# SnakeOnex/vit-is-all-you-need

Measured on AMD Instinct MI355X. Metric: images/sec ViT-B/16 224px bf16 fwd+bwd, higher is better.
Workload: dtype bf16; 1 GPU; ViT-B/16 224x224 bf16 forward+loss+backward, batch 256 per GPU (BASELINE configs[1]; configs[2] at 8 GPUs), random-init weights, 197 tokens, 79.44 M params; global_batch=256, parallelism=dp1

## Files before the change

### include/vitamd.h

```cpp
#ifndef VITAMD_H
#define VITAMD_H

#ifdef __cplusplus
extern "C" {
#endif

#define VITAMD_OK 0
#define VITAMD_ERR_SHAPE 1
#define VITAMD_ERR_ARG 2
#define VITAMD_ERR_LAUNCH 3
#define VITAMD_ERR_INIT 4

int vitamd_abi_version(void);

int vitamd_init(int device, void* stream);

#define VITAMD_EPI_BIAS_BF16 0
#define VITAMD_EPI_GELU 1
#define VITAMD_EPI_RESID_F32 2
#define VITAMD_EPI_DGELU 3
#define VITAMD_EPI_PATCH_F32 4
#define VITAMD_EPI_F32 5
#define VITAMD_EPI_GELU_DG 6
#define VITAMD_EPI_DMUL 7

int vitamd_gemm_nt_bf16(const void* A, const void* B, void* out, void* out2, const float* bias, const void* aux,
                        float* colsum, int M, int N, int K, int ldo, int epi, int n_patches, int seq, int extra,
                        int tile, void* stream);

#define VITAMD_NT_FORM_SMALL 1
#define VITAMD_NT_FORM_PP 2
#define VITAMD_NT_FORM_PP_PERSISTENT 3
#define VITAMD_NT_FORM_SEAM 4
#define VITAMD_NT_FORM_LOADER 5
#define VITAMD_NT_FORM_TAIL_SPLIT 0x80
int vitamd_gemm_nt_plan(int M, int N, int K, int ldo, int epi, int tile);

int vitamd_linear_dropout_resid_bf16(const void* A, const void* B, float* out, const float* bias, const float* resid,
                                     int M, int N, int K, float dropout_p, unsigned long long seed, int tile, void* stream);

int vitamd_gemm_tn_bf16(const void* L, const void* Rm, float* out, int R, int P, int Q, int ldl, int ldr, int ldo,
                        int splits, void* stream);

#define VITAMD_TN_FORM_SHARED 0
#define VITAMD_TN_FORM_EXCLUSIVE 1
int vitamd_gemm_tn_bf16_ws(const void* L, const void* Rm, float* out, int R, int P, int Q, int ldl, int ldr, int ldo,
                           int splits, float* ws, long ws_bytes, int accumulate, int form, void* stream);
long vitamd_gemm_tn_ws_bytes(int R, int P, int Q, int splits);

int vitamd_gemm_tn_bf16_ws_colsum(const void* L, const void* Rm, float* out, float* colsum, int R, int P, int Q, int ldl, int ldr,
                                  int ldo, int splits, float* ws, long ws_bytes, int accumulate, int form, void* stream);

int vitamd_layernorm_fwd(const float* x_in, const void* addend_bf16, float* x_out, void* y_bf16, float* mean,
                         float* rstd, int M, int D, float eps, void* stream);
int vitamd_layernorm_bwd(const void* dy_bf16, const float* x, const float* mean, const float* rstd,
                         const float* g_res, float* g_out, void* g_bf16, float* colsum, int M, int D, void* stream);
int vitamd_layernorm_bwd_dropout(const void* dy_bf16, const float* x, const float* mean, const float* rstd,
                                 const float* g_res, float* g_out, void* g_bf16, float* colsum, int M, int D,
                                 float dropout_p, unsigned long long seed, void* stream);
int vitamd_layernorm_bwd_xhat(const void* dy_bf16, const void* y_bf16, const float* rstd, const float* g_res, float* g_out,
                              void* g_bf16, float* colsum, int M, int D, float dropout_p, unsigned long long seed, void* stream);
int vitamd_layernorm_fwd_keep(const float* x_in, const void* addend_bf16, float* x_out, void* y_bf16, float* mean, float* rstd,
                              int B, int seq, int keep, int D, float eps, void* stream);
int vitamd_layernorm_bwd_keep(const void* dy_bf16, const void* x_or_y, const float* mean, const float* rstd, const float* g_res,
                              float* g_out, void* g_bf16, float* colsum, int B, int seq, int keep, int D, int use_xhat,
                              float dropout_p, unsigned long long seed, void* stream);

int vitamd_layernorm_affine_fwd(const float* x, const float* gamma, const float* beta, void* y_bf16, float* mean,
                                float* rstd, int M, int D, float eps, void* stream);
int vitamd_layernorm_affine_bwd(const void* dy_bf16, const float* x, const float* mean, const float* rstd,
                                const float* gamma, const float* g_res, float* g_out, void* g_bf16, float* colsum,
                                float* dgamma, float* dbeta, int M, int D, void* stream);
int vitamd_layernorm_affine_fwd_f32(const float* x, const float* gamma, const float* beta, float* y, float* mean,
                                    float* rstd, int M, int D, float eps, void* stream);
int vitamd_layernorm_affine_bwd_f32(const float* dy, const float* x, const float* mean, const float* rstd,
                                    const float* gamma, float* g_out, float* dgamma, float* dbeta, int M, int D, void* stream);

int vitamd_attention_fwd(const void* qkv, void* o, float* lse2, int B, int N, int H, int head_dim, int causal,
                         float dropout_p, unsigned long long seed, void* stream);
int vitamd_attention_fwd_resid(const void* qkv, void* o, float* lse2, const float* resid_in, float* resid_out, int B, int N, int H,
                               int head_dim, int causal, float dropout_p, unsigned long long seed, void* stream);
int vitamd_attention_bwd(const void* qkv, const void* o, const float* lse2, const void* d_o, void* dqkv,
                         float* delta, float* dbias, int B, int N, int H, int head_dim, int causal, float dropout_p,
                         unsigned long long seed, void* stream);
int vitamd_attention_keep_forms(int N, int nq);
int vitamd_attention_fwd_keep(const void* qkv, void* o, float* lse2, int B, int N, int H, int head_dim, int nq, void* stream);
int vitamd_attention_bwd_keep(const void* qkv, const void* o, const float* lse2, const void* d_o, void* dqkv, float* delta,
                              float* dbias, int B, int N, int H, int head_dim, int nq, void* stream);

#define VITAMD_ATTN_FWD_SMALL 1
#define VITAMD_ATTN_FWD_SMALL8 2
#define VITAMD_ATTN_FWD_LOOP 3
#define VITAMD_ATTN_FWD_LONG 4
#define VITAMD_ATTN_BWD_PIPE 5
#define VITAMD_ATTN_BWD_LOOP 6
#define VITAMD_ATTN_BWD_LONG 7
#define VITAMD_ATTN_FAMILY(code) ((code) & 0xf)
#define VITAMD_ATTN_TILES(code) ((code) >> 4 & 0xf)
#define VITAMD_ATTN_QTILES(code) ((code) >> 8 & 0xf)
#define VITAMD_ATTN_DROP 0x1000
#define VITAMD_ATTN_CAUSAL 0x2000
#define VITAMD_ATTN_RES 0x4000
#define VITAMD_ATTN_KEEP 0x8000
int vitamd_attention_form(int N, int causal, float dropout_p, int resid, int nq, int backward);

int vitamd_kv_append(const void* qkv, void* k_cache, void* v_cache, const int* len, int B, int T, int H, int head_dim, int Lmax,
                     void* stream);
long vitamd_decode_attention_ws_bytes(int B, int H, int Lmax);
int vitamd_decode_attention(const void* qkv, const void* k_cache, const void* v_cache, void* o, const int* len, int B, int H,
                            int head_dim, int Lmax, float* ws, long ws_bytes, void* stream);
long vitamd_gemm_skinny_ws_bytes(int M, int N, int K);
int vitamd_gemm_skinny_bf16(const void* A, const void* W, void* out, void* out2, const float* bias, const float* aux, int M, int N,
                            int K, int epi, float* ws, long ws_bytes, void* stream);

int vitamd_gemm_skinny_qkv_append(const void* A, const void* W, void* qkv, const float* bias, void* k_cache, void* v_cache, const int* len,
                                  int M, int H, int K, int head_dim, int Lmax, float* ws, long ws_bytes, void* stream);
int vitamd_decode_embed(const float* tok_table, const float* pos_table, const long long* token, const int* len, float* x, int B, int D,
                        int tok_rows, int pos_rows, void* stream);

int vitamd_sample_logits(const float* logits, long long* token, float* info, const float* u, const unsigned long long* step, int B, int V,
                         int ld, float temperature, int top_k, float top_p, unsigned long long seed, void* stream);

int vitamd_cross_entropy_fwd(const void* logits, int logits_bf16, const long long* target, float* loss_row, float* lse, float* stats,
                             int M, int V, int ld, long long ignore_index, void* stream);
int vitamd_cross_entropy_grid_rows(int V);
int vitamd_cross_entropy_bwd(const void* logits, int logits_bf16, const long long* target, const float* lse, const float* stats,
                             const float* grad_out, void* dlogits, int dlogits_bf16, int M, int V, int ld, int ldo,
                             long long ignore_index, void* stream);
int vitamd_soft_cross_entropy_fwd(const void* logits, int logits_bf16, const long long* target_a, const long long* target_b,
                                  const float* lam, float smoothing, float* loss_row, float* lse, float* stats, int M, int V, int ld,
                                  void* stream);
int vitamd_soft_cross_entropy_bwd(const void* logits, int logits_bf16, const long long* target_a, const long long* target_b,
                                  const float* lam, float smoothing, const float* lse, const float* stats, const float* grad_out,
                                  void* dlogits, int dlogits_bf16, int M, int V, int ld, int ldo, void* stream);
int vitamd_embed_tokens_fwd(const float* tok_table, const float* pos_table, const long long* ids, float* x, int B, int S, int D,
                            int tok_rows, int pos_rows, void* stream);
int vitamd_embed_tokens_bwd(const float* g, const long long* ids, float* dtok, float* dpos, int B, int S, int D, int tok_rows, void* stream);
int vitamd_assemble_tokens_fwd(const float* prefix, const float* pos, const float* tok_table, const long long* ids, const float* body,
                               float* x, int B, int E, int S, int D, int tok_rows, int pos_rows, void* stream);
int vitamd_assemble_tokens_bwd(const float* g, const long long* ids, float* dprefix, float* dpos, float* dtok, int B, int E, int S, int D,
                               int tok_rows, int pos_rows, void* stream);
int vitamd_assemble_tokens_grid_cap(void);

int vitamd_frames_prep(const unsigned char* src, const long long* index, const int* geom, const float* table, void* patches_bf16,
                       float* image, int B, int Nsrc, int Hs, int Ws, int C, int H, int W, int p, void* stream);
int vitamd_frames_prep_grid_cap(void);
int vitamd_frames_prep_mix(const unsigned char* src, const long long* index, const int* geom, const float* table, void* patches_bf16,
                           float* image, int B, int Nsrc, int Hs, int Ws, int C, int H, int W, int p, const int* rec, const float* lam,
                           void* stream);
int vitamd_frames_prep_resize(const unsigned char* src, const long long* index, const int* box, const float* mean, const float* std,
                              void* patches_bf16, float* image, int B, int Nsrc, int Hs, int Ws, int C, int H, int W, int p, void* stream);
int vitamd_frames_prep_resize_grid_cap(void);
int vitamd_crop_flip_draw(int* geom, int B, int Hs, int Ws, int H, int W, int flip_enabled, unsigned long long seed,
                          unsigned long long step, void* stream);
int vitamd_frames_to_u8(const float* img, unsigned char* out, int B, int C, int H, int W, void* stream);

int vitamd_cast_f32_bf16(const float* in, void* out_bf16, long n, void* stream);
int vitamd_cast_f32_bf16_dropout(const float* in, void* out_bf16, long n, float dropout_p, unsigned long long seed, void* stream);
int vitamd_dropout_bf16(const void* in, void* out, long n, long group, float dropout_p, unsigned long long seed, void* stream);
int vitamd_dropout_f32(const float* in, float* out, long n, long group, float dropout_p, unsigned long long seed, void* stream);
int vitamd_cast_transpose_weight(const float* w, void* wb, void* wbt, int N, int K, void* stream);
int vitamd_cast_transpose_batched(const void* desc_dev, int n, int total_tiles, void* stream);
int vitamd_im2col_bf16(const float* img, void* out_bf16, int B, int C, int H, int W, int p, void* stream);
int vitamd_colsum_bf16(const void* x_bf16, float* out, int M, int N, int ld, void* stream);
int vitamd_embed_bwd(const float* g, float* dpos, float* dextra, void* dyp_bf16, float* dbias, float* dbias_rows, int B,
                     int seq, int extra, int D, void* stream);

int vitamd_vq_nearest(const float* x, const float* codebook, long long* idx, int M, int K, int d, void* stream);

int vitamd_conv3x3_fwd(const float* x, const float* w, const float* bias, float* y, int B, int Cin, int Cout, int H, int W,
                       void* stream);
// ... 86 lines not shown
```

### vit-is-all-you-need_amd/csrc/attention.hip

```cpp
#include "common.h"
#include "vitamd_internal.h"
#include <type_traits>

namespace {

constexpr int DH = 64;
constexpr int MAX_N = 512;
constexpr int MAX_N_LONG = 16384;
constexpr float NEG_BIG = -1.0e30f;

typedef LDS_AS bf16x4* lds_bf16x4_ptr;

__device__ __forceinline__ int swz(int row) { return (((row >> 1) & 1) << 2) | ((row >> 3) & 3); }

__device__ __forceinline__ void stage_tile(const __bf16* __restrict__ g, int ld, int N, int npad, char* lds, int wave, int lane, int nwaves = 4) {
  const int pieces = npad / 8;
  for (int pc = wave; pc < pieces; pc += nwaves) {
    const int row = pc * 8 + (lane >> 3);
    const int logical = (lane & 7) ^ swz(row);
    const int grow = min(row, N - 1);
    glds16(g + (size_t)grow * ld + logical * 8, lds + pc * 1024);
  }
}

// ... 58 lines not shown
      u32x2 o = {pack_bf16x2(acc[dt][4 * u] * scale, acc[dt][4 * u + 1] * scale),
                 pack_bf16x2(acc[dt][4 * u + 2] * scale, acc[dt][4 * u + 3] * scale)};
      *(u32x2*)(p + 32 * dt + 8 * u) = o;
    }
}

template <int ROWS = 32, bool RES = false>
__device__ __forceinline__ void store_rows_T_img(__bf16* __restrict__ g, int ld, int N, int r0, int lane, const f32x16 (&acc)[2], float scale, char* img,
                                                 float* colacc = nullptr, const float* __restrict__ xi = nullptr, float* __restrict__ xo = nullptr,
                                                 int ldx = 0) {
  const int rr = lane & 31, h = lane >> 5;
  constexpr int ITS = ROWS / 8;
  int pass = 0;
#pragma unroll
  do {
    f32x4 r[ITS][2];
    if constexpr (RES) {
#pragma unroll
      for (int it = 0; it < ITS; ++it) {
        const int row = (lane >> 3) + 8 * it, pc = lane & 7;
        const float* px = xi + (size_t)min(r0 + ROWS * pass + row, N - 1) * ldx + 8 * (pc ^ (row & 7));
        r[it][0] = *(const f32x4*)px;
        r[it][1] = *(const f32x4*)(px + 4);
      }
    }
    if (ROWS == 32 || (rr >> 4) == pass) {
#pragma unroll
      for (int dt = 0; dt < 2; ++dt)
#pragma unroll
        for (int u = 0; u < 4; ++u) {
          u32x2 o = {pack_bf16x2(acc[dt][4 * u] * scale, acc[dt][4 * u + 1] * scale),
                     pack_bf16x2(acc[dt][4 * u + 2] * scale, acc[dt][4 * u + 3] * scale)};
          *(u32x2*)(img + (rr & (ROWS - 1)) * 128 + (((4 * dt + u) ^ (rr & 7)) << 4) + h * 8) = o;
        }
    }
#pragma unroll
    for (int it = 0; it < ITS; ++it) {
      const int row = (lane >> 3) + 8 * it, pc = lane & 7;
      const u32x4 v = *(const u32x4*)(img + row * 128 + pc * 16);
      const int grow = r0 + ROWS * pass + row;
      if (grow < N) {
        const int col = 8 * (pc ^ (row & 7));
        *(u32x4*)(g + (size_t)grow * ld + col) = v;
        if constexpr (RES) {
          f32x4 o0 = {r[it][0][0] + bf16lo(v[0]), r[it][0][1] + bf16hi(v[0]), r[it][0][2] + bf16lo(v[1]), r[it][0][3] + bf16hi(v[1])};
          f32x4 o1 = {r[it][1][0] + bf16lo(v[2]), r[it][1][1] + bf16hi(v[2]), r[it][1][2] + bf16lo(v[3]), r[it][1][3] + bf16hi(v[3])};
          float* po = xo + (size_t)grow * ldx + col;
          *(f32x4*)po = o0;
          *(f32x4*)(po + 4) = o1;
        }
      }
    }
  } while (ROWS == 16 && ++pass < 2);
  if constexpr (ROWS == 32) {
    if (colacc) {
      const int chunk = lane >> 3, within = (lane & 7) * 2;
      const int nrows = min(32, N - r0);
      float sacc = 0.f;
      for (int row = 0; row < nrows; ++row)
        sacc += bf2f(*(const __bf16*)(img + row * 128 + ((chunk ^ (row & 7)) << 4) + within));
      *colacc += sacc;
    }
  }
}

struct AttnArgs {
  const __bf16* qkv;
  __bf16* o;
  float* lse2;
  const __bf16* d_o;
  __bf16* dqkv;
  float* delta;
  float* dbias;
  int B, N, H;
  int causal;
  float scale_log2e;
  float scale;
  unsigned drop_thresh;
  float drop_scale;
  unsigned seed_lo, seed_hi;
  const float* resid_in;
  float* resid_out;
  int nq;
};

struct HeadAddr {
  int b, hh, N, D3, D;
  const __bf16* qbase;
};
template <typename Idx>
__device__ __forceinline__ HeadAddr head_addr(const __bf16* qkv, int N, int H, Idx head) {
  const int b = head / H, hh = head % H, D3 = 3 * H * DH, D = H * DH;
  return {b, hh, N, D3, D, qkv + (size_t)b * N * D3 + hh * DH};
}
__device__ __forceinline__ size_t stat_index(int b, int H, int hh, int N, int row) { return ((size_t)b * H + hh) * N + row; }

__device__ __forceinline__ float attn_keep(const AttnArgs& a, int bh, int query, int key) {
  const unsigned long long idx = ((unsigned long long)bh * a.N + query) * a.N + key;
  return dropout_keep(idx, a.seed_lo, a.seed_hi, a.drop_thresh, a.drop_scale);
}

template <bool DROP>
__global__ __launch_bounds__(256) void attn_fwd_kernel(const AttnArgs a) {
  extern __shared__ __attribute__((aligned(16))) char smem[];
  const int lane = threadIdx.x & 63, wave = __builtin_amdgcn_readfirstlane(threadIdx.x >> 6);
  const auto [b, hh, N, D3, D, qbase] = head_addr(a.qkv, a.N, a.H, blockIdx.x);
  const int nt = (N + 31) / 32, npad = nt * 32;
  char* ktile = smem;
  char* vtile = smem + npad * 128;
  stage_tile(qbase + D, D3, N, npad, ktile, wave, lane);
  stage_tile(qbase + 2 * D, D3, N, npad, vtile, wave, lane);
  asm volatile("s_waitcnt vmcnt(0)" ::: "memory");
  __syncthreads();

  const float c = a.scale_log2e;
  for (int qb = wave; qb < nt; qb += 4) {
    const int q0 = qb * 32;
    const int qrow = q0 + (lane & 31);
    bf16x8 qf[4];
    load_lane_frags(qbase, D3, N, q0, lane, qf);
    f32x16 oacc[2];
    zero(oacc);
    float m = NEG_BIG, l = 0.f;
    const int t_end = a.causal ? min(nt, qb + 1) : nt;
    for (int T = 0; T < t_end; ++T) {
      f32x16 s;
      zero(s);
#pragma unroll
      for (int kk = 0; kk < 4; ++kk) s = __builtin_amdgcn_mfma_f32_32x32x16_bf16(row_frag(ktile, T, kk, lane), qf[kk], s, 0, 0, 0);
      if (32 * T + 32 > N || (a.causal && T == qb)) {
#pragma unroll
        for (int r = 0; r < 16; ++r) {
          const int key = 32 * T + acc_row(r, lane);
          if (!(key < N && (!a.causal || key <= qrow))) s[r] = NEG_BIG;
        }
      }
      float tmax = max16(s);
      tmax = fmaxf(tmax, __shfl_xor(tmax, 32, 64)) * c;
      const float mnew = fmaxf(m, tmax);
      const float alpha = fast_exp2(m - mnew);
      m = mnew;
      float psum = 0.f;
#pragma unroll
      for (int r = 0; r < 16; ++r) {
        s[r] = fast_exp2(__builtin_fmaf(s[r], c, -mnew));
        psum += s[r];
        if constexpr (DROP) s[r] *= attn_keep(a, blockIdx.x, min(qrow, N - 1), min(32 * T + acc_row(r, lane), N - 1));
      }
      l = l * alpha + psum;
#pragma unroll
      for (int dt = 0; dt < 2; ++dt)
#pragma unroll
        for (int r = 0; r < 16; ++r) oacc[dt][r] *= alpha;
#pragma unroll
      for (int sidx = 0; sidx < 2; ++sidx) {
        const bf16x8 pf = acc_to_frag(s, sidx);
#pragma unroll
        for (int dt = 0; dt < 2; ++dt)
          oacc[dt] = __builtin_amdgcn_mfma_f32_32x32x16_bf16(tr_frag(vtile, T, sidx, dt, lane), pf, oacc[dt], 0, 0, 0);
      }
    }
    l += __shfl_xor(l, 32, 64);
    const float inv = 1.0f / l;
    store_rows_T(a.o + (size_t)b * N * D + hh * DH, D, N, q0, lane, oacc, inv);
    if (lane < 32 && qrow < N) a.lse2[stat_index(b, a.H, hh, N, qrow)] = m + log2f(l);
  }
// ... 26 lines not shown

  const float c = a.scale_log2e;
  for (int qb = wrot; qb < nt; qb += 4) {
    const int q0 = qb * 32;
    const int qrow = q0 + (lane & 31);
    if (qb != wrot) {
#pragma unroll
      for (int kk = 0; kk < 4; ++kk) qf[kk] = qf2[kk];
    }
    const int t_end = CAUSAL ? qb + 1 : nt;
    f32x16 s[NKT];
    float mx = NEG_BIG;
#pragma unroll
    for (int T = 0; T < NKT; ++T) {
      if (T < t_end) {
#pragma unroll
        for (int r = 0; r < 16; ++r) s[T][r] = 0.f;
#pragma unroll
        for (int kk = 0; kk < 4; ++kk) s[T] = __builtin_amdgcn_mfma_f32_32x32x16_bf16(row_frag(ktile, T, kk, lane), qf[kk], s[T], 0, 0, 0);
        if (32 * T + 32 > N || (CAUSAL && T == qb)) {
#pragma unroll
          for (int r = 0; r < 16; ++r) {
            const int key = 32 * T + acc_row(r, lane);
            if (!(key < N && (!CAUSAL || key <= qrow))) s[T][r] = NEG_BIG;
          }
        }
        mx = fmaxf(mx, max16(s[T]));
      }
    }
    mx = fmaxf(mx, __shfl_xor(mx, 32, 64));
    const float mc = mx * c;
    float l = 0.f;
    f32x16 oacc[2];
#pragma unroll
    for (int dt = 0; dt < 2; ++dt)
#pragma unroll
      for (int r = 0; r < 16; ++r) oacc[dt][r] = 0.f;
#pragma unroll
    for (int T = 0; T < NKT; ++T) {
      if (T < t_end) {
#pragma unroll
        for (int r = 0; r < 16; ++r) {
          float pexp = fast_exp2(__builtin_fmaf(s[T][r], c, -mc));
          l += pexp;
          if constexpr (DROP) pexp *= attn_keep(a, head, min(qrow, N - 1), min(32 * T + acc_row(r, lane), N - 1));
          s[T][r] = pexp;
        }
#pragma unroll
        for (int sidx = 0; sidx < 2; ++sidx) {
          const bf16x8 pf = acc_to_frag(s[T], sidx);
#pragma unroll
          for (int dt = 0; dt < 2; ++dt)
            oacc[dt] = __builtin_amdgcn_mfma_f32_32x32x16_bf16(tr_frag(vtile, T, sidx, dt, lane), pf, oacc[dt], 0, 0, 0);
        }
      }
    }
    l += __shfl_xor(l, 32, 64);
    const float inv = 1.0f / l;
    if constexpr (RES)
      store_rows_T_img<32, true>(a.o + (size_t)b * N * D + hh * DH, D, N, q0, lane, oacc, inv, oimg, nullptr, a.resid_in + (size_t)b * N * D + hh * DH,
                                 a.resid_out + (size_t)b * N * D + hh * DH, D);
    else
      store_rows_T_img(a.o + (size_t)b * N * D + hh * DH, D, N, q0, lane, oacc, inv, oimg);
    if (lane < 32 && qrow < N) a.lse2[stat_index(b, a.H, hh, N, qrow)] = mc + log2f(l);
  }
}

template <int NKT, bool RES, bool KEEP = false>
__global__ __launch_bounds__(512, 4) void attn_fwd_small8_kernel(const AttnArgs a) {
  extern __shared__ __attribute__((aligned(16))) char smem[];
  const int lane = threadIdx.x & 63, wave = __builtin_amdgcn_readfirstlane(threadIdx.x >> 6);
  const int head = blockIdx.x;
  const auto [b, hh, N, D3, D, qbase] = head_addr(a.qkv, a.N, a.H, head);
  constexpr int nt = NKT, npad = NKT * 32;
  char* ktile = smem;
  char* vtile = smem + npad * 128;
  char* oimg = smem + 2 * npad * 128 + wave * 2048;
  stage_tile(qbase + D, D3, N, npad, ktile, wave, lane, 8);
  stage_tile(qbase + 2 * D, D3, N, npad, vtile, wave, lane, 8);
  const int qb = (wave + head) & 7;
  bool active = qb < nt;
  if constexpr (KEEP) active = qb * 32 < a.nq;
  bf16x8 qf[4];
  load_lane_frags(qbase, D3, N, (active ? qb : 0) * 32, lane, qf);
  asm volatile("s_waitcnt vmcnt(0)" ::: "memory");
#pragma unroll
  for (int kk = 0; kk < 4; ++kk) asm volatile("" : "+v"(qf[kk]));
  __syncthreads();
  if (!active) return;
  const float c = a.scale_log2e;
  const int q0 = qb * 32;
  const int qrow = q0 + (lane & 31);
  float m = NEG_BIG, l = 0.f;
  f32x16 oacc[2];
  zero(oacc);
#pragma unroll 1
  for (int T = 0; T < NKT; ++T) {
    f32x16 st;
    zero(st);
#pragma unroll
    for (int kk = 0; kk < 4; ++kk) st = __builtin_amdgcn_mfma_f32_32x32x16_bf16(row_frag(ktile, T, kk, lane), qf[kk], st, 0, 0, 0);
    if (32 * T + 32 > N) {
#pragma unroll
      for (int r = 0; r < 16; ++r)
        if (!(32 * T + acc_row(r, lane) < N)) st[r] = NEG_BIG;
    }
    float mt = max16(st);
    mt = fmaxf(mt, __shfl_xor(mt, 32, 64));
    const float mn = fmaxf(m, mt);
    const float alpha = fast_exp2((m - mn) * c);
    m = mn;
    const float mc = mn * c;
    float lt = 0.f;
#pragma unroll
    for (int r = 0; r < 16; ++r) {
      const float pexp = fast_exp2(__builtin_fmaf(st[r], c, -mc));
      lt += pexp;
      st[r] = pexp;
    }
    l = l * alpha + lt;
    if (T > 0) {
#pragma unroll
      for (int dt = 0; dt < 2; ++dt)
#pragma unroll
        for (int r = 0; r < 16; ++r) oacc[dt][r] *= alpha;
    }
#pragma unroll
    for (int sidx = 0; sidx < 2; ++sidx) {
      const bf16x8 pf = acc_to_frag(st, sidx);
#pragma unroll
      for (int dt = 0; dt < 2; ++dt)
        oacc[dt] = __builtin_amdgcn_mfma_f32_32x32x16_bf16(tr_frag(vtile, T, sidx, dt, lane), pf, oacc[dt], 0, 0, 0);
    }
  }
  l += __shfl_xor(l, 32, 64);
  const float mc = m * c;
  const float inv = 1.0f / l;
  if constexpr (KEEP) {
    store_rows_T_img<16>(a.o + (size_t)b * a.nq * D + hh * DH, D, a.nq, q0, lane, oacc, inv, oimg);
    if (lane < 32 && qrow < a.nq) a.lse2[stat_index(b, a.H, hh, N, qrow)] = mc + log2f(l);
    return;
  }
  if constexpr (RES)
    store_rows_T_img<16, true>(a.o + (size_t)b * N * D + hh * DH, D, N, q0, lane, oacc, inv, oimg, nullptr, a.resid_in + (size_t)b * N * D + hh * DH,
                               a.resid_out + (size_t)b * N * D + hh * DH, D);
  else
    store_rows_T_img<16>(a.o + (size_t)b * N * D + hh * DH, D, N, q0, lane, oacc, inv, oimg);
  if (lane < 32 && qrow < N) a.lse2[stat_index(b, a.H, hh, N, qrow)] = mc + log2f(l);
}

template <bool DROP, bool CAUSAL>
__global__ __launch_bounds__(256, 2) void attn_bwd_dq_kernel(const AttnArgs a) {
  extern __shared__ __attribute__((aligned(16))) char smem[];
  const int lane = threadIdx.x & 63, wave = __builtin_amdgcn_readfirstlane(threadIdx.x >> 6);
  const auto [b, hh, N, D3, D, qbase] = head_addr(a.qkv, a.N, a.H, blockIdx.x);
  const int nt = (N + 31) / 32, npad = nt * 32;
  char* ktile = smem;
  char* vtile = smem + npad * 128;
  char* oimg = smem + 2 * npad * 128 + wave * 4096;
  stage_tile(qbase + D, D3, N, npad, ktile, wave, lane);
  stage_tile(qbase + 2 * D, D3, N, npad, vtile, wave, lane);
  asm volatile("s_waitcnt vmcnt(0)" ::: "memory");
  __syncthreads();

  const float c = a.scale_log2e;
  const __bf16* obase = a.o + (size_t)b * N * D + hh * DH;
  const __bf16* dobase = a.d_o + (size_t)b * N * D + hh * DH;
  float csum_q = 0.f;
  for (int qb = (wave + blockIdx.x) & 3; qb < nt; qb += 4) {
    const int q0 = qb * 32;
    const int qrow = q0 + (lane & 31);
    bf16x8 qf[4], dof[4], of[4];
    load_lane_frags(qbase, D3, N, q0, lane, qf);
    load_lane_frags(dobase, D, N, q0, lane, dof);
    load_lane_frags(obase, D, N, q0, lane, of);
    float delta = 0.f;
#pragma unroll
    for (int kk = 0; kk < 4; ++kk)
#pragma unroll
      for (int j = 0; j < 8; ++j) delta += (float)dof[kk][j] * (float)of[kk][j];
    delta += __shfl_xor(delta, 32, 64);
    const size_t stat = stat_index(b, a.H, hh, N, min(qrow, N - 1));
    const float lse2 = a.lse2[stat];
    if (lane < 32 && qrow < N) a.delta[stat] = delta;

    f32x16 dq[2];
    zero(dq);
    const int t_end = CAUSAL ? min(nt, qb + 1) : nt;
    for (int T = 0; T < t_end; ++T) {
      f32x16 s, dp;
      zero(s);
      zero(dp);
#pragma unroll
      for (int kk = 0; kk < 4; ++kk) {
        s = __builtin_amdgcn_mfma_f32_32x32x16_bf16(row_frag(ktile, T, kk, lane), qf[kk], s, 0, 0, 0);
        dp = __builtin_amdgcn_mfma_f32_32x32x16_bf16(row_frag(vtile, T, kk, lane), dof[kk], dp, 0, 0, 0);
      }
#pragma unroll
      for (int r = 0; r < 16; ++r) {
        const float pexp = fast_exp2(__builtin_fmaf(s[r], c, -lse2));
        float dpr = dp[r];
        if constexpr (DROP) dpr *= attn_keep(a, blockIdx.x, min(qrow, N - 1), min(32 * T + acc_row(r, lane), N - 1));
        s[r] = pexp * (dpr - delta);
      }
      if (32 * T + 32 > N || (CAUSAL && T == qb)) {
#pragma unroll
        for (int r = 0; r < 16; ++r) {
          const int key = 32 * T + acc_row(r, lane);
          if (!(key < N && (!CAUSAL || key <= qrow))) s[r] = 0.f;
        }
      }
#pragma unroll
      for (int sidx = 0; sidx < 2; ++sidx) {
        const bf16x8 dsf = acc_to_frag(s, sidx);
#pragma unroll
        for (int dt = 0; dt < 2; ++dt)
          dq[dt] = __builtin_amdgcn_mfma_f32_32x32x16_bf16(tr_frag(ktile, T, sidx, dt, lane), dsf, dq[dt], 0, 0, 0);
      }
    }
    store_rows_T_img(a.dqkv + (size_t)b * N * D3 + hh * DH, D3, N, q0, lane, dq, a.scale, oimg, a.dbias ? &csum_q : nullptr);
  }
  if (a.dbias) atomicAdd(a.dbias + hh * DH + lane, csum_q);
}

template <int NT, int NQT = NT, bool LIM = false>
__global__ __launch_bounds__(256, 2) void attn_bwd_dq_pipe_kernel(const AttnArgs a) {
  extern __shared__ __attribute__((aligned(16))) char smem[];
  const int lane = threadIdx.x & 63, wave = __builtin_amdgcn_readfirstlane(threadIdx.x >> 6);
  const int head = blockIdx.x;
  const auto [b, hh, N, D3, D, qbase] = head_addr(a.qkv, a.N, a.H, head);
  constexpr int nt = NT, npad = NT * 32;
  char* ktile = smem;
  char* vtile = smem + npad * 128;
  char* oimg = smem + 2 * npad * 128 + wave * 4096;
  stage_tile(qbase + D, D3, N, npad, ktile, wave, lane);
  stage_tile(qbase + 2 * D, D3, N, npad, vtile, wave, lane);
  int nq = N;
  if constexpr (LIM) nq = a.nq;
  const __bf16* obase = a.o + (size_t)b * nq * D + hh * DH;
  const __bf16* dobase = a.d_o + (size_t)b * nq * D + hh * DH;
  asm volatile("s_waitcnt vmcnt(0)" ::: "memory");
  __syncthreads();

  const float c = a.scale_log2e;
  float csum_q = 0.f;
  for (int qb = (wave + head) & 3; qb < nt; qb += 4) {
    const int q0 = qb * 32;
    const int qrow = q0 + (lane & 31);
    if constexpr (LIM) {
      if (qb >= NQT) {
        __bf16* zp = a.dqkv + (size_t)b * N * D3 + hh * DH + 8 * (lane & 7);
#pragma unroll
        for (int it = 0; it < 4; ++it) {
          const int row = q0 + (lane >> 3) + 8 * it;
          if (row < N) *(u32x4*)(zp + (size_t)row * D3) = (u32x4){0u, 0u, 0u, 0u};
        }
        continue;
      }
    }
    bf16x8 qf[4], dof[4];
    float delta = 0.f;
    {
      bf16x8 of[4];
      load_lane_frags(qbase, D3, N, q0, lane, qf);
      load_lane_frags(dobase, D, nq, q0, lane, dof);
      load_lane_frags(obase, D, nq, q0, lane, of);
      if constexpr (LIM) {
        if (qrow >= nq) {
#pragma unroll
          for (int kk = 0; kk < 4; ++kk)
#pragma unroll
            for (int j = 0; j < 8; ++j) dof[kk][j] = (__bf16)0.f;
        }
      }
#pragma unroll
      for (int kk = 0; kk < 4; ++kk)
#pragma unroll
        for (int j = 0; j < 8; ++j) delta += (float)dof[kk][j] * (float)of[kk][j];
    }
    delta += __shfl_xor(delta, 32, 64);
    const size_t stat = stat_index(b, a.H, hh, N, min(qrow, nq - 1));
    float lse2 = a.lse2[stat];
    if constexpr (LIM) lse2 = qrow < nq ? lse2 : 1.0e30f;
    if (lane < 32 && qrow < nq) a.delta[stat] = delta;

    f32x16 dq[2];
#pragma unroll
    for (int dt = 0; dt < 2; ++dt)
#pragma unroll
      for (int r = 0; r < 16; ++r) dq[dt][r] = 0.f;
    bf16x8 kr[2][4], vr[2][4];
    f32x16 sb[2], dpb[2];
    auto products = [&](int buf) {
#pragma unroll
      for (int r = 0; r < 16; ++r) { sb[buf][r] = 0.f; dpb[buf][r] = 0.f; }
#pragma unroll
      for (int kk = 0; kk < 4; ++kk) {
        sb[buf] = __builtin_amdgcn_mfma_f32_32x32x16_bf16(kr[buf][kk], qf[kk], sb[buf], 0, 0, 0);
        dpb[buf] = __builtin_amdgcn_mfma_f32_32x32x16_bf16(vr[buf][kk], dof[kk], dpb[buf], 0, 0, 0);
      }
    };
#pragma unroll
    for (int kk = 0; kk < 4; ++kk) { kr[0][kk] = row_frag(ktile, 0, kk, lane); vr[0][kk] = row_frag(vtile, 0, kk, lane); }
    if (NT > 1) {
#pragma unroll
      for (int kk = 0; kk < 4; ++kk) { kr[1][kk] = row_frag(ktile, 1, kk, lane); vr[1][kk] = row_frag(vtile, 1, kk, lane); }
    }
    products(0);
#pragma unroll
    for (int T = 0; T < NT; ++T) {
      const int cur = T & 1, nxt = cur ^ 1;
      bf16x8 ktr[2][2];
#pragma unroll
      for (int sidx = 0; sidx < 2; ++sidx)
#pragma unroll
        for (int dt = 0; dt < 2; ++dt) ktr[sidx][dt] = tr_frag(ktile, T, sidx, dt, lane);
      __builtin_amdgcn_sched_barrier(0);
      if (T + 1 < NT) products(nxt);
      if (T + 2 < NT) {
#pragma unroll
        for (int kk = 0; kk < 4; ++kk) { kr[cur][kk] = row_frag(ktile, T + 2, kk, lane); vr[cur][kk] = row_frag(vtile, T + 2, kk, lane); }
      }
#pragma unroll
      for (int r = 0; r < 16; ++r) {
        const float pexp = fast_exp2(__builtin_fmaf(sb[cur][r], c, -lse2));
        sb[cur][r] = pexp * (dpb[cur][r] - delta);
      }
      if (T == NT - 1 && 32 * T + 32 > N) {
#pragma unroll
        for (int r = 0; r < 16; ++r)
          if (!(32 * T + acc_row(r, lane) < N)) sb[cur][r] = 0.f;
      }
#pragma unroll
      for (int sidx = 0; sidx < 2; ++sidx) {
        const bf16x8 dsf = acc_to_frag(sb[cur], sidx);
#pragma unroll
        for (int dt = 0; dt < 2; ++dt) dq[dt] = __builtin_amdgcn_mfma_f32_32x32x16_bf16(ktr[sidx][dt], dsf, dq[dt], 0, 0, 0);
      }
    }
    store_rows_T_img(a.dqkv + (size_t)b * N * D3 + hh * DH, D3, N, q0, lane, dq, a.scale, oimg, a.dbias ? &csum_q : nullptr);
  }
  if (a.dbias) atomicAdd(a.dbias + hh * DH + lane, csum_q);
}

template <bool DROP, bool CAUSAL>
__global__ __launch_bounds__(256, 2) void attn_bwd_dkv_kernel(const AttnArgs a) {
  extern __shared__ __attribute__((aligned(16))) char smem[];
  const int lane = threadIdx.x & 63, wave = __builtin_amdgcn_readfirstlane(threadIdx.x >> 6);
  const auto [b, hh, N, D3, D, qbase] = head_addr(a.qkv, a.N, a.H, blockIdx.x);
  const int nt = (N + 31) / 32, npad = nt * 32;
  char* qtile = smem;
  char* dotile = smem + npad * 128;
  float* lse_s = (float*)(smem + 2 * npad * 128);
  float* delta_s = lse_s + npad;
  char* oimg = smem + 2 * npad * 128 + 2 * npad * 4 + wave * 4096;
  const __bf16* dobase = a.d_o + (size_t)b * N * D + hh * DH;
  stage_tile(qbase, D3, N, npad, qtile, wave, lane);
  stage_tile(dobase, D, N, npad, dotile, wave, lane);
  for (int i = threadIdx.x; i < npad; i += 256) {
    const size_t stat = stat_index(b, a.H, hh, N, min(i, N - 1));
    lse_s[i] = a.lse2[stat];
    delta_s[i] = a.delta[stat];
  }
  asm volatile("s_waitcnt vmcnt(0)" ::: "memory");
  __syncthreads();

  const float c = a.scale_log2e;
  float csum_k = 0.f, csum_v = 0.f;
  for (int kb = (wave + blockIdx.x) & 3; kb < nt; kb += 4) {
    const int k0 = kb * 32;
    const int krow = k0 + (lane & 31);
    bf16x8 kf[4], vf[4];
    load_lane_frags(qbase + D, D3, N, k0, lane, kf);
    load_lane_frags(qbase + 2 * D, D3, N, k0, lane, vf);
    f32x16 dk[2], dv[2];
    zero(dk);
    zero(dv);
    const int t_beg = CAUSAL ? kb : 0;
    for (int T = t_beg; T < nt; ++T) {
      f32x16 s, dp;
      zero(s);
      zero(dp);
#pragma unroll
      for (int kk = 0; kk < 4; ++kk) {
        s = __builtin_amdgcn_mfma_f32_32x32x16_bf16(row_frag(qtile, T, kk, lane), kf[kk], s, 0, 0, 0);
        dp = __builtin_amdgcn_mfma_f32_32x32x16_bf16(row_frag(dotile, T, kk, lane), vf[kk], dp, 0, 0, 0);
      }
      f32x16 pmat;
#pragma unroll
      for (int u = 0; u < 4; ++u) {
        const int qr = 32 * T + 8 * u + 4 * (lane >> 5);
        const f32x4 lse4 = *(const f32x4*)(lse_s + qr);
        const f32x4 del4 = *(const f32x4*)(delta_s + qr);
#pragma unroll
        for (int i = 0; i < 4; ++i) {
          const int r = 4 * u + i;
          const float pexp = fast_exp2(__builtin_fmaf(s[r], c, -lse4[i]));
          float keep = 1.0f;
          if constexpr (DROP) keep = attn_keep(a, blockIdx.x, min(qr + i, N - 1), min(krow, N - 1));
          pmat[r] = pexp * keep;
          s[r] = pexp * (dp[r] * keep - del4[i]);
        }
        if (32 * T + 32 > N || k0 + 32 > N || (CAUSAL && T == kb)) {
#pragma unroll
          for (int i = 0; i < 4; ++i) {
            const int r = 4 * u + i, query = qr + i;
            if (!(query < N && krow < N && (!CAUSAL || krow <= query))) { pmat[r] = 0.f; s[r] = 0.f; }
          }
        }
      }
#pragma unroll
      for (int sidx = 0; sidx < 2; ++sidx) {
        const bf16x8 pf = acc_to_frag(pmat, sidx);
        const bf16x8 dsf = acc_to_frag(s, sidx);
#pragma unroll
        for (int dt = 0; dt < 2; ++dt) {
          dv[dt] = __builtin_amdgcn_mfma_f32_32x32x16_bf16(tr_frag(dotile, T, sidx, dt, lane), pf, dv[dt], 0, 0, 0);
          dk[dt] = __builtin_amdgcn_mfma_f32_32x32x16_bf16(tr_frag(qtile, T, sidx, dt, lane), dsf, dk[dt], 0, 0, 0);
        }
      }
    }
    __bf16* dbase = a.dqkv + (size_t)b * N * D3 + hh * DH;
    store_rows_T_img(dbase + D, D3, N, k0, lane, dk, a.scale, oimg, a.dbias ? &csum_k : nullptr);
    store_rows_T_img(dbase + 2 * D, D3, N, k0, lane, dv, 1.0f, oimg, a.dbias ? &csum_v : nullptr);
  }
  if (a.dbias) {
    atomicAdd(a.dbias + D + hh * DH + lane, csum_k);
    atomicAdd(a.dbias + 2 * D + hh * DH + lane, csum_v);
  }
}

template <int NT, int NQT = NT, bool LIM = false>
__global__ __launch_bounds__(256, 2) void attn_bwd_dkv_pipe_kernel(const AttnArgs a) {
  extern __shared__ __attribute__((aligned(16))) char smem[];
  const int lane = threadIdx.x & 63, wave = __builtin_amdgcn_readfirstlane(threadIdx.x >> 6);
  const int head = blockIdx.x;
  const int b = head / a.H, hh = head % a.H;
  const int N = a.N, D3 = 3 * a.H * DH, D = a.H * DH;
  constexpr int nt = NT, npad = NQT * 32;
  int nq = N;
  if constexpr (LIM) nq = a.nq;
  char* qtile = smem;
  char* dotile = smem + npad * 128;
  float* lse_s = (float*)(smem + 2 * npad * 128);
  float* delta_s = lse_s + npad;
  char* oimg = smem + 2 * npad * 128 + 2 * npad * 4 + wave * 4096;
  const __bf16* qbase = a.qkv + (size_t)b * N * D3 + hh * DH;
  const __bf16* dobase = a.d_o + (size_t)b * nq * D + hh * DH;
  stage_tile(qbase, D3, N, npad, qtile, wave, lane);
  stage_tile(dobase, D, nq, npad, dotile, wave, lane);
  for (int i = threadIdx.x; i < npad; i += 256) {
    const size_t stat = ((size_t)b * a.H + hh) * N + min(i, nq - 1);
    lse_s[i] = i < nq ? a.lse2[stat] : 1.0e30f;
    delta_s[i] = a.delta[stat];
  }
  asm volatile("s_waitcnt vmcnt(0)" ::: "memory");
  __syncthreads();

  const float c = a.scale_log2e;
  float csum_k = 0.f, csum_v = 0.f;
  for (int kb = (wave + head) & 3; kb < nt; kb += 4) {
    const int k0 = kb * 32;
    bf16x8 kf[4], vf[4];
    load_lane_frags(qbase + D, D3, N, k0, lane, kf);
    load_lane_frags(qbase + 2 * D, D3, N, k0, lane, vf);
    f32x16 dk[2], dv[2];
    zero(dk);
    zero(dv);
    bf16x8 qr[4], dor[4];
    f32x16 sb, dpb;
    auto products = [&]() {
      zero(sb);
      zero(dpb);
#pragma unroll
      for (int kk = 0; kk < 4; ++kk) {
        sb = __builtin_amdgcn_mfma_f32_32x32x16_bf16(qr[kk], kf[kk], sb, 0, 0, 0);
        dpb = __builtin_amdgcn_mfma_f32_32x32x16_bf16(dor[kk], vf[kk], dpb, 0, 0, 0);
      }
    };
#pragma unroll
    for (int kk = 0; kk < 4; ++kk) { qr[kk] = row_frag(qtile, 0, kk, lane); dor[kk] = row_frag(dotile, 0, kk, lane); }
    products();
    if (NQT > 1) {
#pragma unroll
      for (int kk = 0; kk < 4; ++kk) { qr[kk] = row_frag(qtile, 1, kk, lane); dor[kk] = row_frag(dotile, 1, kk, lane); }
    }
#pragma unroll
    for (int T = 0; T < NQT; ++T) {
      bf16x8 dotr[2][2], qtr[2][2];
      f32x4 lse4[4], del4[4];
#pragma unroll
      for (int sidx = 0; sidx < 2; ++sidx)
#pragma unroll
        for (int dt = 0; dt < 2; ++dt) { dotr[sidx][dt] = tr_frag(dotile, T, sidx, dt, lane); qtr[sidx][dt] = tr_frag(qtile, T, sidx, dt, lane); }
      __builtin_amdgcn_sched_barrier(0);
#pragma unroll
      for (int u = 0; u < 4; ++u) {
        const int qr0 = 32 * T + 8 * u + 4 * (lane >> 5);
        lse4[u] = *(const f32x4*)(lse_s + qr0);
        del4[u] = *(const f32x4*)(delta_s + qr0);
      }
      f32x16 pmat;
#pragma unroll
      for (int u = 0; u < 4; ++u)
#pragma unroll
        for (int i = 0; i < 4; ++i) {
          const int r = 4 * u + i;
          const float pexp = fast_exp2(__builtin_fmaf(sb[r], c, -lse4[u][i]));
          pmat[r] = pexp;
          sb[r] = pexp * (dpb[r] - del4[u][i]);
        }
#pragma unroll
      for (int sidx = 0; sidx < 2; ++sidx) {
        const bf16x8 pf = acc_to_frag(pmat, sidx);
        const bf16x8 dsf = acc_to_frag(sb, sidx);
#pragma unroll
        for (int dt = 0; dt < 2; ++dt) {
          dv[dt] = __builtin_amdgcn_mfma_f32_32x32x16_bf16(dotr[sidx][dt], pf, dv[dt], 0, 0, 0);
          dk[dt] = __builtin_amdgcn_mfma_f32_32x32x16_bf16(qtr[sidx][dt], dsf, dk[dt], 0, 0, 0);
        }
      }
      if (T + 1 < NQT) products();
      if (T + 2 < NQT) {
#pragma unroll
        for (int kk = 0; kk < 4; ++kk) { qr[kk] = row_frag(qtile, T + 2, kk, lane); dor[kk] = row_frag(dotile, T + 2, kk, lane); }
      }
    }
    __bf16* dbase = a.dqkv + (size_t)b * N * D3 + hh * DH;
    store_rows_T_img(dbase + D, D3, N, k0, lane, dk, a.scale, oimg, a.dbias ? &csum_k : nullptr);
    store_rows_T_img(dbase + 2 * D, D3, N, k0, lane, dv, 1.0f, oimg, a.dbias ? &csum_v : nullptr);
  }
  if (a.dbias) {
// ... 408 lines not shown
      return with_flag(f.drop, [&](auto DR) {
        const dim3 grid(a.B * a.H, (nkt + 3) / 4);
        if (int el = launch<attn_bwd_dq_long_kernel<CONST_OF(DR)>>(grid, block, 2 * CH * 128 + 4 * 4096, stream, a)) return el;
        return launch<attn_bwd_dkv_long_kernel<CONST_OF(DR)>>(grid, block, 2 * CH * 128 + 2 * CH * 4 + 4 * 4096, stream, a);
      });
    case ATTN_BWD_PIPE:
      if (f.keep)
        return with_tiles<2, 7>(f.nt, [&](auto K) {
          return with_tiles<1, 4>(f.nqt, [&](auto Q) { return launch_bwd_pipe<CONST_OF(K), CONST_OF(Q), true>(a, stream); });
        });
      return with_tiles<2, 7>(f.nt, [&](auto K) { return launch_bwd_pipe<CONST_OF(K), CONST_OF(K), false>(a, stream); });
    case ATTN_BWD_LOOP:
      return with_flag(f.drop, [&](auto DR) {
        return with_flag(f.causal, [&](auto CAUSAL) {
          const dim3 grid(a.B * a.H);
          if (int el = launch<attn_bwd_dq_kernel<CONST_OF(DR), CONST_OF(CAUSAL)>>(grid, block, 2 * npad * 128 + 4 * 4096, stream, a)) return el;
          return launch<attn_bwd_dkv_kernel<CONST_OF(DR), CONST_OF(CAUSAL)>>(grid, block, 2 * npad * 128 + 2 * npad * 4 + 4 * 4096, stream, a);
        });
      });
  }
  return VITAMD_ERR_SHAPE;
}

int attention_fwd_impl(const void* qkv, void* o, float* lse2, const float* resid_in, float* resid_out, int B, int N, int H, int head_dim, int causal,
                       float dropout_p, unsigned long long seed, void* stream_) {
  AttnArgs a;
  if (int e = make_args(a, false, qkv, o, lse2, nullptr, nullptr, nullptr, nullptr, B, N, H, head_dim, causal, dropout_p, seed)) return e;
  a.resid_in = resid_in;
  a.resid_out = resid_out;
  AttnForm f;
  if (int e = attention_form(f, N, causal != 0, a.drop_thresh != 0u, resid_in != nullptr, 0, false)) return e;
  return launched(launch_fwd(f, a, (hipStream_t)stream_));
}

}

extern "C" int vitamd_attention_form(int N, int causal, float dropout_p, int resid, int nq, int backward) {
  AttnForm f;
  const DropoutParams d = dropout_params(dropout_p, 0ull);
  if (int e = attention_form(f, N, causal != 0, d.ok ? d.thresh != 0u : dropout_p != 0.f, resid != 0, nq, backward != 0)) return -e;
  if (!d.ok) return -VITAMD_ERR_ARG;
  return f.code();
}

extern "C" int vitamd_attention_fwd(const void* qkv, void* o, float* lse2, int B, int N, int H, int head_dim, int causal,
                                    float dropout_p, unsigned long long seed, void* stream_) {
  return attention_fwd_impl(qkv, o, lse2, nullptr, nullptr, B, N, H, head_dim, causal, dropout_p, seed, stream_);
}

extern "C" int vitamd_attention_fwd_resid(const void* qkv, void* o, float* lse2, const float* resid_in, float* resid_out, int B, int N,
                                          int H, int head_dim, int causal, float dropout_p, unsigned long long seed, void* stream_) {
  if (!resid_in || !resid_out) return VITAMD_ERR_ARG;
  AttnForm f;
  if (int e = attention_form(f, N, false, false, true, 0, false)) return e;
  return attention_fwd_impl(qkv, o, lse2, resid_in, resid_out, B, N, H, head_dim, causal, dropout_p, seed, stream_);
}

extern "C" int vitamd_attention_bwd(const void* qkv, const void* o, const float* lse2, const void* d_o, void* dqkv, float* delta,
                                    float* dbias, int B, int N, int H, int head_dim, int causal, float dropout_p,
                                    unsigned long long seed, void* stream_) {
  AttnArgs a;
  if (int e = make_args(a, true, qkv, o, lse2, d_o, dqkv, delta, dbias, B, N, H, head_dim, causal, dropout_p, seed)) return e;
  AttnForm f;
  if (int e = attention_form(f, N, causal != 0, a.drop_thresh != 0u, false, 0, true)) return e;
  return launched(launch_bwd(f, a, (hipStream_t)stream_));
}

extern "C" int vitamd_attention_keep_forms(int N, int nq) {
  if (nq <= 0) return 0;
  AttnForm f;
  return (attention_form(f, N, false, false, false, nq, false) == VITAMD_OK ? 1 : 0) |
         (attention_form(f, N, false, false, false, nq, true) == VITAMD_OK ? 2 : 0);
}

extern "C" int vitamd_attention_fwd_keep(const void* qkv, void* o, float* lse2, int B, int N, int H, int head_dim, int nq, void* stream_) {
  AttnArgs a;
  if (int e = make_args(a, false, qkv, o, lse2, nullptr, nullptr, nullptr, nullptr, B, N, H, head_dim, 0, 0.f, 0ull, nq)) return e;
  AttnForm f;
  if (nq <= 0) return VITAMD_ERR_SHAPE;
  if (int e = attention_form(f, N, false, false, false, nq, false)) return e;
  return launched(launch_fwd(f, a, (hipStream_t)stream_));
}

extern "C" int vitamd_attention_bwd_keep(const void* qkv, const void* o, const float* lse2, const void* d_o, void* dqkv, float* delta,
                                         float* dbias, int B, int N, int H, int head_dim, int nq, void* stream_) {
  AttnArgs a;
  if (int e = make_args(a, true, qkv, o, lse2, d_o, dqkv, delta, dbias, B, N, H, head_dim, 0, 0.f, 0ull, nq)) return e;
  AttnForm f;
  if (nq <= 0) return VITAMD_ERR_SHAPE;
  if (int e = attention_form(f, N, false, false, false, nq, true)) return e;
  return launched(launch_bwd(f, a, (hipStream_t)stream_));
}
```

### vit-is-all-you-need_amd/csrc/capi.hip

```cpp
#include "common.h"
#include "vitamd_internal.h"
#include "../../include/vitamd.h"

extern "C" int vitamd_abi_version(void) { return 9; }

extern "C" int vitamd_init(int device, void* stream) { return vitamd_init_impl(device, (hipStream_t)stream); }

extern "C" int vitamd_gemm_nt_bf16(const void* A, const void* B, void* out, void* out2, const float* bias, const void* aux,
                                   float* colsum, int M, int N, int K, int ldo, int epi, int n_patches, int seq, int extra,
                                   int tile, void* stream) {
  const int dg = (epi == 6 || epi == 7) ? 1 : 0;
  if (epi == 6) epi = EPI_GELU;
  if (epi == 7) epi = EPI_DGELU;
  GemmNtArgs p{A, B, out, out2, bias, aux, colsum, M, N, K, ldo, epi, n_patches, seq, extra, tile, 0u, 1.0f, 0u, 0u, 0, dg};
  if (!is_auto(tile) && tile != NT_TILE_128 && tile != NT_TILE_256 && tile != NT_TILE_320 && tile != NT_TILE_LOADER && tile != NT_TILE_SEAM) return VITAMD_ERR_ARG;
  return vitamd_gemm_nt_impl(p, (hipStream_t)stream);
}

extern "C" int vitamd_gemm_nt_plan(int M, int N, int K, int ldo, int epi, int tile) {
  const int dg = (epi == 6 || epi == 7) ? 1 : 0;
  if (epi == 6) epi = EPI_GELU;
  if (epi == 7) epi = EPI_DGELU;
  static char dummy[16];
  GemmNtArgs p{dummy, dummy, dummy, dummy, nullptr, dummy, (float*)dummy, M, N, K, ldo, epi, 1, 1, 0, tile, 0u, 1.0f, 0u, 0u, 0, dg};
  if (!is_auto(tile) && tile != NT_TILE_128 && tile != NT_TILE_256 && tile != NT_TILE_320 && tile != NT_TILE_LOADER && tile != NT_TILE_SEAM) return -VITAMD_ERR_ARG;
  return vitamd_gemm_nt_plan_impl(p);
}

extern "C" int vitamd_gemm_tn_bf16(const void* L, const void* Rm, float* out, int R, int P, int Q, int ldl, int ldr, int ldo,
                                   int splits, void* stream) {
  GemmTnArgs a{L, Rm, out, R, P, Q, ldl, ldr, ldo, splits, nullptr, 0, 1, 0};
  return vitamd_gemm_tn_impl(a, (hipStream_t)stream);
}

extern "C" int vitamd_gemm_tn_bf16_ws(const void* L, const void* Rm, float* out, int R, int P, int Q, int ldl, int ldr, int ldo,
                                      int splits, float* ws, long ws_bytes, int accumulate, int form, void* stream) {
  if (form != 0 && form != 1) return VITAMD_ERR_ARG;
  GemmTnArgs a{L, Rm, out, R, P, Q, ldl, ldr, ldo, splits, ws, (size_t)(ws_bytes < 0 ? 0 : ws_bytes), accumulate, form};
  return vitamd_gemm_tn_impl(a, (hipStream_t)stream);
}

extern "C" int vitamd_gemm_tn_bf16_ws_colsum(const void* L, const void* Rm, float* out, float* colsum, int R, int P, int Q, int ldl, int ldr,
                                             int ldo, int splits, float* ws, long ws_bytes, int accumulate, int form, void* stream) {
  if (form != 0 && form != 1) return VITAMD_ERR_ARG;
  GemmTnArgs a{L, Rm, out, R, P, Q, ldl, ldr, ldo, splits, ws, (size_t)(ws_bytes < 0 ? 0 : ws_bytes), accumulate, form, colsum};
  if (colsum && !ws) return VITAMD_ERR_ARG;
  return vitamd_gemm_tn_impl(a, (hipStream_t)stream);
}

extern "C" int vitamd_linear_dropout_resid_bf16(const void* A, const void* B, float* out, const float* bias, const float* resid,
                                                int M, int N, int K, float dropout_p, unsigned long long seed, int tile, void* stream) {
  if (!is_auto(tile) && tile != NT_TILE_128 && tile != NT_TILE_256 && tile != NT_TILE_320) return VITAMD_ERR_ARG;
  const DropoutParams d = dropout_params(dropout_p, seed);
  if (!d.ok) return VITAMD_ERR_ARG;
  GemmNtArgs p{A, B, out, nullptr, bias, resid, nullptr, M, N, K, N, EPI_RESID_F32, 0, 0, 0, tile, d.thresh, d.scale, d.seed_lo, d.seed_hi, 0, 0};
  return vitamd_gemm_nt_impl(p, (hipStream_t)stream);
}
```

### vit-is-all-you-need_amd/csrc/gemm_nt.hip

```cpp
#include <type_traits>
#include <mutex>
#include <atomic>
#include <cmath>
#include <cstring>
#include <climits>
#include "gemm_nt_ld.h"

namespace {

template <int BM, int BN, int WM, int WN, int EPI>
__global__ __launch_bounds__(WM * WN * 64) void gemm_nt_kernel(const GemmNtArgs p) {
  constexpr int NW = WM * WN;
  constexpr int WTM = BM / WM, WTN = BN / WN;
  constexpr int MT = WTM / 16, NT = WTN / 16;
  constexpr int PIECES = (BM + BN) / 8;
  constexpr int PPW = PIECES / NW;
  static_assert(PIECES % NW == 0, "pieces must divide over waves");
  constexpr int BUF_BYTES = (BM + BN) * 128;

  extern __shared__ __attribute__((aligned(16))) char smem[];

  const int tid = threadIdx.x;
  const int lane = tid & 63;
  const int wave = __builtin_amdgcn_readfirstlane(tid >> 6);
  const int wm = wave / WN, wn = wave % WN;

  const int tiles_n = (p.N + BN - 1) / BN;
  const int tiles_m = (p.M + BM - 1) / BM;
  const int tile = xcd_remap(blockIdx.x, tiles_m * tiles_n);
  const int m0 = (tile / tiles_n) * BM;
  const int n0 = (tile % tiles_n) * BN;

  const __bf16* __restrict__ A = (const __bf16*)p.A;
  const __bf16* __restrict__ B = (const __bf16*)p.B;
  const int K = p.K;

  const __bf16* src[PPW];
#pragma unroll
  for (int i = 0; i < PPW; ++i) {
    const int piece = wave * PPW + i;
    const int row = piece * 8 + (lane >> 3);
    const int logical = (lane & 7) ^ (row & 7);
    if (piece < BM / 8) {
      const int g = min(m0 + row, p.M - 1);
      src[i] = A + (size_t)g * K + logical * 8;
    } else {
      const int g = min(n0 + row - BM, p.N - 1);
      src[i] = B + (size_t)g * K + logical * 8;
    }
  }

  auto stage = [&](int kt, int buf) {
    char* base = smem + buf * BUF_BYTES + wave * PPW * 1024;
#pragma unroll
    for (int i = 0; i < PPW; ++i) glds16(src[i] + kt * BK, base + i * 1024);
  };

  f32x4 acc[MT][NT];
#pragma unroll
  for (int i = 0; i < MT; ++i)
#pragma unroll
    for (int j = 0; j < NT; ++j) acc[i][j] = (f32x4){0.f, 0.f, 0.f, 0.f};

  const int frag_off = (lane & 15) * 128 + ((((lane >> 4) ^ (lane & 7)) & 7) << 4);
  const int a_off = wm * WTM * 128 + frag_off;
  const int b_off = BM * 128 + wn * WTN * 128 + frag_off;

  const int nkt = K / BK;
  stage(0, 0);
  for (int kt = 0; kt < nkt; ++kt) {
    const int cur = kt & 1;
    asm volatile("s_waitcnt vmcnt(0)" ::: "memory");
    __syncthreads();
    if (kt + 1 < nkt) stage(kt + 1, cur ^ 1);
    const char* buf = smem + cur * BUF_BYTES;
#pragma unroll
    for (int ks = 0; ks < 2; ++ks) {
      bf16x8 af[MT], bfr[NT];
#pragma unroll
      for (int j = 0; j < NT; ++j) bfr[j] = *(const bf16x8*)(buf + ((b_off + j * 16 * 128) ^ (ks * 64)));
#pragma unroll
      for (int i = 0; i < MT; ++i) af[i] = *(const bf16x8*)(buf + ((a_off + i * 16 * 128) ^ (ks * 64)));
#pragma unroll
      for (int i = 0; i < MT; ++i)
#pragma unroll
        for (int j = 0; j < NT; ++j)
          acc[i][j] = __builtin_amdgcn_mfma_f32_16x16x32_bf16(bfr[j], af[i], acc[i][j], 0, 0, 0);
    }
  }
  if constexpr (BM == 256 && BN == 256 && WM == 2 && WN == 4 && EPI != EPI_F32) {
    if (p.N % 8 == 0 && p.ldo % 8 == 0) {
      gemm_epilogue_rows<EPI>(p, acc, m0, n0, wm, wn, lane, tid, wave, smem);
      return;
    }
  }
  gemm_epilogue<BN, WM, WN, WTM, WTN, MT, NT, EPI>(p, acc, m0, n0, wm, wn, lane, tid, smem);
}

template <int EPI, int MT, int LA, int LB, bool PERS = false>
__global__ __launch_bounds__(512) void gemm_nt_pp_kernel(const GemmNtArgs p) {
  using S = NtSchedule<MT, LA>;
  static_assert(LB == S::LB, "the B lead the shared schedule implements");
  constexpr int NP = S::NP;
  constexpr int BM = 32 * MT, BN = 256, WN = 4, NT = 4;
  constexpr int PART = 64 * 128;
  constexpr int BUFB = NP * PART + 256 * 128;

  extern __shared__ __attribute__((aligned(16))) char smem[];
  const int tid = threadIdx.x, lane = tid & 63;
  const int wave = __builtin_amdgcn_readfirstlane(tid >> 6);
  const int wm = wave / WN, wn = wave % WN;
  const int tiles_n = (p.N + BN - 1) / BN, tiles_m = (p.M + BM - 1) / BM;
  const int ntiles = tiles_m * tiles_n;
  const int K = p.K;
  const int nkt = K / 64;
  const srd_t srdA = make_srd(p.A, (size_t)p.M * K * 2);
  const srd_t srdB = make_srd(p.B, (size_t)p.N * K * 2);
  for (int ti = blockIdx.x; ti < ntiles; ti += PERS ? (int)gridDim.x : ntiles) {
  const NtTile t = nt_tile<BM>(ti, tiles_m, tiles_n);
  const int m0 = t.m0, n0 = t.n0;
  unsigned voffA[NP], voffB[4];
  pp_offsets<MT, false>(p, t, wave, lane, voffA, voffB);
  const unsigned lds0 = lds_addr(smem) + wave * 1024;
  constexpr unsigned OOB = 0x80000000u;
  auto request_a = [&](int kt, int j) {
    const bool live = kt >= 0 && kt < nkt;
    asm_glds16(srdA, lds0 + (kt & 1) * BUFB + j * PART, live ? voffA[j] : OOB, live ? (unsigned)kt * 128u : 0u);
  };
  auto request_b = [&](int kt, int q) {
    const bool live = kt >= 0 && kt < nkt;
    asm_glds16(srdB, lds0 + (kt & 1) * BUFB + NP * PART + q * 8192, live ? voffB[q] : OOB, live ? (unsigned)kt * 128u : 0u);
  };

  f32x4 acc[MT][NT];
#pragma unroll
  for (int i = 0; i < MT; ++i)
#pragma unroll
    for (int j = 0; j < NT; ++j) acc[i][j] = (f32x4){0.f, 0.f, 0.f, 0.f};

  const char *rdA[2], *rdB[2];
  frag_bases(smem + wm * 32 * 128, lane, rdA);
  frag_bases(smem + NP * PART + wn * 64 * 128, lane, rdB);

#pragma unroll
  for (int P = -S::lookback; P < 0; ++P) S::requests(S::tile_of(P), S::phase_of(P), request_a, request_b);
  VITAMD_WAIT_VM(S::wait(NP - 1));
  __builtin_amdgcn_s_barrier();
  asm volatile("" ::: "memory");
  if (wm == 1) __builtin_amdgcn_s_barrier();

  auto ktile = [&](int kt, auto bufc) {
    constexpr int BUF = decltype(bufc)::value;
    pp_ktile<MT, PART>(acc, rdA[0] + BUF * BUFB, rdA[1] + BUF * BUFB, rdB[0] + BUF * BUFB, rdB[1] + BUF * BUFB,
                       [&](int ph) { S::requests(kt, ph, request_a, request_b); }, [&](int ph) { VITAMD_WAIT_VM(S::wait(ph)); });
  };
  int kt = 0;
  for (; kt + 1 < nkt; kt += 2) {
    ktile(kt, std::integral_constant<int, 0>{});
    ktile(kt + 1, std::integral_constant<int, 1>{});
  }
  if (kt < nkt) ktile(kt, std::integral_constant<int, 0>{});
  if (wm == 0) __builtin_amdgcn_s_barrier();
  asm volatile("s_waitcnt vmcnt(0)" ::: "memory");
  if constexpr (EPI == EPI_F32) gemm_epilogue<BN, 2, WN, 16 * MT, 64, MT, NT, EPI>(p, acc, m0, n0, wm, wn, lane, tid, smem);
  else if (p.N % 8 == 0 && p.ldo % 8 == 0) gemm_epilogue_rows<EPI, MT>(p, acc, m0, n0, wm, wn, lane, tid, wave, smem);
  else gemm_epilogue<BN, 2, WN, 16 * MT, 64, MT, NT, EPI>(p, acc, m0, n0, wm, wn, lane, tid, smem);
  if constexpr (PERS) __syncthreads();
  }
}

static int device_cus() {
  static int cus[16] = {};
  int dev = 0;
  if (hipGetDevice(&dev) != hipSuccess || dev < 0 || dev >= 16) return 256;
  if (!cus[dev]) {
    int n = 0;
    cus[dev] = (hipDeviceGetAttribute(&n, hipDeviceAttributeMultiprocessorCount, dev) == hipSuccess && n > 0) ? n : 256;
  }
  return cus[dev];
}

template <int EPI, int MT, int LA, int LB, bool PERS = false>
int launch_pp(const GemmNtArgs& p, hipStream_t stream) {
  constexpr int ops_b = 2 * ((MT / 2) * 8192 + 32768), epi_b = 8 * MT * 2048;
  return launch_tiles(gemm_nt_pp_kernel<EPI, MT, LA, LB, PERS>, p, stream, 32 * MT, 512, ops_b > epi_b ? ops_b : epi_b, PERS ? device_cus() : INT_MAX);
}
#undef VITAMD_WAIT_VM

template <int BM, int BN, int WM, int WN, int EPI>
int launch(const GemmNtArgs& p, hipStream_t stream) {
  constexpr int lds = 2 * (BM + BN) * 128;
  auto kern = gemm_nt_kernel<BM, BN, WM, WN, EPI>;
  if (int e = set_lds(kern, lds)) return e;
  const int tiles = ((p.M + BM - 1) / BM) * ((p.N + BN - 1) / BN);
  hipLaunchKernelGGL(kern, dim3(tiles), dim3(WM * WN * 64), lds, stream, p);
  return hipGetLastError() == hipSuccess ? VITAMD_OK : VITAMD_ERR_LAUNCH;
}

static bool prefer_tall(const GemmNtArgs& p) {
// ... 6 lines not shown

static unsigned short bf16_rne_d(double v) {
  auto val = [](unsigned short b) { const unsigned w = (unsigned)b << 16; float g; memcpy(&g, &w, 4); return (double)g; };
  const float f = (float)v;
  unsigned u;
  memcpy(&u, &f, 4);
  unsigned short best = (unsigned short)((u + 0x7fffu + ((u >> 16) & 1u)) >> 16);
  double bd = fabs(val(best) - v);
  const unsigned short first = best;
  for (int dl = -1; dl <= 1; dl += 2) {
    const unsigned short n = (unsigned short)(first + dl);
    const double dd = fabs(val(n) - v);
    if (dd < bd || (dd == bd && !(n & 1) && (best & 1))) { best = n; bd = dd; }
  }
  return best;
}

static std::atomic<const unsigned*> g_gelu_tab[64];

static const unsigned* gelu_table() {
  int dev = -1;
  if (hipGetDevice(&dev) != hipSuccess || dev < 0 || dev >= 64) { (void)hipGetLastError(); return nullptr; }
  return g_gelu_tab[dev].load(std::memory_order_acquire);
}

}

const unsigned* vitamd_gelu_table() { return gelu_table(); }

int vitamd_init_impl(int device, hipStream_t stream) {
  static std::mutex mu;
  static unsigned host[4096];
  static bool built = false;
  int cur = -1;
  if (hipGetDevice(&cur) != hipSuccess) { (void)hipGetLastError(); return VITAMD_ERR_LAUNCH; }
  if (device < 0) device = cur;
  if (device >= 64) return VITAMD_ERR_ARG;
  std::lock_guard<std::mutex> lock(mu);
  if (g_gelu_tab[device].load(std::memory_order_acquire)) return VITAMD_OK;
  hipStreamCaptureStatus cap = hipStreamCaptureStatusNone;
  if (hipStreamIsCapturing(stream, &cap) != hipSuccess || cap != hipStreamCaptureStatusNone) { (void)hipGetLastError(); return VITAMD_ERR_ARG; }
  if (!built) {
    for (int sg = 0; sg < 2; ++sg)
      for (int i = 0; i < 2048; ++i) {
        const unsigned w = (unsigned)(0x3900 + i) << 16;
        float ax;
        memcpy(&ax, &w, 4);
        const double x = sg ? -(double)ax : (double)ax;
        const double cdf = 0.5 * erfc(-x * 0.70710678118654752440);
        const double pdf = 0.39894228040143267794 * exp(-0.5 * x * x);
        host[sg * 2048 + i] = (unsigned)bf16_rne_d(x * cdf) | ((unsigned)bf16_rne_d(cdf + x * pdf) << 16);
      }
    built = true;
  }
  if (device != cur && hipSetDevice(device) != hipSuccess) { (void)hipGetLastError(); return VITAMD_ERR_ARG; }
  void* d = nullptr;
  bool ok = hipMalloc(&d, sizeof(host)) == hipSuccess;
  ok = ok && hipMemcpy(d, host, sizeof(host), hipMemcpyHostToDevice) == hipSuccess && hipDeviceSynchronize() == hipSuccess;
  if (!ok) {
    (void)hipGetLastError();
    if (d) (void)hipFree(d);
  }
  if (device != cur) (void)hipSetDevice(cur);
  if (!ok) return VITAMD_ERR_LAUNCH;
  g_gelu_tab[device].store((const unsigned*)d, std::memory_order_release);
  return VITAMD_OK;
}

namespace {

enum NtForm { NT_FORM_SMALL = 1, NT_FORM_PP = 2, NT_FORM_PP_PERSISTENT = 3, NT_FORM_SEAM = 4, NT_FORM_LOADER = 5 };
struct NtPlan { int form, rows, err; };

static NtPlan plan_single(const GemmNtArgs& p) {
  int tile = p.tile;
  const int epi = p.epi;
  const bool seam_epi = epi == EPI_BIAS_BF16 || epi == EPI_GELU || epi == EPI_DGELU;
  const bool tall_epi = seam_epi || epi == EPI_RESID_F32;
  if (tile == NT_TILE_LOADER) return (seam_epi && ld_ok(p)) ? NtPlan{NT_FORM_LOADER, 256, VITAMD_OK} : NtPlan{0, 0, VITAMD_ERR_SHAPE};
  if (tile == NT_TILE_SEAM) return (seam_epi && seam_ok(p)) ? NtPlan{NT_FORM_SEAM, 256, VITAMD_OK} : NtPlan{0, 0, VITAMD_ERR_SHAPE};
  const bool no_seam = tile == NT_TILE_AUTO_NO_SEAM;
  if (no_seam) tile = NT_TILE_AUTO;
  const long big_tiles = (long)((p.M + 255) / 256) * ((p.N + 255) / 256);
  const bool pp_ok = (size_t)p.M * p.K * 2 < 0xf0000000ull && (size_t)p.N * p.K * 2 < 0xf0000000ull && p.K % 64 == 0;
  const bool big = p.N >= 256 && big_tiles >= 192 && pp_ok;
  const bool tall = tall_epi && prefer_tall(p);
  if (tile == NT_TILE_AUTO_NO_PERSISTENT) tile = NT_TILE_AUTO;
  else if (tile == NT_TILE_AUTO && big) {
    const int cus = device_cus();
    if (seam_epi && !no_seam && seam_ok(p) && p.K <= 1536) {
      if (epi == EPI_BIAS_BF16 && tall && (long)((p.M + 319) / 320) * ((p.N + 255) / 256) >= 3L * cus) return NtPlan{NT_FORM_SEAM, 320, VITAMD_OK};
      if (big_tiles >= 3L * cus) return NtPlan{ld_ok(p) ? NT_FORM_LOADER : NT_FORM_SEAM, 256, VITAMD_OK};
    }
    return NtPlan{NT_FORM_PP_PERSISTENT, tall ? 320 : 256, VITAMD_OK};
  }
  if (tile == NT_TILE_AUTO) tile = big ? (tall ? NT_TILE_320 : NT_TILE_256) : NT_TILE_128;
  if (tile == NT_TILE_320) return (tall_epi && pp_ok) ? NtPlan{NT_FORM_PP, 320, VITAMD_OK} : NtPlan{0, 0, VITAMD_ERR_SHAPE};
  if (tile == NT_TILE_256) return pp_ok ? NtPlan{NT_FORM_PP, 256, VITAMD_OK} : NtPlan{0, 0, VITAMD_ERR_SHAPE};
  if (tile != NT_TILE_128) return NtPlan{0, 0, VITAMD_ERR_ARG};
  return p.K % BK == 0 ? NtPlan{NT_FORM_SMALL, 128, VITAMD_OK} : NtPlan{0, 0, VITAMD_ERR_SHAPE};
}

template <int EPI>
int dispatch_tile(const GemmNtArgs& p, hipStream_t stream) {
  constexpr bool seam_epi = EPI == EPI_BIAS_BF16 || EPI == EPI_GELU || EPI == EPI_DGELU;
  constexpr bool tall_epi = seam_epi || EPI == EPI_RESID_F32;
  const NtPlan pl = plan_single(p);
  if (pl.err) return pl.err;
  switch (pl.form) {
    case NT_FORM_LOADER:
      if constexpr (EPI == EPI_DGELU) { if (!p.colsum) return launch_ld<EPI_DGELU_NOCS>(p, stream, device_cus()); }
      if constexpr (seam_epi) return launch_ld<EPI, EPI == EPI_GELU>(p, stream, device_cus());
      break;
    case NT_FORM_SEAM:
      if constexpr (EPI == EPI_DGELU) { if (!p.colsum) return launch_seam<EPI_DGELU_NOCS, 8>(p, stream, device_cus()); }
      if constexpr (EPI == EPI_BIAS_BF16) { if (pl.rows == 320) return launch_seam<EPI, 10>(p, stream, device_cus()); }
      if constexpr (seam_epi) return launch_seam<EPI, 8, EPI == EPI_GELU>(p, stream, device_cus());
      break;
    case NT_FORM_PP_PERSISTENT:
      if constexpr (tall_epi) { if (pl.rows == 320) return launch_pp<EPI, 10, 4, 6, true>(p, stream); }
      return launch_pp<EPI, 8, 4, 6, true>(p, stream);
    case NT_FORM_PP:
      if constexpr (tall_epi) { if (pl.rows == 320) return launch_pp<EPI, 10, 4, 6>(p, stream); }
      return launch_pp<EPI, 8, 4, 6>(p, stream);
    case NT_FORM_SMALL:
      return launch<128, 128, 2, 2, EPI>(p, stream);
  }
  return VITAMD_ERR_SHAPE;
}

}

static int dispatch_epi(const GemmNtArgs& p, hipStream_t stream) {
  switch (p.epi) {
    case EPI_BIAS_BF16: return dispatch_tile<EPI_BIAS_BF16>(p, stream);
    case EPI_GELU: return dispatch_tile<EPI_GELU>(p, stream);
    case EPI_RESID_F32: return dispatch_tile<EPI_RESID_F32>(p, stream);
    case EPI_DGELU: return dispatch_tile<EPI_DGELU>(p, stream);
    case EPI_PATCH_F32: return dispatch_tile<EPI_PATCH_F32>(p, stream);
    case EPI_F32: return dispatch_tile<EPI_F32>(p, stream);
    default: return VITAMD_ERR_ARG;
  }
}

static int tail_split_rows(const GemmNtArgs& p, bool& tall) {
  const int CUS = device_cus();
  tall = is_auto(p.tile) && prefer_tall(p);
  const int bm = tall ? 320 : 256;
  const int tiles_m = (p.M + bm - 1) / bm, tiles_n = (p.N + 255) / 256;
  const long big_tiles = (long)tiles_m * tiles_n;
  const long rem = big_tiles % CUS;
  const bool split_on = p.epi == EPI_RESID_F32 && !tall;
  if (!(is_auto(p.tile) && split_on && p.epi != EPI_PATCH_F32 && p.N >= 256 && p.K % 64 == 0 && big_tiles > 2 * CUS && rem != 0 && rem * 10 < CUS * 6))
    return 0;
  const int rows_a = (int)((big_tiles - rem) / tiles_n) * bm;
  return rows_a > 0 && rows_a < p.M ? rows_a : 0;
}

static int check_args(const GemmNtArgs& p) {
  if (p.M <= 0 || p.N <= 0 || p.K <= 0 || p.K % 32 != 0 || p.N % 4 != 0 || p.ldo % 4 != 0) return VITAMD_ERR_SHAPE;
  if (!p.A || !p.B || !p.out) return VITAMD_ERR_ARG;
  if (p.epi == EPI_GELU && !p.out2) return VITAMD_ERR_ARG;
  if ((p.epi == EPI_RESID_F32 || p.epi == EPI_DGELU) && !p.aux) return VITAMD_ERR_ARG;
  if (p.epi == EPI_PATCH_F32 && (!p.aux || p.n_patches <= 0)) return VITAMD_ERR_ARG;
  if (p.epi < EPI_BIAS_BF16 || p.epi > EPI_F32) return VITAMD_ERR_ARG;
  return VITAMD_OK;
}

constexpr size_t NT_SPAN = 0x80000000ull;
constexpr int NT_PANEL_ROWS = 1280;

static size_t out_esz(const GemmNtArgs& p) { return (p.epi == EPI_RESID_F32 || p.epi == EPI_PATCH_F32 || p.epi == EPI_F32) ? 4 : 2; }

static int panel_rows(const GemmNtArgs& p) {
  if ((size_t)p.N * p.K * 2 >= NT_SPAN) return 0;
  const size_t kb = (size_t)p.K * 2, ob = (size_t)p.ldo * out_esz(p), row_bytes = kb > ob ? kb : ob;
  if ((size_t)p.M * row_bytes < NT_SPAN) return p.M;
  if (p.epi == EPI_PATCH_F32) return 0;
  return (int)((NT_SPAN - 1) / row_bytes / NT_PANEL_ROWS) * NT_PANEL_ROWS;
}

static GemmNtArgs rows_of(const GemmNtArgs& p, int r0, int rows) {
  GemmNtArgs q = p;
  q.M = rows;
  q.A = (const char*)p.A + (size_t)r0 * p.K * 2;
  q.out = (char*)p.out + (size_t)r0 * p.ldo * out_esz(p);
  if (p.out2) q.out2 = (char*)p.out2 + (size_t)r0 * p.ldo * 2;
  if (p.aux && p.epi != EPI_PATCH_F32) q.aux = (const char*)p.aux + (size_t)r0 * p.ldo * (p.epi == EPI_RESID_F32 ? 4 : 2);
  q.row0 = p.row0 + r0;
  return q;
}

static GemmNtArgs head_of(const GemmNtArgs& p, int rows_a, bool tall) {
  GemmNtArgs a = p;
  if (rows_a) {
    a.M = rows_a;
    a.tile = tall ? p.tile : NT_TILE_256;
  }
  return a;
}

static int launch_rows(const GemmNtArgs& p, hipStream_t stream) {
  bool tall = false;
  const int rows_a = tail_split_rows(p, tall);
  if (int e = dispatch_epi(head_of(p, rows_a, tall), stream)) return e;
  if (!rows_a) return VITAMD_OK;
  GemmNtArgs b = rows_of(p, rows_a, p.M - rows_a);
  b.tile = NT_TILE_128;
  return dispatch_epi(b, stream);
}

static int plan_rows(const GemmNtArgs& p) {
  bool tall = false;
  const int rows_a = tail_split_rows(p, tall);
  const NtPlan pl = plan_single(head_of(p, rows_a, tall));
  if (pl.err) return -pl.err;
  return pl.form | (pl.rows << 8) | (rows_a ? 0x80 : 0);
}

int vitamd_gemm_nt_impl(const GemmNtArgs& p0, hipStream_t stream) {
  if (int e = check_args(p0)) return e;
  const int rows = panel_rows(p0);
  if (!rows) return VITAMD_ERR_SHAPE;
  GemmNtArgs p = p0;
  if (p.epi == EPI_GELU) {
    p.gelu_tab = gelu_table();
    if (!p.gelu_tab) return VITAMD_ERR_INIT;
  }
  if (rows >= p.M) return launch_rows(p, stream);
  const int last = (p.M - 1) / rows * rows;
  if (int e = plan_rows(rows_of(p, 0, rows)); e < 0) return -e;
  if (int e = plan_rows(rows_of(p, last, p.M - last)); e < 0) return -e;
  for (int r0 = 0; r0 < p.M; r0 += rows)
    if (int e = launch_rows(rows_of(p, r0, p.M - r0 < rows ? p.M - r0 : rows), stream)) return e;
  return VITAMD_OK;
}

int vitamd_gemm_nt_plan_impl(const GemmNtArgs& p0) {
  if (int e = check_args(p0)) return -e;
  const int rows = panel_rows(p0);
  if (!rows) return -VITAMD_ERR_SHAPE;
  if (rows >= p0.M) return plan_rows(p0);
  const int last = (p0.M - 1) / rows * rows;
  if (int e = plan_rows(rows_of(p0, last, p0.M - last)); e < 0) return e;
  return plan_rows(rows_of(p0, 0, rows));
}
```

### vit-is-all-you-need_amd/csrc/gemm_nt_ld.h

```cpp
#pragma once
#include "gemm_nt_seam.h"

namespace {

template <int EPI, bool TAB = false, int SCHED = 1>
__global__ __launch_bounds__(768) void gemm_nt_ld_kernel(const GemmNtArgs p) {
  static_assert(EPI == EPI_BIAS_BF16 || EPI == EPI_GELU || EPI == EPI_DGELU || EPI == EPI_DGELU_NOCS, "epilogues of the loader form");
  static_assert(SCHED == 1, "request schedule");
  static_assert(!TAB || EPI == EPI_GELU, "table = GELU");
  constexpr bool DG = EPI == EPI_DGELU || EPI == EPI_DGELU_NOCS;
  constexpr bool CS = EPI == EPI_DGELU;
  constexpr int BM = 256, BN = 256, MT = 8, NT = 4;
  constexpr int AREG = 16384, ABUF = 32768, BBUF = 32768, BBASE = 2 * ABUF, OPS = BBASE + 2 * BBUF;
  constexpr int STG = 2048, TABOFF = OPS + 8 * STG;
  constexpr unsigned OOB = 0x80000000u;

  extern __shared__ __attribute__((aligned(16))) char smem[];
  const int tid = threadIdx.x, lane = tid & 63;
  const int wave = __builtin_amdgcn_readfirstlane(tid >> 6);
  const int tiles_n = (p.N + BN - 1) / BN, tiles_m = (p.M + BM - 1) / BM;
  const int ntiles = tiles_m * tiles_n;
  const int K = p.K;
  const int nkt = K / 64;
  auto coords = [&](int ti) { return nt_tile<BM>(ti, tiles_m, tiles_n); };

  if (wave >= 8) {
    const int l = wave - 8;
    const srd_t srdA = make_srd(p.A, (size_t)p.M * K * 2);
    const srd_t srdB = make_srd(p.B, (size_t)p.N * K * 2);
    const srd_t srdBias = make_srd(p.bias ? (const void*)p.bias : p.out, p.bias ? (size_t)p.N * 4 : 0);
    const unsigned ldsA = lds_addr(smem) + l * 4096;
    const unsigned ldsB = lds_addr(smem) + BBASE + l * 8192;
    unsigned voffA[2][4], voffB[8];
    auto offsets = [&](const NtTile& t) {
      const int r8 = lane >> 3;
      const unsigned chunk = (unsigned)(((lane & 7) ^ r8) * 16);
#pragma unroll
      for (int h = 0; h < 2; ++h)
#pragma unroll
        for (int i = 0; i < 4; ++i) {
          const int a = 4 * l + i;
          const int row = min(t.m0 + (a >> 3) * 128 + h * 64 + (a & 7) * 8 + r8, p.M - 1);
          voffA[h][i] = (unsigned)row * (unsigned)(K * 2) + chunk;
        }
#pragma unroll
      for (int i = 0; i < 8; ++i) {
        const int row = min(t.n0 + (8 * l + i) * 8 + r8, p.N - 1);
        voffB[i] = (unsigned)row * (unsigned)(K * 2) + chunk;
      }
    };
    bool live = true;
    unsigned so = 0u, par = 0u;
    auto request_b = [&](int i) {
      asm_glds16(srdB, ldsB + par * BBUF + i * 1024, live ? voffB[i] : OOB, so);
    };
    auto request_a = [&](int h, int i) {
      asm_glds16(srdA, ldsA + par * ABUF + h * AREG + i * 1024, live ? voffA[h][i] : OOB, so);
    };
    auto target = [&](int kt, bool lv) {
      live = lv;
      so = live ? (unsigned)kt * 128u : 0u;
      par = (unsigned)(kt & 1);
    };
    __builtin_amdgcn_s_setprio(3);
    int ti = blockIdx.x;
    NtTile cur = coords(ti);
    offsets(cur);
    int bias_n0 = cur.n0;
    target(0, true);
#pragma unroll
    for (int i = 0; i < 8; ++i) request_b(i);
#pragma unroll
    for (int i = 0; i < 4; ++i) request_a(0, i);
#pragma unroll
    for (int i = 0; i < 4; ++i) request_a(1, i);
    VITAMD_WAIT_VM(4);
    __builtin_amdgcn_s_barrier();
    for (;;) {
      const int ti_next = ti + (int)gridDim.x;
      const bool has_next = ti_next < ntiles;
      for (int kt = 0; kt < nkt; ++kt) {
        const bool last = kt + 1 == nkt;
        if (last && has_next) {
          cur = coords(ti_next);
          offsets(cur);
        }
        target(last ? 0 : kt + 1, !last || has_next);
        request_b(0); request_b(1); request_b(2);
        __builtin_amdgcn_s_barrier();
        request_b(3); request_b(4); request_b(5);
        VITAMD_WAIT_VM(6);
        __builtin_amdgcn_s_barrier();
        if constexpr (!DG) {
          if (kt == 0) {
            asm_glds4(srdBias, lds_addr(smem) + OPS + l * STG, (unsigned)(bias_n0 + l * 64 + lane) * 4u, 0u);
            asm_glds4(srdBias, lds_addr(smem) + OPS + (4 + l) * STG, (unsigned)(bias_n0 + l * 64 + lane) * 4u, 0u);
          }
        }
        request_b(6); request_b(7); request_a(0, 0);
        __builtin_amdgcn_s_barrier();
        request_a(0, 1); request_a(0, 2); request_a(0, 3);
        __builtin_amdgcn_s_barrier();
        request_a(1, 0); request_a(1, 1);
        __builtin_amdgcn_s_barrier();
        request_a(1, 2); request_a(1, 3);
        __builtin_amdgcn_s_barrier();
        __builtin_amdgcn_s_barrier();
        VITAMD_WAIT_VM(4);
        __builtin_amdgcn_s_barrier();
      }
      __builtin_amdgcn_s_barrier();
      if (!has_next) break;
      ti = ti_next;
      bias_n0 = cur.n0;
    }
    asm volatile("s_waitcnt vmcnt(0)" ::: "memory");
    return;
  }

  const int wm = wave >> 2, wn = wave & 3;
  const srd_t rsO = make_srd(p.out, (size_t)p.M * p.ldo * 2);
  const srd_t rsO2 = make_srd(EPI == EPI_GELU ? p.out2 : p.out, (size_t)p.M * p.ldo * 2);
  const srd_t srdAux = make_srd(DG ? p.aux : p.out, (size_t)p.M * p.ldo * 2);
  if constexpr (TAB) gelu_table_to_lds(p.gelu_tab, smem + TABOFF, tid);
  __builtin_amdgcn_s_barrier();
  asm volatile("" ::: "memory");
// ... 149 lines not shown
```

### vit-is-all-you-need_amd/csrc/gemm_nt_pp.h

```cpp
#pragma once
#include "gemm_nt_epilogue.h"

namespace {

struct NtTile { int m0, n0; };
template <int BM>
__device__ __forceinline__ NtTile nt_tile(int ti, int tiles_m, int tiles_n) {
  int tm, tn;
  tile_coords(xcd_remap(ti, tiles_m * tiles_n), tiles_m, tiles_n, tiles_n >= 6, tm, tn);
  return NtTile{tm * BM, tn * 256};
}

__device__ __forceinline__ void frag_bases(const char* base, int lane, const char* (&rd)[2]) {
  const int frag_off = (lane & 15) * 128 + ((((lane >> 4) ^ (lane & 7)) & 7) << 4);
  rd[0] = base + frag_off;
  rd[1] = base + (frag_off ^ 64);
}

template <int MT, int LA>
struct NtSchedule {
  static constexpr int NP = MT / 2;
  static constexpr int LB = 6;
  static_assert(MT % 2 == 0 && NP >= 4 && NP <= 5, "tile height");
  static_assert(LA >= 2 && LA <= 2 * NP - 2, "A lead");
  static constexpr int blead(int q) { return LB - q; }
  static constexpr int lookback = LA > LB ? LA : LB;
  static constexpr int phase_of(int P) { return ((P % NP) + NP) % NP; }
  static constexpr int tile_of(int P) { return (P - phase_of(P)) / NP; }
  static constexpr int prologue_requests() {
    int n = 0;
    for (int P = -lookback; P < 0; ++P) {
      ++n;
      for (int q = 0; q < 4; ++q) n += b_here(phase_of(P), q) ? 1 : 0;
    }
    return n;
  }
  static constexpr int a_part(int ph) { return (ph + LA) % NP; }
  static constexpr int a_tile(int ph) { return (ph + LA) / NP; }
  static constexpr bool b_here(int ph, int q) { return (ph + blead(q)) % NP == 0; }
  static constexpr int b_tile(int ph, int q) { return (ph + blead(q)) / NP; }
  static constexpr int wait(int ph, int E = 0) {
    int allowed = 0;
    for (int d = 0; d < 4 * NP; ++d) {
      const int f = ((ph - d) % NP + NP) % NP;
      for (int q = 3; q >= 0; --q)
        if (b_here(f, q)) {
          if (d + 1 >= blead(q)) return allowed + (d > ph ? E : 0);
          ++allowed;
        }
      if (d + 1 >= LA) return allowed + (d > ph ? E : 0);
      ++allowed;
    }
    return allowed;
  }
  template <class ReqA, class ReqB>
  static __device__ __forceinline__ void requests(int kt, int ph, ReqA request_a, ReqB request_b) {
    request_a(kt + a_tile(ph), a_part(ph));
#pragma unroll
    for (int q = 0; q < 4; ++q)
      if (b_here(ph, q)) request_b(kt + b_tile(ph, q), q);
  }
};

#define VITAMD_WAIT_VM(n) asm volatile("s_waitcnt vmcnt(%0)" ::"n"(n) : "memory")

template <int MT, bool MUL32>
__device__ __forceinline__ void pp_offsets(const GemmNtArgs& p, NtTile t, int wave, int lane, unsigned (&voffA)[MT / 2], unsigned (&voffB)[4]) {
  const int lr = 8 * wave + (lane >> 3);
  const unsigned chunk = (unsigned)(((lane & 7) ^ (lr & 7)) * 16);
#pragma unroll
  for (int j = 0; j < MT / 2; ++j) {
    unsigned o = (unsigned)min(t.m0 + (lr >> 5) * (16 * MT) + j * 32 + (lr & 31), p.M - 1) * (unsigned)(p.K * 2);
    if constexpr (MUL32) asm volatile("" : "+v"(o));
    voffA[j] = o + chunk;
  }
#pragma unroll
  for (int q = 0; q < 4; ++q) {
    unsigned o = (unsigned)min(t.n0 + 64 * q + lr, p.N - 1) * (unsigned)(p.K * 2);
    if constexpr (MUL32) asm volatile("" : "+v"(o));
    voffB[q] = o + chunk;
  }
}

template <int MT, int PART, class Request, class Wait>
__device__ __forceinline__ void pp_ktile(f32x4 (&acc)[MT][4], const char* pa0, const char* pa1, const char* pb0, const char* pb1, Request request, Wait wait) {
  bf16x8 bq[4][2], af[2][2];
#pragma unroll
  for (int ph = 0; ph < MT / 2; ++ph) {
    if (ph == 0) {
#pragma unroll
      for (int j = 0; j < 4; ++j) {
        bq[j][0] = *(const bf16x8*)(pb0 + j * 2048);
        bq[j][1] = *(const bf16x8*)(pb1 + j * 2048);
      }
    }
#pragma unroll
    for (int i = 0; i < 2; ++i) {
      af[i][0] = *(const bf16x8*)(pa0 + ph * PART + i * 2048);
      af[i][1] = *(const bf16x8*)(pa1 + ph * PART + i * 2048);
    }
    request(ph);
    wait(ph);
    __builtin_amdgcn_sched_barrier(0);
    __builtin_amdgcn_s_barrier();
    asm volatile("s_waitcnt lgkmcnt(0)" ::: "memory");
    __builtin_amdgcn_sched_barrier(0);
    __builtin_amdgcn_s_setprio(1);
#pragma unroll
    for (int ks = 0; ks < 2; ++ks)
#pragma unroll
      for (int i = 0; i < 2; ++i)
#pragma unroll
        for (int j = 0; j < 4; ++j)
          acc[2 * ph + i][j] = __builtin_amdgcn_mfma_f32_16x16x32_bf16(bq[j][ks], af[i][ks], acc[2 * ph + i][j], 0, 0, 0);
    __builtin_amdgcn_s_setprio(0);
    __builtin_amdgcn_sched_barrier(0);
    __builtin_amdgcn_s_barrier();
    asm volatile("" ::: "memory");
  }
}

template <class Kern>
int launch_tiles(Kern kern, const GemmNtArgs& p, hipStream_t stream, int BM, int threads, int lds, int max_wgs) {
  if (int e = set_lds(kern, lds)) return e;
  const int tiles = ((p.M + BM - 1) / BM) * ((p.N + 255) / 256);
  hipLaunchKernelGGL(kern, dim3(tiles > max_wgs ? max_wgs : tiles), dim3(threads), lds, stream, p);
  return hipGetLastError() == hipSuccess ? VITAMD_OK : VITAMD_ERR_LAUNCH;
}

}
```

### vit-is-all-you-need_amd/csrc/gemm_nt_seam.h

```cpp
#pragma once
#include "gemm_nt_pp.h"

namespace {

template <int EPI, int MT, bool TAB = false>
__global__ __launch_bounds__(512) void gemm_nt_seam_kernel(const GemmNtArgs p) {
  static_assert(EPI == EPI_BIAS_BF16 || EPI == EPI_GELU || EPI == EPI_DGELU || EPI == EPI_DGELU_NOCS, "epilogues without (or with up-front) auxiliary loads");
  static_assert(!TAB || (EPI == EPI_GELU && MT == 8), "the GELU table needs the 16 KiB that only the 256-row ring leaves");
  constexpr bool DG = EPI == EPI_DGELU || EPI == EPI_DGELU_NOCS;
  constexpr bool CS = EPI == EPI_DGELU;
  constexpr int LA = 4;
  using S = NtSchedule<MT, LA>;
  constexpr int NP = S::NP;
  constexpr int BM = 32 * MT, BN = 256, WN = 4, NT = 4;
  constexpr int PART = 8192, ASLOT = NP * PART, BSLOT = 32768, BBASE = 2 * ASLOT, OPS = BBASE + 2 * BSLOT;
  constexpr int STG = TAB ? 2048 : (160 * 1024 - OPS) / 8;
  constexpr int TABOFF = OPS + 8 * STG;
  constexpr int SL = STG / 2048;
  static_assert(SL >= 1 && MT % SL == 0, "staging");
  constexpr int E = EPI == EPI_GELU ? 4 * MT : CS ? 2 * MT + 1 : 2 * MT;
  static_assert(S::wait(NP - 1) + E <= 63 && S::wait(0, E) <= 63, "vmcnt is a 6-bit counter");

  extern __shared__ __attribute__((aligned(16))) char smem[];
  const int tid = threadIdx.x, lane = tid & 63;
  const int wave = __builtin_amdgcn_readfirstlane(tid >> 6);
  const int wm = wave / WN, wn = wave % WN;
  const int tiles_n = (p.N + BN - 1) / BN, tiles_m = (p.M + BM - 1) / BM;
  const int ntiles = tiles_m * tiles_n;
  const int K = p.K;
  const int nkt = K / 64;
  const srd_t srdA = make_srd(p.A, (size_t)p.M * K * 2);
  const srd_t srdB = make_srd(p.B, (size_t)p.N * K * 2);
  const srd_t rsO = make_srd(p.out, (size_t)p.M * p.ldo * 2);
  const srd_t rsO2 = make_srd(EPI == EPI_GELU ? p.out2 : p.out, (size_t)p.M * p.ldo * 2);
  const srd_t srdAux = make_srd(DG ? p.aux : p.out, (size_t)p.M * p.ldo * 2);
  const srd_t srdBias = make_srd(p.bias ? (const void*)p.bias : p.out, p.bias ? (size_t)p.N * 4 : 0);
  constexpr unsigned OOB = 0x80000000u;
  const unsigned lds0 = lds_addr(smem) + wave * 1024;

  unsigned voffA[NP], voffB[4];
  auto offsets = [&](const NtTile& t) {
    int l2 = (int)__builtin_amdgcn_mbcnt_hi(~0u, __builtin_amdgcn_mbcnt_lo(~0u, 0u));
    asm volatile("" : "+v"(l2));
    pp_offsets<MT, true>(p, t, wave, l2, voffA, voffB);
  };
  bool fill = true;
  auto request_a = [&](int kt, int j) {
    const bool live = fill && kt >= 0 && kt < nkt;
    asm_glds16(srdA, lds0 + ((kt + 8) & 1) * ASLOT + j * PART, live ? voffA[j] : OOB, live ? (unsigned)kt * 128u : 0u);
  };
  auto request_b = [&](int kt, int q) {
    const bool live = fill && kt >= 0 && kt < nkt;
    asm_glds16(srdB, lds0 + BBASE + ((kt + 8) & 1) * BSLOT + q * 8192, live ? voffB[q] : OOB, live ? (unsigned)kt * 128u : 0u);
  };
  auto prologue = [&]() {
#pragma unroll
    for (int P = -S::lookback; P < 0; ++P) S::requests(S::tile_of(P), S::phase_of(P), request_a, request_b);
  };

  const char *rdA[2], *rdB[2];
  frag_bases(smem + wm * 32 * 128, lane, rdA);
  frag_bases(smem + BBASE + wn * 64 * 128, lane, rdB);

  if constexpr (TAB) gelu_table_to_lds(p.gelu_tab, smem + TABOFF, tid);
  int ti = blockIdx.x;
  NtTile cur = nt_tile<BM>(ti, tiles_m, tiles_n);
  offsets(cur);
  prologue();
  VITAMD_WAIT_VM(S::wait(NP - 1));
  __builtin_amdgcn_s_barrier();
  asm volatile("" ::: "memory");
  if (wm == 1) __builtin_amdgcn_s_barrier();
  bool seam = false;

  for (;;) {
    f32x4 acc[MT][NT];
#pragma unroll
    for (int i = 0; i < MT; ++i)
#pragma unroll
      for (int j = 0; j < NT; ++j) acc[i][j] = (f32x4){0.f, 0.f, 0.f, 0.f};

    auto ktile = [&](int kt) {
      const bool lenient = seam && kt == 0;
      const int sa = (kt & 1) * ASLOT, sb = (kt & 1) * BSLOT;
      pp_ktile<MT, PART>(acc, rdA[0] + sa, rdA[1] + sa, rdB[0] + sb, rdB[1] + sb,
                         [&](int ph) { S::requests(kt, ph, request_a, request_b); },
                         [&](int ph) {
                           if (S::wait(ph, E) != S::wait(ph) && lenient) VITAMD_WAIT_VM(S::wait(ph, E));
                           else VITAMD_WAIT_VM(S::wait(ph));
                         });
    };
    for (int kt = 0; kt < nkt; ++kt) ktile(kt);
    if (wm == 0) __builtin_amdgcn_s_barrier();
    asm volatile("s_waitcnt vmcnt(0)" ::: "memory");

    int ln = (int)__builtin_amdgcn_mbcnt_hi(~0u, __builtin_amdgcn_mbcnt_lo(~0u, 0u));
    asm volatile("" : "+v"(ln));
    const int mloc = ln & 15, g = ln >> 4, rsub = ln >> 3, pc = ln & 7;
    char* const stg = smem + OPS + wave * STG;
    const int m0 = cur.m0, n0 = cur.n0;
    const int ncol = n0 + wn * 64 + 8 * (pc ^ rsub);
    const bool ncol_ok = ncol < p.N;
    const int mrow0 = m0 + wm * (16 * MT) + rsub;
    const unsigned obase = ncol_ok ? (unsigned)mrow0 * (unsigned)(p.ldo * 2) + (unsigned)ncol * 2u : OOB;
    const unsigned rstep = (unsigned)(p.ldo * 2) * 8u;
    u32x4 aux[DG ? 2 * MT : 1];
    u32x2 pk[DG ? MT : 1][NT];
    if constexpr (DG) {
#pragma unroll
      for (int i = 0; i < MT; ++i)
#pragma unroll
        for (int j = 0; j < NT; ++j) pk[i][j] = (u32x2){pack_bf16x2(acc[i][j][0], acc[i][j][1]), pack_bf16x2(acc[i][j][2], acc[i][j][3])};
#pragma unroll
      for (int it = 0; it < 2 * MT; ++it) {
// ... 32 lines not shown
    for (int c = 0; c < 8; ++c) cs[c] = 0.f;
#pragma unroll
    for (int rd = 0; rd < MT / SL; ++rd) {
#pragma unroll
      for (int s = 0; s < SL; ++s) {
        const int i = rd * SL + s;
#pragma unroll
        for (int j = 0; j < NT; ++j) {
          u32x2 o;
          if constexpr (DG) o = pk[i][j];
          else {
            const f32x4 v = acc[i][j] + bias4[j];
            o = (u32x2){pack_bf16x2(v[0], v[1]), pack_bf16x2(v[2], v[3])};
          }
          *(u32x2*)(stg + s * 2048 + mloc * 128 + (((2 * j + (g >> 1)) ^ (mloc & 7)) << 4) + (g & 1) * 8) = o;
        }
      }
#pragma unroll
      for (int s = 0; s < SL; ++s) {
        const int i = rd * SL + s;
#pragma unroll
        for (int h = 0; h < 2; ++h) {
          const u32x4 v = *(const u32x4*)(stg + s * 2048 + (rsub + 8 * h) * 128 + pc * 16);
          const unsigned voff = mrow0 + 16 * i + 8 * h < p.M ? obase : OOB;
          const unsigned soff = rstep * (unsigned)(2 * i + h);
          if constexpr (EPI == EPI_BIAS_BF16) {
            asm_bstore16_nt(v, rsO, voff, soff);
          } else if constexpr (EPI == EPI_GELU) {
            u32x4 a, d = v;
            if constexpr (TAB) gelu_lookup8(v, smem + TABOFF, p.gelu_dg != 0, a, d);
            else
#pragma unroll
            for (int c = 0; c < 4; ++c) {
              float dlo, dhi;
              a[c] = pack_bf16x2(gelu_fwd_grad(bf16lo(v[c]), dlo), gelu_fwd_grad(bf16hi(v[c]), dhi));
              if (p.gelu_dg) d[c] = pack_bf16x2(dlo, dhi);
            }
            asm_bstore16_nt(d, rsO, voff, soff);
            asm_bstore16_nt(a, rsO2, voff, soff);
          } else {
            const u32x4 pz = aux[2 * i + h];
            u32x4 o;
#pragma unroll
            for (int c = 0; c < 4; ++c) {
              const float lo = round_bf16(bf16lo(v[c]) * bf16lo(pz[c]));
              const float hi = round_bf16(bf16hi(v[c]) * bf16hi(pz[c]));
              if constexpr (CS) { if (voff != OOB) { cs[2 * c] += lo; cs[2 * c + 1] += hi; } }
              o[c] = pack_bf16x2(lo, hi);
            }
            asm_bstore16_nt(o, rsO, voff, soff);
          }
        }
      }
    }
    if constexpr (CS) {
#pragma unroll
      for (int bf = 1; bf < 8; bf <<= 1)
#pragma unroll
        for (int c = 0; c < 8; ++c) cs[c] += __shfl_xor(cs[c], 9 * bf, 64);
      float s = cs[0];
#pragma unroll
      for (int c = 1; c < 8; ++c) s = rsub == c ? cs[c] : s;
      atomicAdd(p.colsum + n0 + wn * 64 + 8 * (pc ^ rsub) + rsub, s);
    }
    if (!has_next) break;
    ti = ti_next;
    VITAMD_WAIT_VM(S::wait(NP - 1) + E);
    asm volatile("s_waitcnt lgkmcnt(0)" ::: "memory");
    __builtin_amdgcn_s_barrier();
    asm volatile("" ::: "memory");
    if (wm == 1) __builtin_amdgcn_s_barrier();
    seam = true;
  }
}

template <int EPI, int MT, bool TAB = false>
int launch_seam(const GemmNtArgs& p, hipStream_t stream, int cus) {
  if (TAB && !p.gelu_tab) return VITAMD_ERR_ARG;
  return launch_tiles(gemm_nt_seam_kernel<EPI, MT, TAB>, p, stream, 32 * MT, 512, 160 * 1024, cus);
}

static bool seam_ok(const GemmNtArgs& p) {
  if (p.K % 64 != 0 || p.K < 128 || p.N % 8 != 0 || p.ldo % 8 != 0) return false;
  if ((size_t)p.M * p.K * 2 >= 0xf0000000ull || (size_t)p.N * p.K * 2 >= 0xf0000000ull || (size_t)p.M * p.ldo * 2 >= 0x80000000ull) return false;
  if (p.epi == EPI_DGELU) return p.gelu_dg && p.N % 256 == 0 && p.aux != nullptr;
  if (p.epi == EPI_GELU) return p.out2 != nullptr;
  return p.epi == EPI_BIAS_BF16;
}

}
```

### vit-is-all-you-need_amd/csrc/vitamd_internal.h

```cpp
#pragma once
#include <hip/hip_runtime.h>

enum GemmEpilogue {
  EPI_BIAS_BF16 = 0,
  EPI_GELU = 1,
  EPI_RESID_F32 = 2,
  EPI_DGELU = 3,
  EPI_PATCH_F32 = 4,
  EPI_F32 = 5,
  EPI_DGELU_NOCS = 6,
};

enum NtTileCode {
  NT_TILE_AUTO = 0,
  NT_TILE_128 = 128,
  NT_TILE_256 = 256,
  NT_TILE_320 = 320,
  NT_TILE_AUTO_NO_PERSISTENT = 512,
  NT_TILE_AUTO_NO_SEAM = 1024,
  NT_TILE_LOADER = 2048,
  NT_TILE_SEAM = 4096,
};
inline bool is_auto(int tile) { return tile == NT_TILE_AUTO || tile == NT_TILE_AUTO_NO_PERSISTENT || tile == NT_TILE_AUTO_NO_SEAM; }

struct GemmNtArgs {
  const void* A;
  const void* B;
  void* out;
  void* out2;
  const float* bias;
  const void* aux;
  float* colsum;
  int M, N, K, ldo;
  int epi;
  int n_patches, seq, extra;
  int tile;
  unsigned drop_thresh;
  float drop_scale;
  unsigned drop_seed_lo, drop_seed_hi;
  int row0;
  int gelu_dg;
  const unsigned* gelu_tab;
};

struct GemmTnArgs {
  const void* L;
  const void* Rm;
  float* out;
  int R, P, Q, ldl, ldr, ldo;
  int splits;
  float* ws;
  size_t ws_bytes;
  int accumulate;
  int form;
  float* colsum;
};

struct DropoutParams {
  unsigned thresh;
  float scale;
  unsigned seed_lo, seed_hi;
  bool ok;
};
inline DropoutParams dropout_params(float p, unsigned long long seed) {
  DropoutParams d{0u, 1.0f, (unsigned)seed, (unsigned)(seed >> 32), p >= 0.f && p < 1.f};
  if (!d.ok) return d;
  d.thresh = p > 0.f ? (unsigned)((double)p * 4294967296.0) : 0u;
  if (p > 0.f && d.thresh == 0u) d.thresh = 1u;
  d.scale = 1.0f / (1.0f - p);
  return d;
}

int vitamd_gemm_nt_impl(const GemmNtArgs& p, hipStream_t stream);
int vitamd_gemm_nt_plan_impl(const GemmNtArgs& p);
int vitamd_init_impl(int device, hipStream_t stream);
const unsigned* vitamd_gelu_table();
int vitamd_gemm_tn_impl(const GemmTnArgs& p, hipStream_t stream);
```

### vit-is-all-you-need_amd/vitamd/functions.py

```python
from __future__ import annotations

import weakref

import torch

from . import ops
from .data import Frames

BF16, F32 = torch.bfloat16, torch.float32

_amp_fwd = torch.amp.custom_fwd(device_type="cuda", cast_inputs=torch.float32)
_amp_bwd = torch.amp.custom_bwd(device_type="cuda")


class WeightCache:

    def __init__(self):
        self._c = {}
        self._groups = {}
        self.epoch = 0

    def clear(self):
        self.epoch += 1

# ... 85 lines not shown
def _tn_splits(dW, R=None):
    target = tn_target_wgs()
    if not target or not SIDE.enabled:
        return 0
    ntile = ((dW.shape[0] + 255) // 256) * ((dW.shape[1] + 255) // 256)
    splits = max(1, round(target / ntile))
    if R is not None:
        splits = min(splits, max(1, (R + 63) // 64))
    return splits


def tn_target_wgs():
    if TN_TARGET_WGS is not None:
        return TN_TARGET_WGS
    return 252 if ops.NT_PERSISTENT else 128


DEFER_RESID = True

KEEP_ROWS = True


def keep_rows(keep, N, causal, p_attn, p_mlp):
    if keep is None or not KEEP_ROWS or keep >= N or causal or p_attn > 0 or p_mlp > 0:
        return None
    return int(keep)


def streams_overlap(device, side=None):
    device = torch.device(device)
    side = side if side is not None else SIDE.stream(device)
    R, P = 16384, 512
    l = torch.ones(R, P, device=device, dtype=torch.bfloat16)
    o1, o2 = torch.empty(P, P, device=device), torch.empty(P, P, device=device)
    cur = torch.cuda.current_stream(device)

    def run(both):
        cur.synchronize(); side.synchronize()
        a, b = torch.cuda.Event(enable_timing=True), torch.cuda.Event(enable_timing=True)
        a.record(cur)
        if both:
            side.wait_stream(cur)
            with torch.cuda.stream(side):
                for _ in range(3):
                    ops.gemm_tn(l, l, o2, accumulate=False, splits=1)
        for _ in range(3):
            ops.gemm_tn(l, l, o1, accumulate=False, splits=1)
        if both:
            cur.wait_stream(side)
        b.record(cur)
        b.synchronize()
        return a.elapsed_time(b)

    run(True)
    one = min(run(False) for _ in range(2))
    two = min(run(True) for _ in range(2))
    return two / max(one, 1e-6)


def ensure_side_overlap(device, attempts=6):
    device = _indexed(device)
    ratio = streams_overlap(device)
    kept = []
    while ratio > 1.5 and attempts > 0:
        kept.append(SIDE._streams[device])
        SIDE._streams[device] = torch.cuda.Stream(device=device)
        ratio = streams_overlap(device)
        attempts -= 1
    return ratio


def _f32c(t):
    return t.detach().to(F32).contiguous()


def new_seed():
    return int(torch.randint(0, 2 ** 62, (1,)).item())


def _keep_native(N, keep):
    return ops.attention_keep_forms(N, keep) == (ops.KEEP_FWD | ops.KEEP_BWD)


def layer_forward(x0, wqkv, bqkv, w1, b1, w2, b2, B, N, H, causal, need_grad, p_attn=0.0, p_mlp=0.0, pending=None, defer=False, keep=None):
    drop = (p_attn, new_seed() if p_attn > 0 else 0, p_mlp, new_seed() if p_mlp > 0 else 0)
    wqkv_b, _ = WEIGHTS.get(wqkv, need_grad)
    w1_b, _ = WEIGHTS.get(w1, need_grad)
    w2_b, _ = WEIGHTS.get(w2, need_grad)
    x0, a, mean1, rstd1 = ops.layernorm_fwd(x0, addend=pending)
    qkv = ops.gemm_nt(a, wqkv_b, ops.EPI_BIAS_BF16, bias=bqkv)
    if keep is not None:
        if causal or p_attn > 0 or p_mlp > 0 or defer or not 0 < keep < N:
            raise ops._lib.VitamdError("layer_forward: keep needs a non-causal layer without dropout, defer=False and 0 < keep < N")
        if _keep_native(N, keep):
            o, lse = ops.attention_fwd_keep(qkv, B, N, H, keep)
            o_k = o
        else:
            o, lse = ops.attention_fwd(qkv, B, N, H)
            o_k = o.view(B, N, -1)[:, :keep].reshape(B * keep, -1).contiguous()
        x1, bln, mean2, rstd2 = ops.layernorm_fwd_keep(x0, o_k, B, N, keep)
        pre, h = ops.gemm_nt(bln, w1_b, ops.EPI_GELU_DG, bias=b1)
        x2 = ops.gemm_nt(h, w2_b, ops.EPI_RESID_F32, bias=b2, aux=x1)
        saved = (x0, mean1, rstd1, a, qkv, o, lse, x1, mean2, rstd2, bln, pre, h) if need_grad else None
        return x2, saved, drop
    o, lse = ops.attention_fwd(qkv, B, N, H, causal, dropout=drop[:2])
    x1, bln, mean2, rstd2 = ops.layernorm_fwd(x0, addend=o)
    pre, h = ops.gemm_nt(bln, w1_b, ops.EPI_GELU_DG, bias=b1)
    y = None
    if p_mlp > 0:
        x2 = ops.linear_dropout_resid(h, w2_b, b2, x1, drop[2:])
    elif defer:
        x2, y = x1, ops.gemm_nt(h, w2_b, ops.EPI_BIAS_BF16, bias=b2)
    else:
        x2 = ops.gemm_nt(h, w2_b, ops.EPI_RESID_F32, bias=b2, aux=x1)
    saved = (x0, mean1, rstd1, a, qkv, o, lse, x1, mean2, rstd2, bln, pre, h) if need_grad else None
    return (x2, y) if defer else x2, saved, drop


def _indexed(device):
    device = torch.device(device)
    if device.type == "cuda" and device.index is None:
        device = torch.device("cuda", torch.cuda.current_device())
    return device


class _Side:

    def __init__(self):
        self._streams = {}
        self.enabled = True

    def stream(self, device):
        device = _indexed(device)
        s = self._streams.get(device)
        if s is None:
            s = self._streams[device] = torch.cuda.Stream(device=device)
        return s


SIDE = _Side()


def claim_streams(device):
    device = _indexed(device)
    with torch.cuda.stream(SIDE.stream(device)):
        torch.zeros(16, device=device).add_(1)
    torch.cuda.current_stream(device).synchronize()


class GradSink:
    _sinks = []

    @classmethod
    def register(cls, sink):
        cls._sinks = [r for r in cls._sinks if r() is not None and r() is not sink]
        cls._sinks.append(weakref.ref(sink))

    @classmethod
    def find(cls, params):
        if params is None:
            return None
        for r in cls._sinks:
            s = r()
            if s is not None and s.owns(params):
                return s
        return None


def layer_sizes(D):
    return (3 * D * D, 3 * D, 4 * D * D, 4 * D, 4 * D * D, D), ((3 * D, D), (3 * D,), (4 * D, D), (4 * D,), (D, 4 * D), (D,))


def grad_arena(D, n_layers, device, params=None):
    sizes, shapes = layer_sizes(D)
    sink = GradSink.find(params)
    if sink is not None:
        got = sink.arena_for(params, n_layers)
        if got is not None:
            return got, sink
    per_w, per_b = sum(sizes[0::2]), sum(sizes[1::2])
    flat_w = torch.empty(per_w * n_layers, dtype=F32, device=device)
    flat_b = torch.zeros(per_b * n_layers, dtype=F32, device=device)
    out = []
    for i in range(n_layers):
        ow, ob, views = i * per_w, i * per_b, []
        for j, (n, sh) in enumerate(zip(sizes, shapes)):
            if j % 2 == 0:
                views.append(flat_w[ow: ow + n].view(sh))
                ow += n
            else:
                views.append(flat_b[ob: ob + n].view(sh))
                ob += n
        out.append(tuple(views))
    return out, None


BIAS_FROM_WGRAD = True

BIAS_QKV_FROM_WGRAD = True

KEEP_WGRAD_SIDE = True


def layer_backward(g2, saved, wqkv, w1, w2, B, N, H, causal, grads, dy2=None, have_db2=False, emit_bf16=False,
                   emit_colsum=None, drop=(0.0, 0, 0.0, 0), emit_dropout=(0.0, 0), keep=None):
    x0, mean1, rstd1, a, qkv, o, lse, x1, mean2, rstd2, bln, pre, h = saved
    dWqkv, dbqkv, dW1, db1, dW2, db2 = grads
    main = torch.cuda.current_stream()
    side = SIDE.stream(g2.device) if SIDE.enabled else main

    def on_side(fn, *tensors):
        if side is main:
            fn()
            return
        ev = torch.cuda.Event()
        ev.record(main)
        side.wait_event(ev)
        with torch.cuda.stream(side):
            fn()
        _SIDE_KEEP.extend(tensors)

    R_mlp = g2.shape[0] if keep is not None else None
    on_side_mlp = on_side if keep is None or KEEP_WGRAD_SIDE else (lambda fn, *tensors: fn())
    _, wqkv_t = WEIGHTS.get(wqkv, True)
    _, w1_t = WEIGHTS.get(w1, True)
    _, w2_t = WEIGHTS.get(w2, True)
    if dy2 is None:
        dy2 = ops.cast_bf16_dropout(g2, drop[2:]) if drop[2] > 0 else ops.cast_bf16(g2)
    from_wgrad = BIAS_FROM_WGRAD
    if from_wgrad:
        emit_colsum = None

    def wgrad_fc2():
        ops.gemm_tn(dy2, h, dW2, accumulate=False, splits=_tn_splits(dW2, R_mlp), form=_tn_form("fc2"), colsum=db2 if from_wgrad else None)
        if not from_wgrad and not have_db2:
            ops.colsum(dy2, db2)
    on_side_mlp(wgrad_fc2, dy2, h, dW2, db2)
    dpre = ops.gemm_nt(dy2, w2_t, ops.EPI_DMUL, aux=pre, colsum=None if from_wgrad else db1)
    on_side_mlp(lambda: ops.gemm_tn(dpre, bln, dW1, accumulate=False, splits=_tn_splits(dW1, R_mlp), form=_tn_form("fc1"),
                                    colsum=db1 if from_wgrad else None), dpre, bln, dW1, db1)
    dbln = ops.gemm_nt(dpre, w1_t, ops.EPI_BIAS_BF16)
    g1, d_o = ops.layernorm_bwd(dbln, x1, mean2, rstd2, g_res=g2, want_bf16=True, xhat=bln)
    qkv_from_wgrad = BIAS_QKV_FROM_WGRAD
    dbias = None if qkv_from_wgrad else dbqkv
    if keep is None:
        dqkv = ops.attention_bwd(qkv, o, lse, d_o, B, N, H, causal, dbias=dbias, dropout=drop[:2])
    elif _keep_native(N, keep):
        dqkv = ops.attention_bwd_keep(qkv, o, lse, d_o, B, N, H, keep, dbias=dbias)
    else:
        d_o_full = torch.zeros((B, N, d_o.shape[1]), dtype=BF16, device=d_o.device)
        d_o_full[:, :keep] = d_o.view(B, keep, -1)
        dqkv = ops.attention_bwd(qkv, o, lse, d_o_full.view(B * N, -1), B, N, H, causal, dbias=dbias)
    on_side(lambda: ops.gemm_tn(dqkv, a, dWqkv, accumulate=False, splits=_tn_splits(dWqkv), form=_tn_form("qkv"),
                                colsum=dbqkv if qkv_from_wgrad else None), dqkv, a, dWqkv, dbqkv)
    da = ops.gemm_nt(dqkv, wqkv_t, ops.EPI_BIAS_BF16)
    g0, g0b = ops.layernorm_bwd(da, x0, mean1, rstd1, g_res=g1, want_bf16=emit_bf16, colsum=emit_colsum, dropout=emit_dropout,
                                xhat=a, keep=None if keep is None else (N, keep))
    return g0, g0b


_SIDE_KEEP = []
_SIDE_DONE = []


def side_checkpoint(device):
    if not SIDE.enabled:
        _SIDE_KEEP.clear()
        return
    ev = torch.cuda.Event()
    ev.record(SIDE.stream(device))
    _SIDE_DONE.append((ev, list(_SIDE_KEEP)))
    _SIDE_KEEP.clear()
    while len(_SIDE_DONE) > 1:
        old_ev, _ = _SIDE_DONE.pop(0)
        torch.cuda.current_stream().wait_event(old_ev)


def join_side(device):
    if SIDE.enabled:
        ev = torch.cuda.Event()
        ev.record(SIDE.stream(device))
        torch.cuda.current_stream().wait_event(ev)
    _SIDE_KEEP.clear()
    _SIDE_DONE.clear()


class TransformerLayerFn(torch.autograd.Function):
    @staticmethod
    @_amp_fwd
    def forward(ctx, x, wqkv, bqkv, w1, b1, w2, b2, n_heads, causal, p_attn=0.0, p_mlp=0.0):
        B, N, D = x.shape
        need_grad = any(ctx.needs_input_grad)
        x2, saved, drop = layer_forward(_f32c(x).view(B * N, D), wqkv, _f32c(bqkv), w1, _f32c(b1), w2, _f32c(b2), B, N, n_heads,
                                        causal, need_grad, p_attn, p_mlp)
        if need_grad:
            ctx.save_for_backward(*saved)
            ctx.weights = (wqkv, w1, w2)
        ctx.drop = drop
        ctx.meta = (B, N, D, n_heads, causal, x.dtype)
        return x2.view(B, N, D).to(x.dtype)

    @staticmethod
    @_amp_bwd
    def backward(ctx, g):
        B, N, D, H, causal, xdtype = ctx.meta
        wqkv, w1, w2 = ctx.weights
        (grads,), _ = grad_arena(D, 1, g.device)
        g0, _ = layer_backward(_f32c(g).view(B * N, D), ctx.saved_tensors, wqkv, w1, w2, B, N, H, causal, grads, drop=ctx.drop)
        join_side(g.device)
        return (g0.view(B, N, D).to(xdtype), *grads, None, None, None, None)


class TransformerStackFn(torch.autograd.Function):

    @staticmethod
    @_amp_fwd
    def forward(ctx, x, n_heads, causal, p_attn, p_mlp, keep, *params):
        B, N, D = x.shape
        L = len(params) // 6
        if keep is not None and keep <= 0:
            raise ValueError(f"keep must be a positive number of tokens, got {keep}")
        k_last = keep_rows(keep, N, causal, p_attn, p_mlp)
        need_grad = any(ctx.needs_input_grad)
        cur = _f32c(x).view(B * N, D)
        saved_all, drops = [], []
        WEIGHTS.prepare([params[6 * i + j] for i in range(L) for j in (0, 2, 4)], need_grad)
        pending = None
        for i in range(L):
            wqkv, bqkv, w1, b1, w2, b2 = params[6 * i: 6 * i + 6]
# ... 202 lines not shown
```

### vit-is-all-you-need_amd/vitamd/lib.py

```python
from __future__ import annotations

import ctypes
import os
import subprocess

_HERE = os.path.dirname(os.path.abspath(__file__))
LIB_PATH = os.path.join(_HERE, "libvitamd.so")
CSRC = os.path.join(os.path.dirname(_HERE), "csrc")
ABI_VERSION = 9

_c = ctypes
_P, _I, _F, _L, _U64, _D, _LL = _c.c_void_p, _c.c_int, _c.c_float, _c.c_long, _c.c_ulonglong, _c.c_double, _c.c_longlong

SIGNATURES = {
    "vitamd_abi_version": [],
    "vitamd_init": [_I, _P],
    "vitamd_gemm_nt_plan": [_I, _I, _I, _I, _I, _I],
    "vitamd_gemm_nt_bf16": [_P, _P, _P, _P, _P, _P, _P, _I, _I, _I, _I, _I, _I, _I, _I, _I, _P],
    "vitamd_gemm_tn_bf16": [_P, _P, _P, _I, _I, _I, _I, _I, _I, _I, _P],
    "vitamd_gemm_tn_bf16_ws": [_P, _P, _P, _I, _I, _I, _I, _I, _I, _I, _P, _L, _I, _I, _P],
    "vitamd_gemm_tn_bf16_ws_colsum": [_P, _P, _P, _P, _I, _I, _I, _I, _I, _I, _I, _P, _L, _I, _I, _P],
    "vitamd_gemm_tn_ws_bytes": [_I, _I, _I, _I],
    "vitamd_layernorm_fwd": [_P, _P, _P, _P, _P, _P, _I, _I, _F, _P],
    "vitamd_layernorm_bwd": [_P, _P, _P, _P, _P, _P, _P, _P, _I, _I, _P],
    "vitamd_layernorm_affine_fwd": [_P, _P, _P, _P, _P, _P, _I, _I, _F, _P],
    "vitamd_layernorm_affine_bwd": [_P, _P, _P, _P, _P, _P, _P, _P, _P, _P, _P, _I, _I, _P],
    "vitamd_layernorm_affine_fwd_f32": [_P, _P, _P, _P, _P, _P, _I, _I, _F, _P],
    "vitamd_layernorm_affine_bwd_f32": [_P, _P, _P, _P, _P, _P, _P, _P, _I, _I, _P],
    "vitamd_attention_fwd": [_P, _P, _P, _I, _I, _I, _I, _I, _F, _U64, _P],
    "vitamd_attention_fwd_resid": [_P, _P, _P, _P, _P, _I, _I, _I, _I, _I, _F, _U64, _P],
    "vitamd_attention_bwd": [_P, _P, _P, _P, _P, _P, _P, _I, _I, _I, _I, _I, _F, _U64, _P],
    "vitamd_layernorm_bwd_dropout": [_P, _P, _P, _P, _P, _P, _P, _P, _I, _I, _F, _U64, _P],
    "vitamd_layernorm_bwd_xhat": [_P, _P, _P, _P, _P, _P, _P, _I, _I, _F, _U64, _P],
    "vitamd_linear_dropout_resid_bf16": [_P, _P, _P, _P, _P, _I, _I, _I, _F, _U64, _I, _P],
    "vitamd_cast_f32_bf16_dropout": [_P, _P, _L, _F, _U64, _P],
    "vitamd_cast_f32_bf16": [_P, _P, _L, _P],
    "vitamd_dropout_bf16": [_P, _P, _L, _L, _F, _U64, _P],
    "vitamd_dropout_f32": [_P, _P, _L, _L, _F, _U64, _P],
    "vitamd_cast_transpose_weight": [_P, _P, _P, _I, _I, _P],
    "vitamd_cast_transpose_batched": [_P, _I, _I, _P],
    "vitamd_im2col_bf16": [_P, _P, _I, _I, _I, _I, _I, _P],
    "vitamd_colsum_bf16": [_P, _P, _I, _I, _I, _P],
    "vitamd_embed_bwd": [_P, _P, _P, _P, _P, _P, _I, _I, _I, _I, _P],
    "vitamd_vq_nearest": [_P, _P, _P, _I, _I, _I, _P],
    "vitamd_conv3x3_fwd": [_P, _P, _P, _P, _I, _I, _I, _I, _I, _P],
    "vitamd_conv3x3_bwd": [_P, _P, _P, _P, _P, _P, _I, _I, _I, _I, _I, _P],
    "vitamd_adamw_step": [_P, _P, _P, _P, _L, _F, _F, _F, _F, _F, _I, _P],
    "vitamd_adamw_step_d": [_P, _P, _P, _P, _L, _F, _D, _D, _F, _F, _I, _P],
    "vitamd_mt_row_bytes": [],
    "vitamd_mt_chunk_elems": [],
    "vitamd_mt_grid_cap": [],
    "vitamd_mt_sumsq": [_P, _P, _I, _I, _P, _P, _F, _P],
    "vitamd_mt_adamw": [_P, _P, _I, _I, _P, _P],
    "vitamd_mt_scale": [_P, _P, _I, _I, _P, _P],
    "vitamd_sched_row_bytes": [],
    "vitamd_sched_advance": [_P, _P, _I, _P],
    "vitamd_kv_append": [_P, _P, _P, _P, _I, _I, _I, _I, _I, _P],
    "vitamd_decode_attention_ws_bytes": [_I, _I, _I],
    "vitamd_decode_attention": [_P, _P, _P, _P, _P, _I, _I, _I, _I, _P, _L, _P],
    "vitamd_gemm_skinny_ws_bytes": [_I, _I, _I],
    "vitamd_gemm_skinny_bf16": [_P, _P, _P, _P, _P, _P, _I, _I, _I, _I, _P, _L, _P],
    "vitamd_gemm_skinny_qkv_append": [_P, _P, _P, _P, _P, _P, _P, _I, _I, _I, _I, _I, _P, _L, _P],
    "vitamd_decode_embed": [_P, _P, _P, _P, _P, _I, _I, _I, _I, _P],
    "vitamd_sample_logits": [_P, _P, _P, _P, _P, _I, _I, _I, _F, _I, _F, _U64, _P],
    "vitamd_layernorm_fwd_keep": [_P, _P, _P, _P, _P, _P, _I, _I, _I, _I, _F, _P],
    "vitamd_layernorm_bwd_keep": [_P, _P, _P, _P, _P, _P, _P, _P, _I, _I, _I, _I, _I, _F, _U64, _P],
    "vitamd_attention_keep_forms": [_I, _I],
    "vitamd_attention_fwd_keep": [_P, _P, _P, _I, _I, _I, _I, _I, _P],
    "vitamd_attention_bwd_keep": [_P, _P, _P, _P, _P, _P, _P, _I, _I, _I, _I, _I, _P],
    "vitamd_attention_form": [_I, _I, _F, _I, _I, _I],
    "vitamd_cross_entropy_grid_rows": [_I],
    "vitamd_cross_entropy_fwd": [_P, _I, _P, _P, _P, _P, _I, _I, _I, _LL, _P],
    "vitamd_cross_entropy_bwd": [_P, _I, _P, _P, _P, _P, _P, _I, _I, _I, _I, _I, _LL, _P],
    "vitamd_soft_cross_entropy_fwd": [_P, _I, _P, _P, _P, _F, _P, _P, _P, _I, _I, _I, _P],
    "vitamd_soft_cross_entropy_bwd": [_P, _I, _P, _P, _P, _F, _P, _P, _P, _P, _I, _I, _I, _I, _I, _P],
    "vitamd_embed_tokens_fwd": [_P, _P, _P, _P, _I, _I, _I, _I, _I, _P],
    "vitamd_embed_tokens_bwd": [_P, _P, _P, _P, _I, _I, _I, _I, _P],
    "vitamd_assemble_tokens_grid_cap": [],
    "vitamd_assemble_tokens_fwd": [_P, _P, _P, _P, _P, _P, _I, _I, _I, _I, _I, _I, _P],
    "vitamd_assemble_tokens_bwd": [_P, _P, _P, _P, _P, _I, _I, _I, _I, _I, _I, _P],
    "vitamd_vq_quantize_ws_bytes": [_I, _I, _I],
    "vitamd_vq_quantize_fwd": [_P, _P, _P, _P, _P, _P, _P, _P, _I, _I, _I, _P],
    "vitamd_vq_quantize_bwd": [_P, _P, _P, _P, _P, _P, _P, _P, _I, _I, _I, _P],
    "vitamd_recon_mse_ws_bytes": [_I, _I, _I, _I, _I],
    "vitamd_recon_mse_fwd": [_P, _I, _P, _P, _P, _I, _I, _I, _I, _I, _P],
    "vitamd_recon_mse_bwd": [_P, _I, _P, _P, _P, _I, _I, _I, _I, _I, _I, _P],
    "vitamd_vq_quantize_unit_fwd": [_P, _P, _P, _P, _P, _P, _P, _P, _I, _I, _I, _P],
    "vitamd_vq_quantize_unit_bwd": [_P, _P, _P, _P, _P, _P, _P, _P, _I, _I, _I, _P],
    "vitamd_conv_recon_mse_ws_bytes": [_I, _I, _I, _I, _I],
    "vitamd_conv_recon_mse_fwd": [_P, _I, _P, _P, _P, _P, _P, _P, _I, _I, _I, _I, _P],
    "vitamd_conv_recon_mse_bwd": [_P, _I, _P, _P, _P, _P, _P, _P, _P, _P, _P, _I, _I, _I, _I, _I, _P],
    "vitamd_dwconv7_fwd": [_P, _I, _P, _P, _P, _I, _I, _I, _I, _P],
    "vitamd_dwconv7_bwd": [_P, _I, _P, _P, _P, _I, _I, _I, _I, _P],
    "vitamd_resize_norm_fwd": [_P, _P, _P, _I, _P, _P, _I, _P, _P, _P, _P, _I, _I, _I, _I, _I, _P],
    "vitamd_resize_norm_bwd": [_P, _I, _P, _P, _I, _P, _P, _I, _P, _P, _I, _I, _I, _I, _I, _P],
    "vitamd_frames_prep": [_P, _P, _P, _P, _P, _P, _I, _I, _I, _I, _I, _I, _I, _I, _P],
    "vitamd_frames_prep_mix": [_P, _P, _P, _P, _P, _P, _I, _I, _I, _I, _I, _I, _I, _I, _P, _P, _P],
    "vitamd_frames_prep_resize": [_P, _P, _P, _P, _P, _P, _P, _I, _I, _I, _I, _I, _I, _I, _I, _P],
    "vitamd_frames_prep_resize_grid_cap": [],
    "vitamd_frames_prep_grid_cap": [],
    "vitamd_crop_flip_draw": [_P, _I, _I, _I, _I, _I, _I, _U64, _U64, _P],
    "vitamd_frames_to_u8": [_P, _P, _I, _I, _I, _I, _P],
    "vitamd_tanh_bf16": [_P, _P, _L, _P],
    "vitamd_tanh_bwd_bf16": [_P, _P, _P, _L, _P],
    "vitamd_recon_l1_fwd": [_P, _I, _P, _P, _P, _P, _L, _I, _I, _I, _I, _I, _P],
    "vitamd_recon_l1_bwd": [_P, _I, _P, _P, _P, _P, _I, _I, _I, _I, _I, _I, _P],
}

ERRORS = {1: "unsupported shape", 2: "bad argument", 3: "HIP launch failure", 4: "vitamd_init has not run for this device"}

_lib = None


class VitamdError(RuntimeError):
    pass


def build(verbose: bool = False) -> str:
    r = subprocess.run(["make", "-C", CSRC, "-j8"], capture_output=True, text=True)
    if verbose or r.returncode != 0:
        print(r.stdout[-4000:], r.stderr[-4000:])
    if r.returncode != 0:
        raise VitamdError("building libvitamd.so failed")
    return LIB_PATH


def hip_runtimes(maps_path="/proc/self/maps"):
    found = set()
    with open(maps_path) as fh:
        for line in fh:
            parts = line.split(None, 5)
            if len(parts) == 6 and "libamdhip64" in os.path.basename(parts[5].strip()):
                found.add(os.path.realpath(parts[5].strip()))
    return sorted(found)


def check_single_hip_runtime(maps_path="/proc/self/maps"):
    found = hip_runtimes(maps_path)
    if len(found) > 1 and os.environ.get("VITAMD_ALLOW_TWO_HIP_RUNTIMES") != "1":
        raise VitamdError("two HIP runtimes are mapped into this process: " + " and ".join(found) + " - libvitamd.so must resolve libamdhip64 to "
                          "the runtime that owns the caller's streams and pointers (import torch / load the framework BEFORE dlopen-ing libvitamd.so)")
    return found


def load():
    global _lib
    if _lib is not None:
        return _lib
    if not os.path.exists(LIB_PATH):
        raise VitamdError(f"{LIB_PATH} is missing: run `python -c 'import __graft_entry__ as g; g.build()'` "
                          "(the HIP kernels are the only implementation of this path; there is no fallback)")
    import torch
# ... 16 lines not shown
```

### vit-is-all-you-need_amd/vitamd/ops.py

```python
from __future__ import annotations

import torch

from . import lib as _lib

EPI_BIAS_BF16, EPI_GELU, EPI_RESID_F32, EPI_DGELU, EPI_PATCH_F32, EPI_F32, EPI_GELU_DG, EPI_DMUL = range(8)
import os as _os
NT_PERSISTENT = _os.environ.get("VITAMD_NT_PERSISTENT", "1") != "0"
_seam_env = _os.environ.get("VITAMD_NT_SEAM", "auto")
NT_SEAM = {"1": True, "0": False}.get(_seam_env)
SEAM_PROBE = {}
NT_FORM_SEAM, NT_FORM_LOADER = 4, 5
_RAW_AUTO = -1
LN_EPS = 1e-5
BF16, F32 = torch.bfloat16, torch.float32


def _L():
    return _lib.load()


_INITIALISED = set()


def init(device=None):
    device = torch.device("cuda", torch.cuda.current_device()) if device is None else torch.device(device)
    idx = device.index if device.index is not None else torch.cuda.current_device()
    if idx in _INITIALISED:
        return
    if torch.cuda.is_current_stream_capturing():
        raise _lib.VitamdError("vitamd.ops.init: first use of a device inside a stream capture; run one eager step (or ops.init(device)) before capturing")
    _lib.check(_L().vitamd_init(idx, torch.cuda.current_stream(device).cuda_stream), f"vitamd_init[device {idx}]")
    _INITIALISED.add(idx)


def _stream():
    return torch.cuda.current_stream().cuda_stream


def _p(t):
    return None if t is None else t.data_ptr()


def _need(t, dtype, name, ndim=None):
    if not isinstance(t, torch.Tensor) or not t.is_cuda:
        raise _lib.VitamdError(f"{name}: expected a ROCm device tensor (the HIP kernels are the only implementation)")
    if t.dtype != dtype:
        raise _lib.VitamdError(f"{name}: expected {dtype}, got {t.dtype}")
    if not t.is_contiguous():
        raise _lib.VitamdError(f"{name}: must be contiguous")
    if ndim is not None and t.dim() != ndim:
        raise _lib.VitamdError(f"{name}: expected {ndim}-d, got {t.dim()}-d")
    return t


def gemm_nt(a, b, epi, *, bias=None, aux=None, out=None, out2=None, colsum=None, n_patches=0, seq=0, extra=0,
            out_rows=None, tile=0):
    _need(a, BF16, "a", 2); _need(b, BF16, "b", 2)
    M, K = a.shape
    N, K2 = b.shape
    if K != K2:
        raise _lib.VitamdError(f"gemm_nt: K mismatch {K} vs {K2}")
    out_dtype = F32 if epi in (EPI_RESID_F32, EPI_PATCH_F32, EPI_F32) else BF16
    if out is None:
        out = torch.empty((out_rows if out_rows is not None else M, N), dtype=out_dtype, device=a.device)
    _need(out, out_dtype, "out")
    if epi in (EPI_GELU, EPI_GELU_DG) and out2 is None:
        out2 = torch.empty((M, N), dtype=BF16, device=a.device)
    if bias is not None:
        _need(bias, F32, "bias", 1)
    if epi in (EPI_GELU, EPI_GELU_DG):
        init(a.device)
    if tile == 0:
        tile = auto_tile(a.device, M, N, K, epi)
    elif tile == _RAW_AUTO:
        tile = 0
    code = _L().vitamd_gemm_nt_bf16(_p(a), _p(b), _p(out), _p(out2), _p(bias), _p(aux), _p(colsum), M, N, K, N, epi,
                                    n_patches, seq, extra, tile, _stream())
    _lib.check(code, f"gemm_nt[M={M},N={N},K={K},epi={epi}]")
    return (out, out2) if epi in (EPI_GELU, EPI_GELU_DG) else out


def seam_enabled(device):
    if NT_SEAM is not None:
        return NT_SEAM
    idx = device.index if device.index is not None else torch.cuda.current_device()
    rec = SEAM_PROBE.get(idx)
    return None if rec is None else rec["enabled"]


def auto_tile(device, M, N, K, epi):
    if not NT_PERSISTENT:
        return 512
    on = seam_enabled(device)
    if on is None:
        if _L().vitamd_gemm_nt_plan(M, N, K, N, epi, 0) & 0x7f not in (NT_FORM_SEAM, NT_FORM_LOADER) or torch.cuda.is_current_stream_capturing():
            return 0
        on = seam_probe(device)
    return 0 if on else 1024


def seam_probe(device, rows=49152, reps=3):
    device = torch.device(device)
    if device.index is None:
        device = torch.device("cuda", torch.cuda.current_device())
    x = torch.randn(rows, 768, device=device).to(BF16)
    w = torch.randn(2304, 768, device=device).mul_(0.03).to(BF16)
    out = torch.empty((rows, 2304), dtype=BF16, device=device)
    times = {}
    for name, tile in (("seam_us", _RAW_AUTO), ("plain_us", 1024)):
        launch = lambda: gemm_nt(x, w, EPI_BIAS_BF16, out=out, tile=tile)
        launch()
        s, e = torch.cuda.Event(enable_timing=True), torch.cuda.Event(enable_timing=True)
        s.record()
        for _ in range(reps):
            launch()
        e.record()
        e.synchronize()
        times[name] = s.elapsed_time(e) / reps * 1e3
    on = times["seam_us"] <= 1.25 * times["plain_us"]
    SEAM_PROBE[device.index] = {"seam_us": round(times["seam_us"], 1), "plain_us": round(times["plain_us"], 1), "enabled": on}
    if not on:
        import warnings
        warnings.warn(f"vitamd: the seam form of the NT GEMM is slower than the plain persistent form on {device} "
                      f"({times['seam_us']:.0f} vs {times['plain_us']:.0f} us): switched off for this device")
    return on


_WORKSPACES = {}


def _workspace(device, nbytes):
    key = (device, torch.cuda.current_stream().cuda_stream)
    ws = _WORKSPACES.get(key)
    if ws is None or ws.numel() * 4 < nbytes:
        ws = _WORKSPACES[key] = torch.empty((nbytes + 3) // 4, dtype=F32, device=device)
    return ws


TN_FORM_SHARED, TN_FORM_EXCLUSIVE = 0, 1


def gemm_tn(l, r, out, splits=0, accumulate=True, atomic=False, form=TN_FORM_SHARED, colsum=None):
    _need(l, BF16, "l", 2); _need(r, BF16, "r", 2); _need(out, F32, "out", 2)
    R, P = l.shape
    R2, Q = r.shape
    if R != R2 or tuple(out.shape) != (P, Q):
        raise _lib.VitamdError("gemm_tn: shape mismatch")
    if colsum is not None:
        _need(colsum, F32, "colsum", 1)
        if colsum.numel() != P:
            raise _lib.VitamdError("gemm_tn: colsum must be fp32 [P]")
    if atomic:
        if not accumulate:
            raise _lib.VitamdError("gemm_tn: the atomic form can only accumulate")
        if colsum is not None:
            raise _lib.VitamdError("gemm_tn: the atomic form has no reduce pass to sum colsum in")
        code = _L().vitamd_gemm_tn_bf16(_p(l), _p(r), _p(out), R, P, Q, P, Q, Q, splits, _stream())
    else:
        nbytes = _L().vitamd_gemm_tn_ws_bytes(R, P, Q, splits)
        ws = _workspace(l.device, nbytes)
        if colsum is not None:
            code = _L().vitamd_gemm_tn_bf16_ws_colsum(_p(l), _p(r), _p(out), _p(colsum), R, P, Q, P, Q, Q, splits, _p(ws), ws.numel() * 4,
                                                      int(accumulate), int(form), _stream())
        else:
            code = _L().vitamd_gemm_tn_bf16_ws(_p(l), _p(r), _p(out), R, P, Q, P, Q, Q, splits, _p(ws), ws.numel() * 4, int(accumulate),
                                               int(form), _stream())
    _lib.check(code, f"gemm_tn[R={R},P={P},Q={Q}]")
    return out


def layernorm_fwd(x, addend=None):
    _need(x, F32, "x", 2)
    M, D = x.shape
    y = torch.empty((M, D), dtype=BF16, device=x.device)
    mean = torch.empty((M,), dtype=F32, device=x.device)
    rstd = torch.empty((M,), dtype=F32, device=x.device)
    x_out = None
    if addend is not None:
        _need(addend, BF16, "addend", 2)
        x_out = torch.empty_like(x)
    code = _L().vitamd_layernorm_fwd(_p(x), _p(addend), _p(x_out), _p(y), _p(mean), _p(rstd), M, D, LN_EPS, _stream())
    _lib.check(code, f"layernorm_fwd[M={M},D={D}]")
    return (x_out if addend is not None else x), y, mean, rstd


def layernorm_fwd_keep(x, addend, B, seq, keep):
    _need(x, F32, "x", 2); _need(addend, BF16, "addend", 2)
    D = x.shape[1]
    if x.shape[0] != B * seq or tuple(addend.shape) != (B * keep, D) or not 0 < keep <= seq:
        raise _lib.VitamdError(f"layernorm_fwd_keep: x must be [B*seq, D], addend [B*keep, D], 0 < keep <= seq (B={B}, seq={seq}, keep={keep})")
    Mk = B * keep
    x_out = torch.empty((Mk, D), dtype=F32, device=x.device)
    y = torch.empty((Mk, D), dtype=BF16, device=x.device)
    mean = torch.empty((Mk,), dtype=F32, device=x.device)
    rstd = torch.empty((Mk,), dtype=F32, device=x.device)
    _lib.check(_L().vitamd_layernorm_fwd_keep(_p(x), _p(addend), _p(x_out), _p(y), _p(mean), _p(rstd), B, seq, keep, D, LN_EPS, _stream()),
               f"layernorm_fwd_keep[B={B},seq={seq},keep={keep},D={D}]")
    return x_out, y, mean, rstd


def layernorm_bwd(dy, x, mean, rstd, g_res=None, want_bf16=False, colsum=None, dropout=(0.0, 0), xhat=None, keep=None):
    _need(dy, BF16, "dy", 2); _need(x, F32, "x", 2)
    M, D = x.shape
    g = torch.empty_like(x)
    gb = torch.empty((M, D), dtype=BF16, device=x.device) if want_bf16 else None
    if g_res is not None:
        _need(g_res, F32, "g_res", 2)
    if keep is not None:
        seq, k = keep
        if g_res is None or M % seq or not 0 < k <= seq or tuple(g_res.shape) != (M // seq * k, D):
            raise _lib.VitamdError(f"layernorm_bwd: keep=({seq}, {k}) needs M % seq == 0 and g_res fp32 [M/seq*k, D]")
        use_xhat = xhat is not None and D in (256, 512, 768, 1024)
        if use_xhat:
            _need(xhat, BF16, "xhat", 2)
        code = _L().vitamd_layernorm_bwd_keep(_p(dy), _p(xhat if use_xhat else x), _p(mean), _p(rstd), _p(g_res), _p(g), _p(gb), _p(colsum),
                                              M // seq, seq, k, D, int(use_xhat), float(dropout[0]), int(dropout[1]), _stream())
        _lib.check(code, f"layernorm_bwd_keep[M={M},D={D},seq={seq},keep={k}]")
        return g, gb
    if xhat is not None and D in (256, 512, 768, 1024):
        _need(xhat, BF16, "xhat", 2)
        code = _L().vitamd_layernorm_bwd_xhat(_p(dy), _p(xhat), _p(rstd), _p(g_res), _p(g), _p(gb), _p(colsum), M, D,
                                              float(dropout[0]), int(dropout[1]), _stream())
        _lib.check(code, f"layernorm_bwd_xhat[M={M},D={D}]")
        return g, gb
    code = _L().vitamd_layernorm_bwd_dropout(_p(dy), _p(x), _p(mean), _p(rstd), _p(g_res), _p(g), _p(gb), _p(colsum), M, D,
                                             float(dropout[0]), int(dropout[1]), _stream())
    _lib.check(code, f"layernorm_bwd[M={M},D={D}]")
    return g, gb


def layernorm_affine_fwd(x, gamma, beta, eps=LN_EPS):
    _need(x, F32, "x", 2); _need(gamma, F32, "gamma", 1); _need(beta, F32, "beta", 1)
    M, D = x.shape
    y = torch.empty((M, D), dtype=BF16, device=x.device)
    mean = torch.empty((M,), dtype=F32, device=x.device)
    rstd = torch.empty((M,), dtype=F32, device=x.device)
    _lib.check(_L().vitamd_layernorm_affine_fwd(_p(x), _p(gamma), _p(beta), _p(y), _p(mean), _p(rstd), M, D, float(eps), _stream()),
               "layernorm_affine_fwd")
    return y, mean, rstd


def layernorm_affine_bwd(dy, x, mean, rstd, gamma, dgamma, dbeta, g_res=None, want_bf16=False, colsum=None):
    _need(dy, BF16, "dy", 2); _need(x, F32, "x", 2); _need(gamma, F32, "gamma", 1)
    _need(dgamma, F32, "dgamma", 1); _need(dbeta, F32, "dbeta", 1)
    M, D = x.shape
    g = torch.empty_like(x)
    gb = torch.empty((M, D), dtype=BF16, device=x.device) if want_bf16 else None
    _lib.check(_L().vitamd_layernorm_affine_bwd(_p(dy), _p(x), _p(mean), _p(rstd), _p(gamma), _p(g_res), _p(g), _p(gb), _p(colsum),
                                                _p(dgamma), _p(dbeta), M, D, _stream()), "layernorm_affine_bwd")
    return g, gb

# ... 9 lines not shown
    return y, mean, rstd


def layernorm_affine_bwd_f32(dy, x, mean, rstd, gamma, dgamma, dbeta):
    _need(dy, F32, "dy", 2); _need(x, F32, "x", 2); _need(gamma, F32, "gamma", 1)
    _need(dgamma, F32, "dgamma", 1); _need(dbeta, F32, "dbeta", 1)
    M, D = x.shape
    g = torch.empty_like(x)
    _lib.check(_L().vitamd_layernorm_affine_bwd_f32(_p(dy), _p(x), _p(mean), _p(rstd), _p(gamma), _p(g), _p(dgamma), _p(dbeta), M, D,
                                                    _stream()), "layernorm_affine_bwd_f32")
    return g


ATTN_RESID_MAX_N = 256


def attention_fwd(qkv, B, N, H, causal=False, dropout=(0.0, 0), resid=None):
    _need(qkv, BF16, "qkv", 2)
    D = H * 64
    if tuple(qkv.shape) != (B * N, 3 * D):
        raise _lib.VitamdError("attention_fwd: qkv must be [B*N, 3*H*64] (head_dim 64 only)")
    o = torch.empty((B * N, D), dtype=BF16, device=qkv.device)
    lse = torch.empty((B, H, N), dtype=F32, device=qkv.device)
    if resid is not None:
        _need(resid, F32, "resid", 2)
        if tuple(resid.shape) != (B * N, D):
            raise _lib.VitamdError("attention_fwd: resid must be [B*N, H*64]")
        x1 = torch.empty_like(resid)
        code = _L().vitamd_attention_fwd_resid(_p(qkv), _p(o), _p(lse), _p(resid), _p(x1), B, N, H, 64, int(causal), float(dropout[0]),
                                               int(dropout[1]), _stream())
        _lib.check(code, f"attention_fwd_resid[B={B},N={N},H={H}]")
        return o, lse, x1
    code = _L().vitamd_attention_fwd(_p(qkv), _p(o), _p(lse), B, N, H, 64, int(causal), float(dropout[0]), int(dropout[1]), _stream())
    _lib.check(code, f"attention_fwd[B={B},N={N},H={H}]")
    return o, lse


def attention_bwd(qkv, o, lse, d_o, B, N, H, causal=False, dbias=None, dropout=(0.0, 0)):
    _need(qkv, BF16, "qkv", 2); _need(o, BF16, "o", 2); _need(d_o, BF16, "d_o", 2); _need(lse, F32, "lse")
    if dbias is not None:
        _need(dbias, F32, "dbias", 1)
    dqkv = torch.empty_like(qkv)
    delta = torch.empty_like(lse)
    code = _L().vitamd_attention_bwd(_p(qkv), _p(o), _p(lse), _p(d_o), _p(dqkv), _p(delta), _p(dbias), B, N, H, 64, int(causal),
                                     float(dropout[0]), int(dropout[1]), _stream())
    _lib.check(code, f"attention_bwd[B={B},N={N},H={H}]")
    return dqkv


ATTN_FWD_SMALL, ATTN_FWD_SMALL8, ATTN_FWD_LOOP, ATTN_FWD_LONG, ATTN_BWD_PIPE, ATTN_BWD_LOOP, ATTN_BWD_LONG = 1, 2, 3, 4, 5, 6, 7
ATTN_DROP, ATTN_CAUSAL, ATTN_RES, ATTN_KEEP = 0x1000, 0x2000, 0x4000, 0x8000


def attention_form(N, causal=False, dropout_p=0.0, resid=False, nq=0, backward=False):
    code = int(_L().vitamd_attention_form(int(N), int(causal), float(dropout_p), int(bool(resid)), int(nq), int(backward)))
    if code < 0:
        raise _lib.VitamdError(f"attention_form[N={N},causal={int(causal)},p={dropout_p},resid={int(bool(resid))},nq={nq},backward={int(backward)}]: "
                               f"{_lib.ERRORS.get(-code, code)}")
    return code


def attention_form_fields(code):
    return code & 0xf, code >> 4 & 0xf, code >> 8 & 0xf, code & 0xf000


KEEP_FWD, KEEP_BWD = 1, 2


def attention_keep_forms(N, nq):
    return int(_L().vitamd_attention_keep_forms(int(N), int(nq)))


def attention_fwd_keep(qkv, B, N, H, nq):
    _need(qkv, BF16, "qkv", 2)
    D = H * 64
    if tuple(qkv.shape) != (B * N, 3 * D) or not 0 < nq <= N:
        raise _lib.VitamdError("attention_fwd_keep: qkv must be [B*N, 3*H*64] (head_dim 64 only) and 0 < nq <= N")
    o = torch.empty((B * nq, D), dtype=BF16, device=qkv.device)
    lse = torch.empty((B, H, N), dtype=F32, device=qkv.device)
    _lib.check(_L().vitamd_attention_fwd_keep(_p(qkv), _p(o), _p(lse), B, N, H, 64, nq, _stream()), f"attention_fwd_keep[B={B},N={N},H={H},nq={nq}]")
    return o, lse


def attention_bwd_keep(qkv, o, lse, d_o, B, N, H, nq, dbias=None, delta=None):
    _need(qkv, BF16, "qkv", 2); _need(o, BF16, "o", 2); _need(d_o, BF16, "d_o", 2); _need(lse, F32, "lse")
    D = H * 64
    if tuple(qkv.shape) != (B * N, 3 * D) or tuple(o.shape) != (B * nq, D) or tuple(d_o.shape) != (B * nq, D) or lse.numel() != B * H * N:
        raise _lib.VitamdError("attention_bwd_keep: qkv [B*N, 3*H*64], o and d_o compact [B*nq, H*64], lse [B, H, N]")
    if dbias is not None:
        _need(dbias, F32, "dbias", 1)
    dqkv = torch.empty_like(qkv)
    if delta is None:
        delta = torch.empty_like(lse)
    else:
        _need(delta, F32, "delta")
        if delta.numel() != B * H * N:
            raise _lib.VitamdError("attention_bwd_keep: delta must be [B, H, N]")
    _lib.check(_L().vitamd_attention_bwd_keep(_p(qkv), _p(o), _p(lse), _p(d_o), _p(dqkv), _p(delta), _p(dbias), B, N, H, 64, nq, _stream()),
               f"attention_bwd_keep[B={B},N={N},H={H},nq={nq}]")
    return dqkv


def linear_dropout_resid(a, b, bias, resid, dropout):
    _need(a, BF16, "a", 2); _need(b, BF16, "b", 2); _need(resid, F32, "resid", 2); _need(bias, F32, "bias", 1)
    M, K = a.shape
    N = b.shape[0]
    out = torch.empty((M, N), dtype=F32, device=a.device)
    code = _L().vitamd_linear_dropout_resid_bf16(_p(a), _p(b), _p(out), _p(bias), _p(resid), M, N, K, float(dropout[0]), int(dropout[1]),
                                                 0 if NT_PERSISTENT else 512, _stream())
    _lib.check(code, f"linear_dropout_resid[M={M},N={N},K={K}]")
    return out


def cast_bf16_dropout(x, dropout):
    _need(x, F32, "x")
    out = torch.empty(x.shape, dtype=BF16, device=x.device)
    _lib.check(_L().vitamd_cast_f32_bf16_dropout(_p(x), _p(out), x.numel(), float(dropout[0]), int(dropout[1]), _stream()), "cast_dropout")
    return out


def dropout(x, p, seed, group=1, inplace=False):
    if x.dtype not in (BF16, F32):
        raise _lib.VitamdError(f"dropout: expected bf16 or fp32, got {x.dtype}")
    _need(x, x.dtype, "x")
    out = x if inplace else torch.empty_like(x)
    fn = _L().vitamd_dropout_bf16 if x.dtype == BF16 else _L().vitamd_dropout_f32
    _lib.check(fn(_p(x), _p(out), x.numel(), int(group), float(p), int(seed), _stream()), "dropout")
    return out


def cast_bf16(x):
    _need(x, F32, "x")
    out = torch.empty(x.shape, dtype=BF16, device=x.device)
    _lib.check(_L().vitamd_cast_f32_bf16(_p(x), _p(out), x.numel(), _stream()), "cast_f32_bf16")
    return out


def cast_weight(w, want_plain=True, want_transposed=False):
    _need(w, F32, "w", 2)
    N, K = w.shape
    wb = torch.empty((N, K), dtype=BF16, device=w.device) if want_plain else None
    wbt = torch.empty((K, N), dtype=BF16, device=w.device) if want_transposed else None
    _lib.check(_L().vitamd_cast_transpose_weight(_p(w), _p(wb), _p(wbt), N, K, _stream()), "cast_transpose_weight")
    return wb, wbt


def im2col(img, p):
    _need(img, F32, "img", 4)
    B, C, H, W = img.shape
    out = torch.empty((B * (H // p) * (W // p), C * p * p), dtype=BF16, device=img.device)
    _lib.check(_L().vitamd_im2col_bf16(_p(img), _p(out), B, C, H, W, p, _stream()), "im2col")
    return out


def colsum(x, out=None):
    _need(x, BF16, "x", 2)
    M, N = x.shape
    if out is None:
        out = torch.zeros((N,), dtype=F32, device=x.device)
    _lib.check(_L().vitamd_colsum_bf16(_p(x), _p(out), M, N, N, _stream()), "colsum")
    return out


def embed_bwd(g, B, seq, extra, D):
    _need(g, F32, "g", 2)
    n_p = seq - extra
    dev = g.device
    dpos = torch.zeros((n_p, D), dtype=F32, device=dev)
    dextra = torch.zeros((extra, D), dtype=F32, device=dev)
    dyp = torch.empty((B * n_p, D), dtype=BF16, device=dev)
    dbias = torch.zeros((D,), dtype=F32, device=dev)
    rows = torch.zeros((max(n_p, 1), D), dtype=F32, device=dev)
    _lib.check(_L().vitamd_embed_bwd(_p(g), _p(dpos), _p(dextra) if extra > 0 else None, _p(dyp), _p(dbias), _p(rows), B, seq, extra, D,
                                     _stream()), "embed_bwd")
    return dpos, dextra, dyp, dbias


def vq_nearest(x, codebook):
    _need(x, F32, "x", 2); _need(codebook, F32, "codebook", 2)
    M, d = x.shape
    K, d2 = codebook.shape
# ... 818 lines not shown
```

Baseline: 9128 images/sec.

## Compute Q projection only for kept rows in last block and skip unused dQ rows

Adds a leading-dimension (lda) parameter to the NT GEMM and strided-output support so the QKV projection can be split. K/V are computed for all tokens while Q is computed only for the kept query rows, here just the CLS token in the final block, on a side stream. The keep-mode attention backward gains a kept_q_only flag that skips zero-filling and storing dQ for discarded query rows, and the TN GEMM gets strided inputs and an output row offset so weight gradients can be accumulated per slice. This removes redundant Q projection FLOPs and dQ writes in the last layer, at the cost of extra launches, stream synchronisation and more complex bookkeeping.

```diff
diff --git a/include/vitamd.h b/include/vitamd.h
--- a/include/vitamd.h
+++ b/include/vitamd.h
@@ -28,6 +28,10 @@
                         float* colsum, int M, int N, int K, int ldo, int epi, int n_patches, int seq, int extra,
                         int tile, void* stream);
 
+int vitamd_gemm_nt_bf16_ld(const void* A, const void* B, void* out, void* out2, const float* bias, const void* aux,
+                           float* colsum, int M, int N, int K, int lda, int ldo, int epi, int n_patches, int seq, int extra,
+                           int tile, void* stream);
+
 #define VITAMD_NT_FORM_SMALL 1
 #define VITAMD_NT_FORM_PP 2
 #define VITAMD_NT_FORM_PP_PERSISTENT 3
@@ -35,6 +39,7 @@
 #define VITAMD_NT_FORM_LOADER 5
 #define VITAMD_NT_FORM_TAIL_SPLIT 0x80
 int vitamd_gemm_nt_plan(int M, int N, int K, int ldo, int epi, int tile);
+int vitamd_gemm_nt_plan_ld(int M, int N, int K, int lda, int ldo, int epi, int tile);
 
 int vitamd_linear_dropout_resid_bf16(const void* A, const void* B, float* out, const float* bias, const float* resid,
                                      int M, int N, int K, float dropout_p, unsigned long long seed, int tile, void* stream);
@@ -87,6 +92,8 @@
 int vitamd_attention_fwd_keep(const void* qkv, void* o, float* lse2, int B, int N, int H, int head_dim, int nq, void* stream);
 int vitamd_attention_bwd_keep(const void* qkv, const void* o, const float* lse2, const void* d_o, void* dqkv, float* delta,
                               float* dbias, int B, int N, int H, int head_dim, int nq, void* stream);
+int vitamd_attention_bwd_keep_q(const void* qkv, const void* o, const float* lse2, const void* d_o, void* dqkv, float* delta,
+                                float* dbias, int B, int N, int H, int head_dim, int nq, int kept_q_only, void* stream);
 
 #define VITAMD_ATTN_FWD_SMALL 1
 #define VITAMD_ATTN_FWD_SMALL8 2
diff --git a/vit-is-all-you-need_amd/csrc/attention.hip b/vit-is-all-you-need_amd/csrc/attention.hip
--- a/vit-is-all-you-need_amd/csrc/attention.hip
+++ b/vit-is-all-you-need_amd/csrc/attention.hip
@@ -164,6 +164,7 @@
   const float* resid_in;
   float* resid_out;
   int nq;
+  int kept_q_only;
 };
 
 struct HeadAddr {
@@ -356,7 +357,7 @@
   bool active = qb < nt;
   if constexpr (KEEP) active = qb * 32 < a.nq;
   bf16x8 qf[4];
-  load_lane_frags(qbase, D3, N, (active ? qb : 0) * 32, lane, qf);
+  load_lane_frags(qbase, D3, KEEP ? a.nq : N, (active ? qb : 0) * 32, lane, qf);
   asm volatile("s_waitcnt vmcnt(0)" ::: "memory");
 #pragma unroll
   for (int kk = 0; kk < 4; ++kk) asm volatile("" : "+v"(qf[kk]));
@@ -523,6 +524,7 @@
     const int qrow = q0 + (lane & 31);
     if constexpr (LIM) {
       if (qb >= NQT) {
+        if (a.kept_q_only) continue;
         __bf16* zp = a.dqkv + (size_t)b * N * D3 + hh * DH + 8 * (lane & 7);
 #pragma unroll
         for (int it = 0; it < 4; ++it) {
@@ -536,7 +538,7 @@
     float delta = 0.f;
     {
       bf16x8 of[4];
-      load_lane_frags(qbase, D3, N, q0, lane, qf);
+      load_lane_frags(qbase, D3, nq, q0, lane, qf);
       load_lane_frags(dobase, D, nq, q0, lane, dof);
       load_lane_frags(obase, D, nq, q0, lane, of);
       if constexpr (LIM) {
@@ -612,7 +614,9 @@
         for (int dt = 0; dt < 2; ++dt) dq[dt] = __builtin_amdgcn_mfma_f32_32x32x16_bf16(ktr[sidx][dt], dsf, dq[dt], 0, 0, 0);
       }
     }
-    store_rows_T_img(a.dqkv + (size_t)b * N * D3 + hh * DH, D3, N, q0, lane, dq, a.scale, oimg, a.dbias ? &csum_q : nullptr);
+    int nstore = N;
+    if constexpr (LIM) nstore = a.kept_q_only ? nq : N;
+    store_rows_T_img(a.dqkv + (size_t)b * N * D3 + hh * DH, D3, nstore, q0, lane, dq, a.scale, oimg, a.dbias ? &csum_q : nullptr);
   }
   if (a.dbias) atomicAdd(a.dbias + hh * DH + lane, csum_q);
 }
@@ -721,7 +725,7 @@
   char* oimg = smem + 2 * npad * 128 + 2 * npad * 4 + wave * 4096;
   const __bf16* qbase = a.qkv + (size_t)b * N * D3 + hh * DH;
   const __bf16* dobase = a.d_o + (size_t)b * nq * D + hh * DH;
-  stage_tile(qbase, D3, N, npad, qtile, wave, lane);
+  stage_tile(qbase, D3, nq, npad, qtile, wave, lane);
   stage_tile(dobase, D, nq, npad, dotile, wave, lane);
   for (int i = threadIdx.x; i < npad; i += 256) {
     const size_t stat = ((size_t)b * a.H + hh) * N + min(i, nq - 1);
@@ -1296,12 +1300,21 @@
   return launched(launch_fwd(f, a, (hipStream_t)stream_));
 }
 
+extern "C" int vitamd_attention_bwd_keep_q(const void* qkv, const void* o, const float* lse2, const void* d_o, void* dqkv, float* delta,
+                                           float* dbias, int B, int N, int H, int head_dim, int nq, int kept_q_only, void* stream_);
+
 extern "C" int vitamd_attention_bwd_keep(const void* qkv, const void* o, const float* lse2, const void* d_o, void* dqkv, float* delta,
                                          float* dbias, int B, int N, int H, int head_dim, int nq, void* stream_) {
+  return vitamd_attention_bwd_keep_q(qkv, o, lse2, d_o, dqkv, delta, dbias, B, N, H, head_dim, nq, 0, stream_);
+}
+
+extern "C" int vitamd_attention_bwd_keep_q(const void* qkv, const void* o, const float* lse2, const void* d_o, void* dqkv, float* delta,
+                                           float* dbias, int B, int N, int H, int head_dim, int nq, int kept_q_only, void* stream_) {
   AttnArgs a;
   if (int e = make_args(a, true, qkv, o, lse2, d_o, dqkv, delta, dbias, B, N, H, head_dim, 0, 0.f, 0ull, nq)) return e;
   AttnForm f;
   if (nq <= 0) return VITAMD_ERR_SHAPE;
   if (int e = attention_form(f, N, false, false, false, nq, true)) return e;
+  a.kept_q_only = kept_q_only != 0;
   return launched(launch_bwd(f, a, (hipStream_t)stream_));
 }
diff --git a/vit-is-all-you-need_amd/csrc/capi.hip b/vit-is-all-you-need_amd/csrc/capi.hip
--- a/vit-is-all-you-need_amd/csrc/capi.hip
+++ b/vit-is-all-you-need_amd/csrc/capi.hip
@@ -6,24 +6,37 @@
 
 extern "C" int vitamd_init(int device, void* stream) { return vitamd_init_impl(device, (hipStream_t)stream); }
 
+static GemmNtArgs nt_args(const void* A, const void* B, void* out, void* out2, const float* bias, const void* aux, float* colsum, int M, int N, int K,
+                          int lda, int ldo, int epi, int n_patches, int seq, int extra, int tile, bool& ok) {
+  const int dg = (epi == 6 || epi == 7) ? 1 : 0;
+  if (epi == 6) epi = EPI_GELU;
+  if (epi == 7) epi = EPI_DGELU;
+  ok = is_auto(tile) || tile == NT_TILE_128 || tile == NT_TILE_256 || tile == NT_TILE_320 || tile == NT_TILE_LOADER || tile == NT_TILE_SEAM;
+  return GemmNtArgs{A, B, out, out2, bias, aux, colsum, M, N, K, ldo, epi, n_patches, seq, extra, tile, 0u, 1.0f, 0u, 0u, 0, dg, nullptr, lda};
+}
+
 extern "C" int vitamd_gemm_nt_bf16(const void* A, const void* B, void* out, void* out2, const float* bias, const void* aux,
                                    float* colsum, int M, int N, int K, int ldo, int epi, int n_patches, int seq, int extra,
                                    int tile, void* stream) {
-  const int dg = (epi == 6 || epi == 7) ? 1 : 0;
-  if (epi == 6) epi = EPI_GELU;
-  if (epi == 7) epi = EPI_DGELU;
-  GemmNtArgs p{A, B, out, out2, bias, aux, colsum, M, N, K, ldo, epi, n_patches, seq, extra, tile, 0u, 1.0f, 0u, 0u, 0, dg};
-  if (!is_auto(tile) && tile != NT_TILE_128 && tile != NT_TILE_256 && tile != NT_TILE_320 && tile != NT_TILE_LOADER && tile != NT_TILE_SEAM) return VITAMD_ERR_ARG;
+  return vitamd_gemm_nt_bf16_ld(A, B, out, out2, bias, aux, colsum, M, N, K, 0, ldo, epi, n_patches, seq, extra, tile, stream);
+}
+
+extern "C" int vitamd_gemm_nt_bf16_ld(const void* A, const void* B, void* out, void* out2, const float* bias, const void* aux,
+                                      float* colsum, int M, int N, int K, int lda, int ldo, int epi, int n_patches, int seq, int extra,
+                                      int tile, void* stream) {
+  bool ok;
+  const GemmNtArgs p = nt_args(A, B, out, out2, bias, aux, colsum, M, N, K, lda, ldo, epi, n_patches, seq, extra, tile, ok);
+  if (!ok || lda < 0) return VITAMD_ERR_ARG;
   return vitamd_gemm_nt_impl(p, (hipStream_t)stream);
 }
 
-extern "C" int vitamd_gemm_nt_plan(int M, int N, int K, int ldo, int epi, int tile) {
-  const int dg = (epi == 6 || epi == 7) ? 1 : 0;
-  if (epi == 6) epi = EPI_GELU;
-  if (epi == 7) epi = EPI_DGELU;
+extern "C" int vitamd_gemm_nt_plan(int M, int N, int K, int ldo, int epi, int tile) { return vitamd_gemm_nt_plan_ld(M, N, K, 0, ldo, epi, tile); }
+
+extern "C" int vitamd_gemm_nt_plan_ld(int M, int N, int K, int lda, int ldo, int epi, int tile) {
   static char dummy[16];
-  GemmNtArgs p{dummy, dummy, dummy, dummy, nullptr, dummy, (float*)dummy, M, N, K, ldo, epi, 1, 1, 0, tile, 0u, 1.0f, 0u, 0u, 0, dg};
-  if (!is_auto(tile) && tile != NT_TILE_128 && tile != NT_TILE_256 && tile != NT_TILE_320 && tile != NT_TILE_LOADER && tile != NT_TILE_SEAM) return -VITAMD_ERR_ARG;
+  bool ok;
+  const GemmNtArgs p = nt_args(dummy, dummy, dummy, dummy, nullptr, dummy, (float*)dummy, M, N, K, lda, ldo, epi, 1, 1, 0, tile, ok);
+  if (!ok || lda < 0) return -VITAMD_ERR_ARG;
   return vitamd_gemm_nt_plan_impl(p);
 }
 
diff --git a/vit-is-all-you-need_amd/csrc/gemm_nt.hip b/vit-is-all-you-need_amd/csrc/gemm_nt.hip
--- a/vit-is-all-you-need_amd/csrc/gemm_nt.hip
+++ b/vit-is-all-you-need_amd/csrc/gemm_nt.hip
@@ -43,7 +43,7 @@
     const int logical = (lane & 7) ^ (row & 7);
     if (piece < BM / 8) {
       const int g = min(m0 + row, p.M - 1);
-      src[i] = A + (size_t)g * K + logical * 8;
+      src[i] = A + (size_t)g * p.lda + logical * 8;
     } else {
       const int g = min(n0 + row - BM, p.N - 1);
       src[i] = B + (size_t)g * K + logical * 8;
@@ -114,7 +114,7 @@
   const int ntiles = tiles_m * tiles_n;
   const int K = p.K;
   const int nkt = K / 64;
-  const srd_t srdA = make_srd(p.A, (size_t)p.M * K * 2);
+  const srd_t srdA = make_srd(p.A, (size_t)p.M * p.lda * 2);
   const srd_t srdB = make_srd(p.B, (size_t)p.N * K * 2);
   for (int ti = blockIdx.x; ti < ntiles; ti += PERS ? (int)gridDim.x : ntiles) {
   const NtTile t = nt_tile<BM>(ti, tiles_m, tiles_n);
@@ -287,7 +287,7 @@
   const bool no_seam = tile == NT_TILE_AUTO_NO_SEAM;
   if (no_seam) tile = NT_TILE_AUTO;
   const long big_tiles = (long)((p.M + 255) / 256) * ((p.N + 255) / 256);
-  const bool pp_ok = (size_t)p.M * p.K * 2 < 0xf0000000ull && (size_t)p.N * p.K * 2 < 0xf0000000ull && p.K % 64 == 0;
+  const bool pp_ok = (size_t)p.M * p.lda * 2 < 0xf0000000ull && (size_t)p.N * p.K * 2 < 0xf0000000ull && p.K % 64 == 0;
   const bool big = p.N >= 256 && big_tiles >= 192 && pp_ok;
   const bool tall = tall_epi && prefer_tall(p);
   if (tile == NT_TILE_AUTO_NO_PERSISTENT) tile = NT_TILE_AUTO;
@@ -364,6 +364,7 @@
 
 static int check_args(const GemmNtArgs& p) {
   if (p.M <= 0 || p.N <= 0 || p.K <= 0 || p.K % 32 != 0 || p.N % 4 != 0 || p.ldo % 4 != 0) return VITAMD_ERR_SHAPE;
+  if (p.lda < p.K || p.lda % 8 != 0) return VITAMD_ERR_SHAPE;
   if (!p.A || !p.B || !p.out) return VITAMD_ERR_ARG;
   if (p.epi == EPI_GELU && !p.out2) return VITAMD_ERR_ARG;
   if ((p.epi == EPI_RESID_F32 || p.epi == EPI_DGELU) && !p.aux) return VITAMD_ERR_ARG;
@@ -379,7 +380,7 @@
 
 static int panel_rows(const GemmNtArgs& p) {
   if ((size_t)p.N * p.K * 2 >= NT_SPAN) return 0;
-  const size_t kb = (size_t)p.K * 2, ob = (size_t)p.ldo * out_esz(p), row_bytes = kb > ob ? kb : ob;
+  const size_t kb = (size_t)p.lda * 2, ob = (size_t)p.ldo * out_esz(p), row_bytes = kb > ob ? kb : ob;
   if ((size_t)p.M * row_bytes < NT_SPAN) return p.M;
   if (p.epi == EPI_PATCH_F32) return 0;
   return (int)((NT_SPAN - 1) / row_bytes / NT_PANEL_ROWS) * NT_PANEL_ROWS;
@@ -388,7 +389,7 @@
 static GemmNtArgs rows_of(const GemmNtArgs& p, int r0, int rows) {
   GemmNtArgs q = p;
   q.M = rows;
-  q.A = (const char*)p.A + (size_t)r0 * p.K * 2;
+  q.A = (const char*)p.A + (size_t)r0 * p.lda * 2;
   q.out = (char*)p.out + (size_t)r0 * p.ldo * out_esz(p);
   if (p.out2) q.out2 = (char*)p.out2 + (size_t)r0 * p.ldo * 2;
   if (p.aux && p.epi != EPI_PATCH_F32) q.aux = (const char*)p.aux + (size_t)r0 * p.ldo * (p.epi == EPI_RESID_F32 ? 4 : 2);
@@ -423,7 +424,14 @@
   return pl.form | (pl.rows << 8) | (rows_a ? 0x80 : 0);
 }
 
-int vitamd_gemm_nt_impl(const GemmNtArgs& p0, hipStream_t stream) {
+static GemmNtArgs with_lda(const GemmNtArgs& p0) {
+  GemmNtArgs p = p0;
+  if (p.lda == 0) p.lda = p.K;
+  return p;
+}
+
+int vitamd_gemm_nt_impl(const GemmNtArgs& p00, hipStream_t stream) {
+  const GemmNtArgs p0 = with_lda(p00);
   if (int e = check_args(p0)) return e;
   const int rows = panel_rows(p0);
   if (!rows) return VITAMD_ERR_SHAPE;
@@ -441,7 +449,8 @@
   return VITAMD_OK;
 }
 
-int vitamd_gemm_nt_plan_impl(const GemmNtArgs& p0) {
+int vitamd_gemm_nt_plan_impl(const GemmNtArgs& p00) {
+  const GemmNtArgs p0 = with_lda(p00);
   if (int e = check_args(p0)) return -e;
   const int rows = panel_rows(p0);
   if (!rows) return -VITAMD_ERR_SHAPE;
diff --git a/vit-is-all-you-need_amd/csrc/gemm_nt_ld.h b/vit-is-all-you-need_amd/csrc/gemm_nt_ld.h
--- a/vit-is-all-you-need_amd/csrc/gemm_nt_ld.h
+++ b/vit-is-all-you-need_amd/csrc/gemm_nt_ld.h
@@ -26,7 +26,7 @@
 
   if (wave >= 8) {
     const int l = wave - 8;
-    const srd_t srdA = make_srd(p.A, (size_t)p.M * K * 2);
+    const srd_t srdA = make_srd(p.A, (size_t)p.M * p.lda * 2);
     const srd_t srdB = make_srd(p.B, (size_t)p.N * K * 2);
     const srd_t srdBias = make_srd(p.bias ? (const void*)p.bias : p.out, p.bias ? (size_t)p.N * 4 : 0);
     const unsigned ldsA = lds_addr(smem) + l * 4096;
@@ -41,7 +41,7 @@
         for (int i = 0; i < 4; ++i) {
           const int a = 4 * l + i;
           const int row = min(t.m0 + (a >> 3) * 128 + h * 64 + (a & 7) * 8 + r8, p.M - 1);
-          voffA[h][i] = (unsigned)row * (unsigned)(K * 2) + chunk;
+          voffA[h][i] = (unsigned)row * (unsigned)(p.lda * 2) + chunk;
         }
 #pragma unroll
       for (int i = 0; i < 8; ++i) {
diff --git a/vit-is-all-you-need_amd/csrc/gemm_nt_pp.h b/vit-is-all-you-need_amd/csrc/gemm_nt_pp.h
--- a/vit-is-all-you-need_amd/csrc/gemm_nt_pp.h
+++ b/vit-is-all-you-need_amd/csrc/gemm_nt_pp.h
@@ -70,7 +70,7 @@
   const unsigned chunk = (unsigned)(((lane & 7) ^ (lr & 7)) * 16);
 #pragma unroll
   for (int j = 0; j < MT / 2; ++j) {
-    unsigned o = (unsigned)min(t.m0 + (lr >> 5) * (16 * MT) + j * 32 + (lr & 31), p.M - 1) * (unsigned)(p.K * 2);
+    unsigned o = (unsigned)min(t.m0 + (lr >> 5) * (16 * MT) + j * 32 + (lr & 31), p.M - 1) * (unsigned)(p.lda * 2);
     if constexpr (MUL32) asm volatile("" : "+v"(o));
     voffA[j] = o + chunk;
   }
diff --git a/vit-is-all-you-need_amd/csrc/gemm_nt_seam.h b/vit-is-all-you-need_amd/csrc/gemm_nt_seam.h
--- a/vit-is-all-you-need_amd/csrc/gemm_nt_seam.h
+++ b/vit-is-all-you-need_amd/csrc/gemm_nt_seam.h
@@ -29,7 +29,7 @@
   const int ntiles = tiles_m * tiles_n;
   const int K = p.K;
   const int nkt = K / 64;
-  const srd_t srdA = make_srd(p.A, (size_t)p.M * K * 2);
+  const srd_t srdA = make_srd(p.A, (size_t)p.M * p.lda * 2);
   const srd_t srdB = make_srd(p.B, (size_t)p.N * K * 2);
   const srd_t rsO = make_srd(p.out, (size_t)p.M * p.ldo * 2);
   const srd_t rsO2 = make_srd(EPI == EPI_GELU ? p.out2 : p.out, (size_t)p.M * p.ldo * 2);
@@ -228,7 +228,7 @@
 
 static bool seam_ok(const GemmNtArgs& p) {
   if (p.K % 64 != 0 || p.K < 128 || p.N % 8 != 0 || p.ldo % 8 != 0) return false;
-  if ((size_t)p.M * p.K * 2 >= 0xf0000000ull || (size_t)p.N * p.K * 2 >= 0xf0000000ull || (size_t)p.M * p.ldo * 2 >= 0x80000000ull) return false;
+  if ((size_t)p.M * p.lda * 2 >= 0xf0000000ull || (size_t)p.N * p.K * 2 >= 0xf0000000ull || (size_t)p.M * p.ldo * 2 >= 0x80000000ull) return false;
   if (p.epi == EPI_DGELU) return p.gelu_dg && p.N % 256 == 0 && p.aux != nullptr;
   if (p.epi == EPI_GELU) return p.out2 != nullptr;
   return p.epi == EPI_BIAS_BF16;
diff --git a/vit-is-all-you-need_amd/csrc/vitamd_internal.h b/vit-is-all-you-need_amd/csrc/vitamd_internal.h
--- a/vit-is-all-you-need_amd/csrc/vitamd_internal.h
+++ b/vit-is-all-you-need_amd/csrc/vitamd_internal.h
@@ -41,6 +41,7 @@
   int row0;
   int gelu_dg;
   const unsigned* gelu_tab;
+  int lda;
 };
 
 struct GemmTnArgs {
diff --git a/vit-is-all-you-need_amd/vitamd/functions.py b/vit-is-all-you-need_amd/vitamd/functions.py
--- a/vit-is-all-you-need_amd/vitamd/functions.py
+++ b/vit-is-all-you-need_amd/vitamd/functions.py
@@ -191,13 +191,53 @@
     return ops.attention_keep_forms(N, keep) == (ops.KEEP_FWD | ops.KEEP_BWD)
 
 
+KEEP_Q_ROWS = True
+
+
+def _kept_rows(t, B, N, keep):
+    v = t.view(B, N, -1)[:, :keep]
+    return v[:, 0] if keep == 1 else v.reshape(B * keep, -1)
+
+
+def _put_kept_rows(dst, src, B, N, keep, col0=0):
+    dst.view(B, N, -1)[:, :keep, col0: col0 + src.shape[1]] = src.view(B, keep, -1)
+
+
+def _kept_rows_out(t, B, N, keep, cols):
+    return t.view(B, -1)[:, :cols] if keep == 1 else None
+
+
+def _qkv_kept_q(a, wqkv_b, bqkv, B, N, keep):
+    D = a.shape[1]
+    main = torch.cuda.current_stream()
+    side = SIDE.stream(a.device) if SIDE.enabled else main
+    fork = torch.cuda.Event()
+    fork.record(main)
+    qkv = ops.gemm_nt(a, wqkv_b[D:], ops.EPI_BIAS_BF16, bias=bqkv[D:], out_cols=(D, 3 * D))
+    if side is not main:
+        side.wait_event(fork)
+    with torch.cuda.stream(side):
+        q_out = _kept_rows_out(qkv, B, N, keep, D)
+        q = ops.gemm_nt(_kept_rows(a, B, N, keep), wqkv_b[:D], ops.EPI_BIAS_BF16, bias=bqkv[:D], out=q_out)
+        if q_out is None:
+            _put_kept_rows(qkv, q, B, N, keep)
+    if side is not main:
+        done = torch.cuda.Event()
+        done.record(side)
+        main.wait_event(done)
+    return qkv
+
+
 def layer_forward(x0, wqkv, bqkv, w1, b1, w2, b2, B, N, H, causal, need_grad, p_attn=0.0, p_mlp=0.0, pending=None, defer=False, keep=None):
     drop = (p_attn, new_seed() if p_attn > 0 else 0, p_mlp, new_seed() if p_mlp > 0 else 0)
     wqkv_b, _ = WEIGHTS.get(wqkv, need_grad)
     w1_b, _ = WEIGHTS.get(w1, need_grad)
     w2_b, _ = WEIGHTS.get(w2, need_grad)
     x0, a, mean1, rstd1 = ops.layernorm_fwd(x0, addend=pending)
-    qkv = ops.gemm_nt(a, wqkv_b, ops.EPI_BIAS_BF16, bias=bqkv)
+    if keep is not None and KEEP_Q_ROWS and 0 < keep < N and _keep_native(N, keep):
+        qkv = _qkv_kept_q(a, wqkv_b, bqkv, B, N, keep)
+    else:
+        qkv = ops.gemm_nt(a, wqkv_b, ops.EPI_BIAS_BF16, bias=bqkv)
     if keep is not None:
         if causal or p_attn > 0 or p_mlp > 0 or defer or not 0 < keep < N:
             raise ops._lib.VitamdError("layer_forward: keep needs a non-causal layer without dropout, defer=False and 0 < keep < N")
@@ -354,6 +394,34 @@
     dbias = None if qkv_from_wgrad else dbqkv
     if keep is None:
         dqkv = ops.attention_bwd(qkv, o, lse, d_o, B, N, H, causal, dbias=dbias, dropout=drop[:2])
+    elif _keep_native(N, keep) and KEEP_Q_ROWS:
+        dqkv = ops.attention_bwd_keep(qkv, o, lse, d_o, B, N, H, keep, dbias=dbias, kept_q_only=True)
+        D = a.shape[1]
+        kept = {}
+        da_k = d_o
+
+        def dgrad_kept():
+            kept["dqkv"], kept["a"] = _kept_rows(dqkv, B, N, keep), _kept_rows(a, B, N, keep)
+            ops.gemm_nt(kept["dqkv"], wqkv_t, ops.EPI_BIAS_BF16, out=da_k)
+            kept["done"] = torch.cuda.Event()
+            kept["done"].record(side)
+        on_side(dgrad_kept, dqkv, a, da_k)
+        full = ((dWqkv.shape[0] + 255) // 256) * ((dWqkv.shape[1] + 255) // 256)
+        splits = _tn_splits(dWqkv) or (1 if full >= 256 else 256 // full)
+        colsum = dbqkv if qkv_from_wgrad else None
+
+        def wgrad_qkv():
+            ops.gemm_tn(dqkv[:, D:], a, dWqkv, accumulate=False, splits=splits, form=_tn_form("qkv"), colsum=colsum, out_row0=D)
+            ops.gemm_tn(kept["dqkv"][:, :D], kept["a"], dWqkv, accumulate=False, splits=_tn_splits(dWqkv[:D], g2.shape[0]), form=_tn_form("qkv"),
+                        colsum=colsum, out_row0=0)
+        on_side(wgrad_qkv, dqkv, a, dWqkv, dbqkv)
+        da = ops.gemm_nt(dqkv[:, D:], wqkv_t[:, D:].contiguous(), ops.EPI_BIAS_BF16)
+        if side is not main:
+            main.wait_event(kept["done"])
+        _put_kept_rows(da, da_k, B, N, keep)
+        g0, g0b = ops.layernorm_bwd(da, x0, mean1, rstd1, g_res=g1, want_bf16=emit_bf16, colsum=emit_colsum, dropout=emit_dropout,
+                                    xhat=a, keep=(N, keep))
+        return g0, g0b
     elif _keep_native(N, keep):
         dqkv = ops.attention_bwd_keep(qkv, o, lse, d_o, B, N, H, keep, dbias=dbias)
     else:
diff --git a/vit-is-all-you-need_amd/vitamd/lib.py b/vit-is-all-you-need_amd/vitamd/lib.py
--- a/vit-is-all-you-need_amd/vitamd/lib.py
+++ b/vit-is-all-you-need_amd/vitamd/lib.py
@@ -17,6 +17,8 @@
     "vitamd_init": [_I, _P],
     "vitamd_gemm_nt_plan": [_I, _I, _I, _I, _I, _I],
     "vitamd_gemm_nt_bf16": [_P, _P, _P, _P, _P, _P, _P, _I, _I, _I, _I, _I, _I, _I, _I, _I, _P],
+    "vitamd_gemm_nt_plan_ld": [_I, _I, _I, _I, _I, _I, _I],
+    "vitamd_gemm_nt_bf16_ld": [_P, _P, _P, _P, _P, _P, _P, _I, _I, _I, _I, _I, _I, _I, _I, _I, _I, _P],
     "vitamd_gemm_tn_bf16": [_P, _P, _P, _I, _I, _I, _I, _I, _I, _I, _P],
     "vitamd_gemm_tn_bf16_ws": [_P, _P, _P, _I, _I, _I, _I, _I, _I, _I, _P, _L, _I, _I, _P],
     "vitamd_gemm_tn_bf16_ws_colsum": [_P, _P, _P, _P, _I, _I, _I, _I, _I, _I, _I, _P, _L, _I, _I, _P],
@@ -68,6 +70,7 @@
     "vitamd_attention_keep_forms": [_I, _I],
     "vitamd_attention_fwd_keep": [_P, _P, _P, _I, _I, _I, _I, _I, _P],
     "vitamd_attention_bwd_keep": [_P, _P, _P, _P, _P, _P, _P, _I, _I, _I, _I, _I, _P],
+    "vitamd_attention_bwd_keep_q": [_P, _P, _P, _P, _P, _P, _P, _I, _I, _I, _I, _I, _I, _P],
     "vitamd_attention_form": [_I, _I, _F, _I, _I, _I],
     "vitamd_cross_entropy_grid_rows": [_I],
     "vitamd_cross_entropy_fwd": [_P, _I, _P, _P, _P, _P, _I, _I, _I, _LL, _P],
diff --git a/vit-is-all-you-need_amd/vitamd/ops.py b/vit-is-all-you-need_amd/vitamd/ops.py
--- a/vit-is-all-you-need_amd/vitamd/ops.py
+++ b/vit-is-all-you-need_amd/vitamd/ops.py
@@ -55,16 +55,16 @@
 
 
 def gemm_nt(a, b, epi, *, bias=None, aux=None, out=None, out2=None, colsum=None, n_patches=0, seq=0, extra=0,
-            out_rows=None, tile=0):
-    _need(a, BF16, "a", 2); _need(b, BF16, "b", 2)
+            out_rows=None, tile=0, out_cols=None):
+    lda = _need_rows(a, BF16, "a"); _need(b, BF16, "b", 2)
     M, K = a.shape
     N, K2 = b.shape
     if K != K2:
         raise _lib.VitamdError(f"gemm_nt: K mismatch {K} vs {K2}")
     out_dtype = F32 if epi in (EPI_RESID_F32, EPI_PATCH_F32, EPI_F32) else BF16
     if out is None:
-        out = torch.empty((out_rows if out_rows is not None else M, N), dtype=out_dtype, device=a.device)
-    _need(out, out_dtype, "out")
+        out = torch.empty((out_rows if out_rows is not None else M, N if out_cols is None else out_cols[1]), dtype=out_dtype, device=a.device)
+    dst, ldo = _nt_out(out, out_dtype, M, N, out_cols, out2, aux, epi)
     if epi in (EPI_GELU, EPI_GELU_DG) and out2 is None:
         out2 = torch.empty((M, N), dtype=BF16, device=a.device)
     if bias is not None:
@@ -75,8 +75,8 @@
         tile = auto_tile(a.device, M, N, K, epi)
     elif tile == _RAW_AUTO:
         tile = 0
-    code = _L().vitamd_gemm_nt_bf16(_p(a), _p(b), _p(out), _p(out2), _p(bias), _p(aux), _p(colsum), M, N, K, N, epi,
-                                    n_patches, seq, extra, tile, _stream())
+    code = _L().vitamd_gemm_nt_bf16_ld(_p(a), _p(b), _p(dst), _p(out2), _p(bias), _p(aux), _p(colsum), M, N, K, lda if lda != K else 0, ldo, epi,
+                                       n_patches, seq, extra, tile, _stream())
     _lib.check(code, f"gemm_nt[M={M},N={N},K={K},epi={epi}]")
     return (out, out2) if epi in (EPI_GELU, EPI_GELU_DG) else out
 
@@ -127,6 +127,39 @@
     return on
 
 
+def _need_rows(t, dtype, name):
+    if not isinstance(t, torch.Tensor) or not t.is_cuda:
+        raise _lib.VitamdError(f"{name}: expected a ROCm device tensor (the HIP kernels are the only implementation)")
+    if t.dtype != dtype:
+        raise _lib.VitamdError(f"{name}: expected {dtype}, got {t.dtype}")
+    if t.dim() != 2:
+        raise _lib.VitamdError(f"{name}: expected 2-d, got {t.dim()}-d")
+    if t.is_contiguous() or t.shape[0] == 1:
+        return t.shape[1]
+    if t.stride(1) != 1 or t.stride(0) < t.shape[1]:
+        raise _lib.VitamdError(f"{name}: rows must be contiguous and must not overlap (strides {tuple(t.stride())})")
+    return t.stride(0)
+
+
+def _nt_out(out, out_dtype, M, N, out_cols, out2, aux, epi):
+    if out_cols is not None:
+        _need(out, out_dtype, "out", 2)
+        col0, width = out_cols
+        if out.shape[0] != M or out.shape[1] != width or not 0 <= col0 <= width - N:
+            raise _lib.VitamdError(f"gemm_nt: out_cols={out_cols} needs out [M, {width}] and col0 + N <= width")
+        out = out[:, col0: col0 + N]
+    if out.dim() == 2 and tuple(out.shape) == (M, N) and not out.is_contiguous():
+        ldo = _need_rows(out, out_dtype, "out")
+    else:
+        _need(out, out_dtype, "out")
+        ldo = N
+    if ldo != N and epi != EPI_PATCH_F32:
+        for t, name in ((out2, "out2"), (aux, "aux")):
+            if t is not None and (t.dim() != 2 or t.stride(1) != 1 or t.stride(0) != ldo):
+                raise _lib.VitamdError(f"gemm_nt: {name} must have the row stride of out ({ldo})")
+    return out, ldo
+
+
 _WORKSPACES = {}
 
 
@@ -141,10 +174,18 @@
 TN_FORM_SHARED, TN_FORM_EXCLUSIVE = 0, 1
 
 
-def gemm_tn(l, r, out, splits=0, accumulate=True, atomic=False, form=TN_FORM_SHARED, colsum=None):
-    _need(l, BF16, "l", 2); _need(r, BF16, "r", 2); _need(out, F32, "out", 2)
+def gemm_tn(l, r, out, splits=0, accumulate=True, atomic=False, form=TN_FORM_SHARED, colsum=None, out_row0=None):
+    ldl, ldr = _need_rows(l, BF16, "l"), _need_rows(r, BF16, "r")
+    _need(out, F32, "out", 2)
     R, P = l.shape
     R2, Q = r.shape
+    if out_row0 is not None:
+        if not 0 <= out_row0 <= out.shape[0] - P or (colsum is not None and colsum.numel() != out.shape[0]):
+            raise _lib.VitamdError("gemm_tn: out_row0 needs out [P_all, Q] and colsum [P_all] with out_row0 + P <= P_all")
+        out_all, out = out, out[out_row0: out_row0 + P]
+        if colsum is not None:
+            _need(colsum, F32, "colsum", 1)
+            colsum = colsum[out_row0: out_row0 + P]
     if R != R2 or tuple(out.shape) != (P, Q):
         raise _lib.VitamdError("gemm_tn: shape mismatch")
     if colsum is not None:
@@ -156,18 +197,18 @@
             raise _lib.VitamdError("gemm_tn: the atomic form can only accumulate")
         if colsum is not None:
             raise _lib.VitamdError("gemm_tn: the atomic form has no reduce pass to sum colsum in")
-        code = _L().vitamd_gemm_tn_bf16(_p(l), _p(r), _p(out), R, P, Q, P, Q, Q, splits, _stream())
+        code = _L().vitamd_gemm_tn_bf16(_p(l), _p(r), _p(out), R, P, Q, ldl, ldr, Q, splits, _stream())
     else:
         nbytes = _L().vitamd_gemm_tn_ws_bytes(R, P, Q, splits)
         ws = _workspace(l.device, nbytes)
         if colsum is not None:
-            code = _L().vitamd_gemm_tn_bf16_ws_colsum(_p(l), _p(r), _p(out), _p(colsum), R, P, Q, P, Q, Q, splits, _p(ws), ws.numel() * 4,
+            code = _L().vitamd_gemm_tn_bf16_ws_colsum(_p(l), _p(r), _p(out), _p(colsum), R, P, Q, ldl, ldr, Q, splits, _p(ws), ws.numel() * 4,
                                                       int(accumulate), int(form), _stream())
         else:
-            code = _L().vitamd_gemm_tn_bf16_ws(_p(l), _p(r), _p(out), R, P, Q, P, Q, Q, splits, _p(ws), ws.numel() * 4, int(accumulate),
+            code = _L().vitamd_gemm_tn_bf16_ws(_p(l), _p(r), _p(out), R, P, Q, ldl, ldr, Q, splits, _p(ws), ws.numel() * 4, int(accumulate),
                                                int(form), _stream())
-    _lib.check(code, f"gemm_tn[R={R},P={P},Q={Q}]")
-    return out
+    _lib.check(code, f"gemm_tn[R={R},P={P},Q={Q},ldl={ldl},ldr={ldr}]")
+    return out if out_row0 is None else out_all
 
 
 def layernorm_fwd(x, addend=None):
@@ -343,7 +384,7 @@
     return o, lse
 
 
-def attention_bwd_keep(qkv, o, lse, d_o, B, N, H, nq, dbias=None, delta=None):
+def attention_bwd_keep(qkv, o, lse, d_o, B, N, H, nq, dbias=None, delta=None, kept_q_only=False):
     _need(qkv, BF16, "qkv", 2); _need(o, BF16, "o", 2); _need(d_o, BF16, "d_o", 2); _need(lse, F32, "lse")
     D = H * 64
     if tuple(qkv.shape) != (B * N, 3 * D) or tuple(o.shape) != (B * nq, D) or tuple(d_o.shape) != (B * nq, D) or lse.numel() != B * H * N:
@@ -357,7 +398,8 @@
         _need(delta, F32, "delta")
         if delta.numel() != B * H * N:
             raise _lib.VitamdError("attention_bwd_keep: delta must be [B, H, N]")
-    _lib.check(_L().vitamd_attention_bwd_keep(_p(qkv), _p(o), _p(lse), _p(d_o), _p(dqkv), _p(delta), _p(dbias), B, N, H, 64, nq, _stream()),
+    _lib.check(_L().vitamd_attention_bwd_keep_q(_p(qkv), _p(o), _p(lse), _p(d_o), _p(dqkv), _p(delta), _p(dbias), B, N, H, 64, nq, int(bool(kept_q_only)),
+                                              _stream()),
                f"attention_bwd_keep[B={B},N={N},H={H},nq={nq}]")
     return dqkv
 
```

Result: no change. 9159 images/sec, median of 6 (+0.3%).
